# lisaweijler/SE3Conv3D

Measured on AMD Instinct MI355X. Metric: Mpoints/sec fwd+bwd PNEConvLayerRotEquiv (N=64k,k=32,F=2), higher is better.
Workload: dtype bf16x3 (fp32 split into bf16 hi+lo, 3 MFMA products, fp32 accumulate); 1 GPU; headline: 4-level PNEConvLayerRotEquiv stack, N=65536, k=32, F=2, C=64; conv-only fwd+bwd (dX,dA,dbeta,dW), one scene per GPU; n_points=65536, clouds_per_gpu=1, k=32, frames=2, num_basis=32, point_order=random, launch=hipGraph replay of the captured step, cpu_threads_per_rank=8

## Files before the change

se3conv3d_amd/_lib.py:

```python
from __future__ import annotations

import ctypes as C
import os

_PKG = os.path.dirname(os.path.abspath(__file__))
LIB_PATH = os.path.join(_PKG, "lib", f"libse3conv_hip{os.environ.get('SE3_LIB_SUFFIX', '')}.so")

SE3_OK = 0
ABI_VERSION = 6
PRECISIONS = {"fp32": 0, "bf16x3": 1, "bf16x3_t16": 2}
REL_ROT = {"6D": (0, 9), "matrix": (1, 12), "quaternion": (2, 7)}


class Se3Shape(C.Structure):

    _fields_ = [
        ("n_in", C.c_int64), ("n_out", C.c_int64), ("n_edges", C.c_int64),
        ("f_in", C.c_int32), ("f_out", C.c_int32), ("c_in", C.c_int32), ("c_out", C.c_int32),
        ("num_basis", C.c_int32), ("precision", C.c_int32),
    ]


class Se3Prepared(C.Structure):

    _fields_ = [("geom_in", C.c_void_p), ("geom_out", C.c_void_p), ("feat_words", C.c_void_p),
                ("geom_in_valid", C.c_int32), ("geom_out_valid", C.c_int32), ("feat_words_valid", C.c_int32)]


class Se3LibraryError(RuntimeError):
    pass


_P = C.c_void_p
_I64 = C.c_int64
_I32 = C.c_int32
_SZ = C.c_size_t
_F = C.c_float
_SHP = C.POINTER(Se3Shape)

SIGNATURES = {
    "se3_abi_version": (C.c_int, []),
    "se3_error_string": (C.c_char_p, [C.c_int]),
    "se3conv_intermediate_bytes_per_element": (C.c_int, [_SHP, C.c_int]),
    "se3conv_intermediate_row_bytes": (C.c_int64, [_SHP, C.c_int]),
    "se3_compute_keys": (C.c_int, [_P, _P, _P, _P, _P, _I64, _P, _P]),
    "se3_batch_aabb": (C.c_int, [_P, _P, _I64, _I32, _P, _P, _P]),
    "se3_grid_subsample_workspace_bytes": (_SZ, [_I64, _I32]),
    "se3_grid_subsample": (C.c_int, [_P, _P, _I64, _I32, _F, _P, _SZ, _P, _P, _P, _P, _P, _P, _P]),
    "se3_segment_pool": (C.c_int, [_P, _P, _P, _I64, _I32, _I32, _P, _P, _P]),
    "se3_segment_unpool": (C.c_int, [_P, _P, _P, _P, _I64, _I32, _I32, _P, _P]),
    "se3_frame_pool": (C.c_int, [_P, _I64, _I32, _I32, _I32, _P, _P, _P]),
    "se3_frame_unpool": (C.c_int, [_P, _P, _I64, _I32, _I32, _I32, _P, _P]),
    "se3_ball_query_grid": (C.c_int, [_P, _P, _I64, _I32, _F, _P, _P, _P, _P]),
    "se3_ball_query_grid_from_box": (C.c_int, [_P, _P, _I32, _F, _P, _P, _P]),
    "se3_ball_query_needs_grid": (C.c_int, [_I64]),
    "se3_ball_query_workspace_bytes": (_SZ, [_I64, _I64]),
    "se3_ball_query_count": (C.c_int, [_P, _P, _P, _P, _P, _P, _F, _I64, _I64, _P, _SZ, _P, _P]),
    "se3_ball_query_store": (C.c_int, [_P, _P, _F, _I64, _I64, _P, _SZ, _P, _I64, _P, _P]),
    "se3_ball_query_bounded": (C.c_int, [_P, _P, _P, _P, _P, _P, _F, _I64, _I64, _I32, _P, _SZ, _I64, _P, _P, _P, _P, _P]),
    "se3_ball_query_grid_bytes": (_SZ, [_I64]),
    "se3_ball_query_bounded_shared": (C.c_int, [_P, _P, _P, _P, _P, _P, _F, _I64, _I64, _I32, _P, _SZ, _I32, _P, _SZ, _I64, _P,
                                                _P, _P, _P, _P]),
    "se3_csr_transpose_workspace_bytes": (_SZ, [_I64]),
    "se3_csr_transpose": (C.c_int, [_P, _I64, _I64, _P, _SZ, _P, _P, _P, _P]),
    "se3_csr_transpose_bounded": (C.c_int, [_P, _I64, _P, _I64, _P, _SZ, _P, _P, _P, _P]),
    "se3_rot_tensors": (C.c_int, [_P, _P, _P, _P, _P, _P, _P, _SHP, _P, _P, _P, _P]),
    "se3_rot_tensors_rel": (C.c_int, [_P, _P, _P, _P, _P, _P, _P, _SHP, _I32, _P, _P, _P, _P]),
    "se3_feat_basis_proj": (C.c_int, [_P, _P, _P, _P, _I64, _I64, _I64, _I32, _I32, _P, _P]),
    "se3_feat_basis_proj_grad": (C.c_int, [_P, _P, _P, _P, _P, _I64, _I64, _I64, _I32, _I32, _P, _P, _P]),
    "se3conv_fwd_workspace_bytes": (_SZ, [_SHP, C.c_int]),
    "se3conv_fwd": (C.c_int, [_P] * 12 + [_SHP, _P, _P, _P, _SZ, _P]),
    "se3conv_bwd_workspace_bytes": (_SZ, [_SHP, C.c_int, C.c_int, C.c_int]),
    "se3conv_bwd_needs_t": (C.c_int, [_SHP, C.c_int]),
    "se3conv_bwd": (C.c_int, [_P] * 17 + [_SHP, _P, _P, _P, _P, _P, _SZ, _P]),
    "se3conv_fwd_prepared": (C.c_int, [_P] * 12 + [_SHP, _P, _P, _P, _SZ, _P, C.POINTER(Se3Prepared)]),
    "se3conv_bwd_prepared": (C.c_int, [_P] * 17 + [_SHP, _P, _P, _P, _P, _P, _SZ, _P, C.POINTER(Se3Prepared)]),
    "se3_knn_query": (C.c_int, [_P, _P, _I64, _I32, _P, _P]),
    "se3_knn_query_pair": (C.c_int, [_P, _P, _I64, _P, _P, _I64, _I32, _P, _P]),
    "se3_grid_pick": (C.c_int, [_P, _P, _P, _I64, _P, _P, _P]),
    "se3_rows_gather": (C.c_int, [_P, _P, _I64, _I64, _P, _P]),
    "se3_rows_scatter": (C.c_int, [_P, _P, _I64, _I64, _P, _P]),
    "se3_knn_query_grid_workspace_bytes": (C.c_size_t, [_I64]),
    "se3_knn_grid_params": (C.c_int, [_P, _I64, _P, _P, _I32, _I32, C.c_float, _P, _P, _P, _P]),
    "se3_knn_query_grid": (C.c_int, [_P, _P, _P, _P, _P, _I64, _I32, _P, _P, C.c_size_t, _P]),
    "se3_pca_frames": (C.c_int, [_P, _P, _I64, _I32, _I32, _P, _P]),
    "se3_shuffle_frames": (C.c_int, [_P, _P, _I64, _I32, _I32, _P, _P]),
    "se3_glue_workspace_bytes": (_SZ, [_I32]),
    "se3_bn_fwd": (C.c_int, [_P, _P, _P, _I64, _I32, _F, _F, _P, _P, _P, _P, _P, _P, _P, _SZ, _P]),
    "se3_affine_act": (C.c_int, [_P, _P, _P, _P, _I64, _I32, _I32, _P, _P]),
    "se3_bn_bwd": (C.c_int, [_P, _P, _P, _P, _P, _I64, _I32, _P, _P, _P, _P, _SZ, _P]),
    "se3_skip_fwd": (C.c_int, [_P, _P, _P, _P, _F, _P, _I64, _I32, _P, _P]),
    "se3_skip_bwd": (C.c_int, [_P, _P, _P, _P, _F, _P, _I64, _I32, _P, _P, _P, _SZ, _P]),
    "se3_bias_gelu_bwd": (C.c_int, [_P, _P, _P, _I64, _I32, _P, _P, _P, _SZ, _P]),
    "se3_linear_wgrad_workspace_bytes": (_SZ, [_I64, _I32, _I32]),
    "se3_linear_wgrad": (C.c_int, [_P, _P, _I64, _I32, _I32, _P, _P, _SZ, _P]),
    "se3_profile_enable": (C.c_int, [C.c_int]),
    "se3_profile_reset": (C.c_int, []),
    "se3_profile_read": (C.c_int, [C.c_char_p, C.POINTER(C.c_double), C.POINTER(C.c_int64)]),
    "se3_profile_tags": (C.c_int, [C.c_char_p, _SZ]),
}

CAPPED_SIGNATURES = {
    "se3_ball_query_capped_workspace_bytes": (_SZ, [_I64, _I64]),
    "se3_ball_query_capped": (C.c_int, [_P, _P, _P, _P, _P, _P, _F, _I64, _I64, _I32, _P, _SZ, _I32, _P, _SZ, _I64, _P, _P, _P, _P,
                                        _P, _I32, C.c_uint32, _P, _P]),
}

_lib = None


def load() -> C.CDLL:
    global _lib
    if _lib is not None:
        return _lib
    if not os.path.exists(LIB_PATH):
        raise Se3LibraryError(
            f"{LIB_PATH} not found: build it with `python -m se3conv3d_amd.build` "
            "(there is deliberately no CPU fallback for the HIP path)")
    lib = C.CDLL(LIB_PATH)
    lib.se3_abi_version.restype = C.c_int
    if lib.se3_abi_version() != ABI_VERSION:
        raise Se3LibraryError(f"{LIB_PATH} has ABI version {lib.se3_abi_version()}, this binding expects {ABI_VERSION}: "
                              "rebuild it (`python -m se3conv3d_amd.build`)")
    for name, (res, args) in list(SIGNATURES.items()) + list(CAPPED_SIGNATURES.items()):
        try:
            fn = getattr(lib, name)
        except AttributeError:
            raise Se3LibraryError(f"{LIB_PATH} does not export {name}: it was built from older sources -- rebuild it "
                                  "(`python -m se3conv3d_amd.build`)") from None
        fn.restype = res
        fn.argtypes = args
    _lib = lib
    return lib


def check(code: int, what: str) -> None:
    if code != SE3_OK:
        msg = load().se3_error_string(code).decode()
        raise Se3LibraryError(f"{what} failed with code {code}: {msg}")
```

se3conv3d_amd/build.py:

```python
from __future__ import annotations

import hashlib
import os
import shutil
import subprocess
import sys
from concurrent.futures import ThreadPoolExecutor

PKG = os.path.dirname(os.path.abspath(__file__))
CSRC = os.path.join(PKG, "csrc")
SUFFIX = os.environ.get("SE3_LIB_SUFFIX", "")
LIBDIR = os.path.join(PKG, "lib")
OBJDIR = os.path.join(LIBDIR, "obj" + SUFFIX) if SUFFIX else LIBDIR
LIB = os.path.join(LIBDIR, f"libse3conv_hip{SUFFIX}.so")
SOURCES = ["geometry.hip", "edge_kernels.hip", "edge_bf16.hip", "edge_dx.hip", "gemm.hip", "gemm_bf16.hip", "prep.hip", "frames.hip", "glue.hip", "api.hip"]
HEADERS = [os.path.join(CSRC, "common.h"), os.path.join(CSRC, "edge_bf16_body.h"), os.path.join(os.path.dirname(PKG), "include", "se3conv.h"),
           os.path.join(os.path.dirname(PKG), "include", "se3conv_capped.h")]
ARCH = "gfx950"
FLAGS = os.environ.get("SE3_CXXFLAGS", "").split() + ["-O3", "-fno-slp-vectorize", "-std=c++17", "-fPIC", f"--offload-arch={ARCH}", "-fno-gpu-rdc", "-Wall", "-Wno-unused-function"]


def _hipcc() -> str:
    exe = shutil.which("hipcc") or "/opt/rocm/bin/hipcc"
    if not os.path.exists(exe):
        raise RuntimeError("hipcc not found: the HIP library cannot be built on this machine")
    return exe


def _stale(target: str, deps) -> bool:
    if not os.path.exists(target):
        return True
    t = os.path.getmtime(target)
    return any(os.path.getmtime(d) > t for d in deps)


def _fingerprint() -> str:
    return hashlib.sha256(" ".join([ARCH, *FLAGS]).encode()).hexdigest()


def build(force: bool = False, verbose: bool = True) -> str:
    os.makedirs(OBJDIR, exist_ok=True)
    hipcc = _hipcc()
    stamp = os.path.join(OBJDIR, "build_flags.sha256")
    fp = _fingerprint()
    try:
        with open(stamp) as fh:
            same_flags = fh.read().strip() == fp
    except OSError:
        same_flags = False
    force = force or not same_flags
    objs, jobs = [], []
    for src in SOURCES:
        s = os.path.join(CSRC, src)
        o = os.path.join(OBJDIR, src.replace(".hip", ".o"))
        objs.append(o)
        if force or _stale(o, [s] + HEADERS):
            jobs.append([hipcc, *FLAGS, "-c", s, "-o", o])

    def run(cmd):
        if verbose:
            print(" ".join(cmd), flush=True)
        subprocess.run(cmd, check=True)

    if jobs:
        if os.path.exists(stamp):
            os.remove(stamp)
        with ThreadPoolExecutor(max_workers=min(6, len(jobs))) as ex:
            list(ex.map(run, jobs))
    if jobs or force or _stale(LIB, objs):
        run([hipcc, "-shared", "-fPIC", f"--offload-arch={ARCH}", "-Wl,--no-undefined", *objs, "-o", LIB])
    with open(stamp, "w") as fh:
        fh.write(fp + "\n")
    return LIB


if __name__ == "__main__":
    print(build(force="--force" in sys.argv))
```

se3conv3d_amd/csrc/api.hip:

```cpp
#include <cstdlib>
#include <cstring>
#include <map>
#include <mutex>
#include <string>
#include <utility>
#include <vector>

#include "common.h"

namespace se3 {

namespace {

__global__ void transpose_kernel(const float* __restrict__ src, float* __restrict__ dst, int rows, int cols) {
  const int64_t total = (int64_t)rows * cols;
  for (int64_t i = (int64_t)blockIdx.x * blockDim.x + threadIdx.x; i < total; i += (int64_t)gridDim.x * blockDim.x) {
    const int c = (int)(i / rows), r = (int)(i % rows);
    dst[i] = src[(int64_t)r * cols + c];
  }
}

__global__ void permute_weights_oki_kernel(const float* __restrict__ w, float* __restrict__ w2, int c_in, int kb,
                                           int c_out) {
  const int64_t total = (int64_t)c_in * kb * c_out;
  for (int64_t idx = (int64_t)blockIdx.x * blockDim.x + threadIdx.x; idx < total;
       idx += (int64_t)gridDim.x * blockDim.x) {
    const int i = (int)(idx % c_in);
    const int ok = (int)(idx / c_in);
    const int k = ok % kb, o = ok / kb;
    w2[idx] = w[((int64_t)i * kb + k) * c_out + o];
  }
}

__global__ __launch_bounds__(256) void reduce_param_partials_kernel(const float* __restrict__ partials, int n_partials,
                                                                    float* __restrict__ grad_axes,
                                                                    float* __restrict__ grad_biases, float scale) {
  __shared__ float red[256];
  const int i = blockIdx.x;
  float s = 0.f;
  for (int p = threadIdx.x; p < n_partials; p += 256) s += partials[(int64_t)p * kDescExt * kBasis + i];
  red[threadIdx.x] = s;
  __syncthreads();
  for (int w = 128; w > 0; w >>= 1) {
    if (threadIdx.x < w) red[threadIdx.x] += red[threadIdx.x + w];
    __syncthreads();
  }
  if (threadIdx.x == 0) {
    if (i < SE3_DESC_DIMS * kBasis) {
      if (grad_axes) grad_axes[i] = red[0] * scale;
    } else if (grad_biases) {
      grad_biases[i - SE3_DESC_DIMS * kBasis] = red[0] * scale;
    }
  }
}


__device__ __forceinline__ void matrix_to_quaternion(const float m[9], float q[4]) {
  const float t[4] = {1.0f + m[0] + m[4] + m[8], 1.0f + m[0] - m[4] - m[8], 1.0f - m[0] + m[4] - m[8],
                      1.0f - m[0] - m[4] + m[8]};
  float qa[4];
  int best = 0;
#pragma unroll
  for (int i = 0; i < 4; ++i) {
    qa[i] = t[i] > 0.f ? sqrtf(t[i]) : 0.f;
    if (qa[i] > qa[best]) best = i;
  }
  const float c[4][4] = {{qa[0] * qa[0], m[7] - m[5], m[2] - m[6], m[3] - m[1]},
                         {m[7] - m[5], qa[1] * qa[1], m[3] + m[1], m[2] + m[6]},
                         {m[2] - m[6], m[3] + m[1], qa[2] * qa[2], m[5] + m[7]},
                         {m[3] - m[1], m[6] + m[2], m[7] + m[5], qa[3] * qa[3]}};
  const float den = 2.0f * fmaxf(qa[best], 0.1f);
#pragma unroll
  for (int i = 0; i < 4; ++i) q[i] = (best == 0 ? c[0][i] : best == 1 ? c[1][i] : best == 2 ? c[2][i] : c[3][i]) / den;
}

template <int REL>
__global__ void rot_tensors_kernel(const float* __restrict__ pts_in, const float* __restrict__ pts_out,
                                   const float* __restrict__ frames_in, const float* __restrict__ frames_out,
                                   const int32_t* __restrict__ neighbors, const int32_t* __restrict__ ends,
                                   const float* __restrict__ rho_p, int64_t n_edges, int f_in, int f_out,
                                   float* __restrict__ desc, int32_t* __restrict__ fe_neighbors) {
  constexpr int D = REL == 0 ? 9 : (REL == 1 ? 12 : 7);
  const float rho = *rho_p;
  const int ff = f_in * f_out;
  for (int64_t t = (int64_t)blockIdx.x * blockDim.x + threadIdx.x; t < n_edges * ff;
       t += (int64_t)gridDim.x * blockDim.x) {
    const int64_t e = t / ff;
    const int ab = (int)(t - e * ff);
    const int a = ab / f_in, b = ab % f_in;
    const int s = neighbors[e * 2], p = neighbors[e * 2 + 1];
    const int start = s > 0 ? ends[s - 1] : 0;
    const int deg = ends[s] - start;
    const int64_t idx = (int64_t)ff * start + (int64_t)a * deg * f_in + (e - start) * f_in + b;
    float x[3], y[3], ri[9], ro[9], d[9];
#pragma unroll
    for (int i = 0; i < 3; ++i) x[i] = pts_in[(int64_t)p * 3 + i], y[i] = pts_out[(int64_t)s * 3 + i];
#pragma unroll
    for (int i = 0; i < 9; ++i)
      ri[i] = frames_in[((int64_t)p * f_in + b) * 9 + i], ro[i] = frames_out[((int64_t)s * f_out + a) * 9 + i];
    edge_descriptor(x, ri, y, ro, rho, d);
    if constexpr (REL == 0) {
#pragma unroll
      for (int i = 0; i < 9; ++i) desc[idx * 9 + i] = d[i];
    } else {
      float rel[9];
#pragma unroll
      for (int i = 0; i < 6; ++i) rel[i] = d[3 + i];
#pragma unroll
      for (int c = 0; c < 3; ++c) rel[6 + c] = ro[2] * ri[c] + ro[5] * ri[3 + c] + ro[8] * ri[6 + c];
#pragma unroll
      for (int i = 0; i < 3; ++i) desc[idx * D + i] = d[i];
      if constexpr (REL == 1) {
#pragma unroll
        for (int i = 0; i < 9; ++i) desc[idx * D + 3 + i] = rel[i];
      } else {
        float q[4];
        matrix_to_quaternion(rel, q);
#pragma unroll
        for (int i = 0; i < 4; ++i) desc[idx * D + 3 + i] = q[i];
      }
    }
    fe_neighbors[idx * 2] = s * f_out + a;
    fe_neighbors[idx * 2 + 1] = p * f_in + b;
  }
}

__global__ void rot_tensor_ends_kernel(const int32_t* __restrict__ ends, int64_t n_out, int f_in, int f_out,
                                       int32_t* __restrict__ fe_ends) {
  for (int64_t m = (int64_t)blockIdx.x * blockDim.x + threadIdx.x; m < n_out * f_out;
       m += (int64_t)gridDim.x * blockDim.x) {
    const int64_t s = m / f_out;
    const int a = (int)(m - s * f_out);
    const int start = s > 0 ? ends[s - 1] : 0;
    const int deg = ends[s] - start;
    fe_ends[m] = f_in * f_out * start + (a + 1) * deg * f_in;
  }
}

__global__ __launch_bounds__(256) void feat_basis_proj_kernel(const float* __restrict__ basis,
                                                              const float* __restrict__ feat,
                                                              const int32_t* __restrict__ neighbors,
                                                              const int32_t* __restrict__ ends, int channels, int kb,
                                                              float* __restrict__ out) {
  const int64_t m = blockIdx.x;
  const int start = m > 0 ? ends[m - 1] : 0, end = ends[m];
  const int k = threadIdx.x % kb, cg = threadIdx.x / kb, ncg = blockDim.x / kb;
  for (int c = cg; c < channels; c += ncg) {
    float acc = 0.f;
    for (int e = start; e < end; ++e)
      acc += basis[(int64_t)e * kb + k] * feat[(int64_t)neighbors[(int64_t)e * 2 + 1] * channels + c];
    out[(m * channels + c) * kb + k] = acc;
  }
}

__device__ __forceinline__ int row_of_edge(const int32_t* __restrict__ ends, int64_t n_rows, int64_t e) {
  int64_t lo = 0, hi = n_rows;
  while (lo < hi) {
    const int64_t mid = (lo + hi) >> 1;
    if (ends[mid] <= e) lo = mid + 1; else hi = mid;
  }
  return (int)lo;
// ... 285 lines not shown
  const size_t wsz = (size_t)s->c_in * kBasis * s->c_out * 4;
  l.slices = (s->num_basis + kBasis - 1) / kBasis;
  l.a32 = take(SE3_DESC_DIMS * kBasis * 4);
  l.b32 = take(kBasis * 4);
  l.w32 = take(wsz);
  l.out_tmp = take(l.slices > 1 ? out_tmp_bytes : 0);
  if (grads) {
    l.da32 = take(SE3_DESC_DIMS * kBasis * 4);
    l.db32 = take(kBasis * 4);
    l.dw32 = take(wsz);
  }
  l.inner = take(inner_bytes);
  l.total = off;
  return l;
}
int64_t slice_items(const se3conv_shape* s) {
  const int64_t n_w = (int64_t)s->c_in * kBasis * s->c_out;
  return n_w > SE3_DESC_DIMS * kBasis ? n_w : SE3_DESC_DIMS * kBasis;
}
se3conv_shape with_32_basis(const se3conv_shape* s) {
  se3conv_shape t = *s;
  t.num_basis = kBasis;
  return t;
}

}
}

using namespace se3;

extern "C" int se3_abi_version(void) { return SE3_ABI_VERSION; }

extern "C" const char* se3_error_string(int code) {
  switch (code) {
    case SE3_OK: return "ok";
    case SE3_ERR_INVALID_ARGUMENT: return "invalid argument (null pointer, negative size or bad shape)";
    case SE3_ERR_UNSUPPORTED: return "unsupported shape (int32-sized clouds; API-parity ops: K in {8, 16, 32, 64})";
    case SE3_ERR_WORKSPACE: return "workspace too small";
    case SE3_ERR_LAUNCH: return "HIP launch/runtime error";
    default: return "unknown error";
  }
}

extern "C" int se3_rot_tensors_rel(const float* pts_in, const float* pts_out, const float* frames_in,
                                   const float* frames_out, const int32_t* neighbors, const int32_t* ends,
                                   const float* rho, const se3conv_shape* s, int32_t rel_rot, float* desc,
                                   int32_t* fe_neighbors, int32_t* fe_ends, void* stream_) {
  if (!shape_ok(s) || rel_rot < SE3_REL_ROT_6D || rel_rot > SE3_REL_ROT_QUATERNION) return SE3_ERR_INVALID_ARGUMENT;
  if (s->n_edges * s->f_in * s->f_out >= (1ll << 31)) return SE3_ERR_UNSUPPORTED;
  hipStream_t stream = (hipStream_t)stream_;
  if (s->n_out > 0) {
    if (!ends || !fe_ends) return SE3_ERR_INVALID_ARGUMENT;
    hipLaunchKernelGGL(rot_tensor_ends_kernel, dim3(grid_for(s->n_out * s->f_out)), dim3(256), 0, stream, ends, s->n_out,
                       s->f_in, s->f_out, fe_ends);
  }
  if (s->n_edges > 0) {
    if (!pts_in || !pts_out || !frames_in || !frames_out || !neighbors || !ends || !rho || !desc || !fe_neighbors)
      return SE3_ERR_INVALID_ARGUMENT;
    const dim3 grid(grid_for(s->n_edges * s->f_in * s->f_out));
#define SE3_ROT(REL)                                                                                                  \
  hipLaunchKernelGGL(rot_tensors_kernel<REL>, grid, dim3(256), 0, stream, pts_in, pts_out, frames_in, frames_out, neighbors, \
                     ends, rho, s->n_edges, s->f_in, s->f_out, desc, fe_neighbors)
    if (rel_rot == SE3_REL_ROT_6D) SE3_ROT(0);
    else if (rel_rot == SE3_REL_ROT_MATRIX) SE3_ROT(1);
    else SE3_ROT(2);
#undef SE3_ROT
  }
  return check_launch();
}

extern "C" int se3_rot_tensors(const float* pts_in, const float* pts_out, const float* frames_in,
                               const float* frames_out, const int32_t* neighbors, const int32_t* ends,
                               const float* rho, const se3conv_shape* s, float* desc, int32_t* fe_neighbors,
                               int32_t* fe_ends, void* stream) {
  return se3_rot_tensors_rel(pts_in, pts_out, frames_in, frames_out, neighbors, ends, rho, s, SE3_REL_ROT_6D, desc,
                             fe_neighbors, fe_ends, stream);
}

static bool basis_count_ok(int kb) { return kb == 8 || kb == 16 || kb == 32 || kb == 64; }

extern "C" int se3_feat_basis_proj(const float* basis, const float* feat, const int32_t* neighbors, const int32_t* ends,
                                   int64_t n_edges, int64_t n_rows, int64_t n_feat, int32_t channels,
                                   int32_t num_basis, float* out, void* stream) {
  if (n_edges < 0 || n_rows < 0 || n_feat < 0 || channels < 1) return SE3_ERR_INVALID_ARGUMENT;
  if (!basis_count_ok(num_basis)) return SE3_ERR_UNSUPPORTED;
  if (n_rows == 0) return SE3_OK;
  if (!ends || !out || (n_edges > 0 && (!basis || !feat || !neighbors))) return SE3_ERR_INVALID_ARGUMENT;
  if (n_rows >= (1ll << 31)) return SE3_ERR_UNSUPPORTED;
  hipLaunchKernelGGL(feat_basis_proj_kernel, dim3((unsigned)n_rows), dim3(256), 0, (hipStream_t)stream, basis, feat,
                     neighbors, ends, channels, num_basis, out);
  return check_launch();
}

extern "C" int se3_feat_basis_proj_grad(const float* basis, const float* feat, const int32_t* neighbors,
                                        const int32_t* ends, const float* grad_out, int64_t n_edges, int64_t n_rows,
                                        int64_t n_feat, int32_t channels, int32_t num_basis, float* g_feat,
                                        float* g_basis, void* stream_) {
  if (n_edges < 0 || n_rows < 0 || n_feat < 0 || channels < 1) return SE3_ERR_INVALID_ARGUMENT;
  if (!basis_count_ok(num_basis)) return SE3_ERR_UNSUPPORTED;
  hipStream_t stream = (hipStream_t)stream_;
  if (n_feat > 0) {
    if (!g_feat) return SE3_ERR_INVALID_ARGUMENT;
    if (int rc = launch_fill_words(g_feat, 0u, n_feat * channels, stream)) return rc;
  }
  if (n_edges == 0) return SE3_OK;
  if (!basis || !feat || !neighbors || !ends || !grad_out || !g_basis) return SE3_ERR_INVALID_ARGUMENT;
  hipLaunchKernelGGL(feat_basis_proj_grad_basis_kernel, dim3(grid_for(n_edges * num_basis)), dim3(256), 0, stream, feat,
                     neighbors, ends, grad_out, n_edges, n_rows, channels, num_basis, g_basis);
  hipLaunchKernelGGL(feat_basis_proj_grad_feat_kernel, dim3(grid_for(n_edges * channels)), dim3(256), 0, stream, basis,
                     neighbors, ends, grad_out, n_edges, n_rows, channels, num_basis, g_feat);
  return check_launch();
}

static int64_t intermediate_row_bytes(const se3conv_shape* s, int which) {
  const int64_t ck = (int64_t)(which == 1 ? s->c_out : s->c_in) * s->num_basis;
  if (s->precision == SE3_PRECISION_FP32 || s->num_basis != kBasis || which == 2) return ck * 4;
  const BwdPlan p = plan_bwd(s, true, true, false);
  const int fmt = which == 0 ? p.fmt_t : p.fmt_u;
  return fmt == 2 ? t16_row_bytes(which == 0 ? s->c_in : s->c_out) : ck * (fmt == 1 ? 3 : 4);
}
extern "C" int64_t se3conv_intermediate_row_bytes(const se3conv_shape* s, int which) {
  if (!shape_ok(s) || which < 0 || which > 2) return SE3_ERR_INVALID_ARGUMENT;
  return intermediate_row_bytes(s, which);
}
extern "C" int se3conv_intermediate_bytes_per_element(const se3conv_shape* s, int which) {
  if (!shape_ok(s) || which < 0 || which > 2) return SE3_ERR_INVALID_ARGUMENT;
  const int64_t ck = (int64_t)(which == 1 ? s->c_out : s->c_in) * s->num_basis;
  return (int)(intermediate_row_bytes(s, which) / ck);
}

extern "C" size_t se3conv_fwd_workspace_bytes(const se3conv_shape* s, int save_t) {
  if (!shape_ok(s)) return 0;
  if (s->num_basis != kBasis) {
    const se3conv_shape s32 = with_32_basis(s);
    return any_basis_layout(s, (size_t)s->n_out * s->f_out * s->c_out * 4, false, plan_fwd(&s32, false).total).total;
  }
  return plan_fwd(s, save_t != 0).total;
}

extern "C" int se3conv_fwd(const float* pts_in, const float* pts_out, const float* frames_in, const float* frames_out,
                           const int32_t* neighbors, const int32_t* ends, const float* feat, const float* proj_axes,
                           const float* proj_biases, const float* conv_weights, const float* rho, const float* nu,
                           const se3conv_shape* s, float* out, float* t_save, void* workspace, size_t workspace_bytes,
                           void* stream_) {
  return se3conv_fwd_prepared(pts_in, pts_out, frames_in, frames_out, neighbors, ends, feat, proj_axes, proj_biases, conv_weights,
                              rho, nu, s, out, t_save, workspace, workspace_bytes, stream_, nullptr);
}

extern "C" int se3conv_fwd_prepared(const float* pts_in, const float* pts_out, const float* frames_in, const float* frames_out,
                                    const int32_t* neighbors, const int32_t* ends, const float* feat, const float* proj_axes,
                                    const float* proj_biases, const float* conv_weights, const float* rho, const float* nu,
                                    const se3conv_shape* s, float* out, float* t_save, void* workspace, size_t workspace_bytes,
                                    void* stream_, const se3conv_prepared* prep) {
  if (!shape_ok(s)) return SE3_ERR_INVALID_ARGUMENT;
  if (s->num_basis != kBasis) {
    if (s->n_out == 0) return SE3_OK;
    if (!proj_axes || !proj_biases || !conv_weights || !out || !workspace) return SE3_ERR_INVALID_ARGUMENT;
    const se3conv_shape s32 = with_32_basis(s);
    const int64_t n_out_el = s->n_out * s->f_out * s->c_out;
    const AnyBasisLayout l = any_basis_layout(s, (size_t)n_out_el * 4, false, plan_fwd(&s32, false).total);
    if (workspace_bytes < l.total) return SE3_ERR_WORKSPACE;
    hipStream_t stream = (hipStream_t)stream_;
    char* ws = (char*)workspace;
    float *a32 = (float*)(ws + l.a32), *b32 = (float*)(ws + l.b32), *w32 = (float*)(ws + l.w32);
    for (int sl = 0; sl < l.slices; ++sl) {
      const int k0 = sl * kBasis, kn = s->num_basis - k0 < kBasis ? s->num_basis - k0 : kBasis;
      hipLaunchKernelGGL(slice_params_kernel, dim3(grid_for(slice_items(s))), dim3(256), 0, stream,
                         proj_axes, proj_biases, conv_weights, s->num_basis, k0, kn, s->c_in, s->c_out, a32, b32, w32);
      float* dst = sl == 0 ? out : (float*)(ws + l.out_tmp);
      if (int rc = se3conv_fwd(pts_in, pts_out, frames_in, frames_out, neighbors, ends, feat, a32, b32, w32, rho, nu, &s32, dst,
                               nullptr, ws + l.inner, l.total - l.inner, stream_))
        return rc;
      if (sl > 0)
        hipLaunchKernelGGL(add_into_kernel, dim3(grid_for(n_out_el)), dim3(256), 0, stream, out, dst, n_out_el);
    }
    return check_launch();
  }
  if (int rc = shape_supported(s)) return rc;
  if (s->n_out == 0) return SE3_OK;
  if (!pts_out || !frames_out || !ends || !proj_axes || !proj_biases || !conv_weights || !rho || !nu || !out ||
      !workspace || (s->n_edges > 0 && (!pts_in || !frames_in || !neighbors || !feat)))
    return SE3_ERR_INVALID_ARGUMENT;
  const FwdPlan p = plan_fwd(s, t_save != nullptr);
  if (workspace_bytes < p.total) return SE3_ERR_WORKSPACE;
  hipStream_t stream = (hipStream_t)stream_;
  char* ws = (char*)workspace;
  float* axes_ext = (float*)(ws + p.axes_ext);
  float* t = t_save ? t_save : (float*)(ws + p.t);

  EdgeGeom g = forward_geom(s, pts_in, pts_out, frames_in, frames_out, neighbors, ends);
  const int64_t rows_out = s->n_out * s->f_out;
  const int ck = s->c_in * s->num_basis;
  const float inv_fin = 1.0f / (float)s->f_in;
  PrepBatch pb;
  pb.axes(proj_axes, proj_biases, axes_ext);
  prepare_geometry(pb, prep, s, (float*)(ws + p.geom_in), (float*)(ws + p.geom_out), &g, nullptr);
  if (s->precision == SE3_PRECISION_FP32) {
    if (int rc = pb.launch(stream)) return rc;
    if (int rc = launch_edge_t("edge_t_fwd", g, feat, s->c_in, s->n_in * s->f_in, axes_ext, rho, t, stream)) return rc;
    return launch_gemm_nn("gemm_out", t, conv_weights, out, rows_out, s->c_out, ck, nu, inv_fin, stream, (float*)(ws + p.split));
  }
  uint32_t* featpk = prep && prep->feat_words ? prep->feat_words : (uint32_t*)(ws + p.featpk);
  const bool need_featpk = !(prep && prep->feat_words && prep->feat_words_valid);
  uint16_t* bt_hi = (uint16_t*)(ws + p.bt_hi);
  uint16_t* bt_lo = (uint16_t*)(ws + p.bt_lo);
  const float inv_phi = inv_fin / kGeluOut;
  if (need_featpk) pb.split(feat, featpk, s->n_in * s->f_in * s->c_in);
  pb.weights(conv_weights, s->c_in, s->num_basis, s->c_out, 0, bt_hi, bt_lo, nullptr, 1.0f, false, p.fmt_t);
  if (int rc = pb.launch(stream)) return rc;
  if (int rc = launch_edge_t_bf16("edge_t_fwd", g, featpk, s->c_in, s->n_in * s->f_in, axes_ext, rho, (uint32_t*)t, stream, p.fmt_t))
    return rc;
  return launch_gemm_nn_bf16("gemm_out", (const uint32_t*)t, bt_hi, bt_lo, out, false, rows_out, s->c_out, ck,
                             (float*)(ws + p.split), nu, inv_phi, stream, p.fmt_t);
}

extern "C" int se3conv_bwd_needs_t(const se3conv_shape* s, int want_feat) {
  if (!shape_ok(s)) return SE3_ERR_INVALID_ARGUMENT;
  if (s->num_basis != kBasis) return 0;
  return plan_bwd(s, want_feat != 0, true, false).dw == WeightGrad::u ? 0 : 1;
}

extern "C" size_t se3conv_bwd_workspace_bytes(const se3conv_shape* s, int want_feat, int want_params, int have_t) {
  if (!shape_ok(s)) return 0;
  if (s->num_basis != kBasis) {
    const se3conv_shape s32 = with_32_basis(s);
    return any_basis_layout(s, want_feat ? (size_t)s->n_in * s->f_in * s->c_in * 4 : 0, want_params != 0,
                            plan_bwd(&s32, want_feat != 0, want_params != 0, false).total).total;
  }
  return plan_bwd(s, want_feat != 0, want_params != 0, have_t != 0).total;
}

extern "C" int se3conv_bwd(const float* pts_in, const float* pts_out, const float* frames_in, const float* frames_out,
                           const int32_t* neighbors, const int32_t* ends, const int32_t* t_samples,
                           const int32_t* t_ends, const int32_t* t_edge_ids, const float* feat, const float* proj_axes,
                           const float* proj_biases,
                           const float* conv_weights, const float* rho, const float* nu, const float* t_save,
                           const float* grad_out, const se3conv_shape* s, float* grad_feat, float* grad_axes,
                           float* grad_biases, float* grad_weights, void* workspace, size_t workspace_bytes,
                           void* stream_) {
  return se3conv_bwd_prepared(pts_in, pts_out, frames_in, frames_out, neighbors, ends, t_samples, t_ends, t_edge_ids, feat, proj_axes,
                              proj_biases, conv_weights, rho, nu, t_save, grad_out, s, grad_feat, grad_axes, grad_biases, grad_weights,
                              workspace, workspace_bytes, stream_, nullptr);
}

extern "C" int se3conv_bwd_prepared(const float* pts_in, const float* pts_out, const float* frames_in, const float* frames_out,
                                    const int32_t* neighbors, const int32_t* ends, const int32_t* t_samples,
                                    const int32_t* t_ends, const int32_t* t_edge_ids, const float* feat, const float* proj_axes,
                                    const float* proj_biases, const float* conv_weights, const float* rho, const float* nu,
                                    const float* t_save, const float* grad_out, const se3conv_shape* s, float* grad_feat,
                                    float* grad_axes, float* grad_biases, float* grad_weights, void* workspace,
                                    size_t workspace_bytes, void* stream_, const se3conv_prepared* prep) {
  if (!shape_ok(s)) return SE3_ERR_INVALID_ARGUMENT;
  if (s->num_basis != kBasis) {
    const bool wf = grad_feat != nullptr, wp = grad_axes || grad_biases || grad_weights;
    if (!wf && !wp) return SE3_OK;
    if (!proj_axes || !proj_biases || !conv_weights || !workspace) return SE3_ERR_INVALID_ARGUMENT;
    const se3conv_shape s32 = with_32_basis(s);
    const int64_t n_in_el = s->n_in * s->f_in * s->c_in;
    const AnyBasisLayout l = any_basis_layout(s, wf ? (size_t)n_in_el * 4 : 0, wp, plan_bwd(&s32, wf, wp, false).total);
    if (workspace_bytes < l.total) return SE3_ERR_WORKSPACE;
    hipStream_t stream = (hipStream_t)stream_;
    char* ws = (char*)workspace;
    float *a32 = (float*)(ws + l.a32), *b32 = (float*)(ws + l.b32), *w32 = (float*)(ws + l.w32);
    float *da32 = wp ? (float*)(ws + l.da32) : nullptr, *db32 = wp ? (float*)(ws + l.db32) : nullptr;
    float* dw32 = wp ? (float*)(ws + l.dw32) : nullptr;
    const dim3 pgrid(grid_for(slice_items(s)));
    for (int sl = 0; sl < l.slices; ++sl) {
      const int k0 = sl * kBasis, kn = s->num_basis - k0 < kBasis ? s->num_basis - k0 : kBasis;
      hipLaunchKernelGGL(slice_params_kernel, pgrid, dim3(256), 0, stream, proj_axes, proj_biases, conv_weights,
                         s->num_basis, k0, kn, s->c_in, s->c_out, a32, b32, w32);
      float* dx = !wf ? nullptr : (sl == 0 ? grad_feat : (float*)(ws + l.out_tmp));
      if (int rc = se3conv_bwd(pts_in, pts_out, frames_in, frames_out, neighbors, ends, t_samples, t_ends, t_edge_ids, feat, a32, b32, w32, rho,
                               nu, nullptr, grad_out, &s32, dx, da32, db32, dw32, ws + l.inner, l.total - l.inner, stream_))
        return rc;
      if (wf && sl > 0 && n_in_el > 0)
        hipLaunchKernelGGL(add_into_kernel, dim3(grid_for(n_in_el)), dim3(256), 0, stream, grad_feat, dx, n_in_el);
      if (wp)
        hipLaunchKernelGGL(unslice_grads_kernel, pgrid, dim3(256), 0, stream, da32, db32, dw32, s->num_basis, k0, kn, s->c_in,
                           s->c_out, grad_axes, grad_biases, grad_weights);
    }
    return check_launch();
  }
  if (int rc = shape_supported(s)) return rc;
  const bool want_feat = grad_feat != nullptr;
  const bool want_params = grad_axes || grad_biases || grad_weights;
  if (!want_feat && !want_params) return SE3_OK;
  if (!proj_axes || !proj_biases || !conv_weights || !rho || !nu || !workspace) return SE3_ERR_INVALID_ARGUMENT;
  if (s->n_out > 0 && (!pts_out || !frames_out || !ends || !grad_out)) return SE3_ERR_INVALID_ARGUMENT;
  if (s->n_in > 0 && (!pts_in || !frames_in || !feat)) return SE3_ERR_INVALID_ARGUMENT;
  if (s->n_edges > 0 && !neighbors) return SE3_ERR_INVALID_ARGUMENT;
  if (want_feat && s->n_in > 0 && (!t_ends || (s->n_edges > 0 && !t_samples))) return SE3_ERR_INVALID_ARGUMENT;
  const BwdPlan p = plan_bwd(s, want_feat, want_params, t_save != nullptr);
  if (workspace_bytes < p.total) return SE3_ERR_WORKSPACE;
  hipStream_t stream = (hipStream_t)stream_;
  char* ws = (char*)workspace;
  float* axes_ext = (float*)(ws + p.axes_ext);
  float* big = (float*)(ws + p.big);
  const int kb = s->num_basis;
  const int ck = s->c_in * kb;
  const int64_t rows_out = s->n_out * s->f_out, rows_in = s->n_in * s->f_in;
  const float inv_fin = 1.0f / (float)s->f_in;
  float* partials = (float*)(ws + p.param_partials);
  float* tn_partials = (float*)(ws + p.tn_partials);

  EdgeGeom g = forward_geom(s, pts_in, pts_out, frames_in, frames_out, neighbors, ends);
  EdgeGeom gt = transposed_geom(s, pts_in, pts_out, frames_in, frames_out, t_samples, t_ends);
  PrepBatch pb;
  pb.axes(proj_axes, proj_biases, axes_ext);
  prepare_geometry(pb, prep, s, (float*)(ws + p.geom_in), (float*)(ws + p.geom_out), &g, &gt);

  if (!p.fast) {
    if (int rc = pb.launch(stream)) return rc;
    if (want_params) {
      float* wt = (float*)(ws + p.wt);
      hipLaunchKernelGGL(transpose_kernel, dim3(grid_for((int64_t)ck * s->c_out)), dim3(256), 0, stream, conv_weights,
                         wt, ck, s->c_out);
      if (int rc = launch_gemm_nn("gemm_gradT", grad_out, wt, big, rows_out, ck, s->c_out, nu, inv_fin, stream)) return rc;
      if (grad_axes || grad_biases) {
        int n_part = 0;
        if (int rc = launch_edge_param_grad("edge_param_grad", g, feat, s->c_in, rows_in, axes_ext, rho, big, partials,
                                            p.n_param_partials, &n_part, stream))
          return rc;
        hipLaunchKernelGGL(reduce_param_partials_kernel, dim3(kDescExt * kBasis), dim3(256), 0, stream, partials,
                           n_part, grad_axes, grad_biases, 1.0f);
      }
      if (grad_weights) {
        const float* t = t_save;
        if (p.dw == WeightGrad::t_recomputed) {
          float* tt = (float*)(ws + p.t);
          if (int rc = launch_edge_t("edge_t_recompute", g, feat, s->c_in, rows_in, axes_ext, rho, tt, stream)) return rc;
          t = tt;
        }
        if (int rc = launch_gemm_tn("gemm_gradW", t, grad_out, grad_weights, tn_partials, p.tn.splits, p.tn.m, p.tn.ka,
                                    p.tn.n, nu, inv_fin, stream))
          return rc;
      }
    }
    if (p.feat_branch) {
      float* u = (float*)(ws + p.u);
      if (int rc = launch_edge_t("edge_t_transposed", gt, grad_out, s->c_out, rows_out, axes_ext, rho, u, stream)) return rc;
      float* w2 = (float*)(ws + p.w2);
      hipLaunchKernelGGL(permute_weights_oki_kernel, dim3(grid_for((int64_t)ck * s->c_out)), dim3(256), 0, stream,
                         conv_weights, w2, s->c_in, kb, s->c_out);
      if (int rc = launch_gemm_nn("gemm_gradX", u, w2, grad_feat, rows_in, s->c_in, s->c_out * kb, nu, inv_fin, stream,
                                  (float*)(ws + p.split_x)))
        return rc;
    }
    return check_launch();
  }

  const bool u_form = p.feat_branch && p.feat == FeatGrad::u, edge_major = p.feat == FeatGrad::edge_major;
  uint16_t* bt_hi = (uint16_t*)(ws + p.bt_hi);
  uint16_t* bt_lo = (uint16_t*)(ws + p.bt_lo);
  uint16_t* bx_hi = (uint16_t*)(ws + p.bx_hi);
  uint16_t* bx_lo = (uint16_t*)(ws + p.bx_lo);
  uint32_t* gpk = (uint32_t*)(ws + p.gpk);
  const bool have_featpk = prep && prep->feat_words && prep->feat_words_valid;
  uint32_t* featpk = prep && prep->feat_words ? prep->feat_words : (uint32_t*)(ws + p.featpk);
  uint32_t* bigw = (uint32_t*)big;
  uint32_t* u = (uint32_t*)(ws + p.u);
  const float inv_phi = inv_fin / kGeluOut;
  pb.split(grad_out, gpk, rows_out * s->c_out);
  if (u_form) pb.weights(conv_weights, s->c_in, kb, s->c_out, 2, bx_hi, bx_lo, nullptr, 1.0f, false, p.fmt_u);
  if (want_params && !have_featpk) pb.split(feat, featpk, rows_in * s->c_in);
  if (p.grad_t)
    pb.weights(conv_weights, s->c_in, kb, s->c_out, 1, bt_hi, bt_lo, nu, inv_fin, p.strip_t);
  if (int rc = pb.launch(stream)) return rc;
  ReduceBatch final_sums;

  if (u_form) {
    if (int rc = launch_edge_t_bf16("edge_t_transposed", gt, gpk, s->c_out, rows_out, axes_ext, rho, u, stream, p.fmt_u))
      return rc;
  }
  if (p.grad_t) {
    if (int rc = p.strip_t ? launch_gemm_strip_bf16("gemm_gradT", gpk, bt_hi, bt_lo, bigw, rows_out, ck, s->c_out, stream)
                           : launch_gemm_nn_bf16("gemm_gradT", gpk, bt_hi, bt_lo, bigw, true, rows_out, ck, s->c_out,
                                                 (float*)(ws + p.split), nullptr, 1.0f, stream))
      return rc;
  }
  if (edge_major) {
    float* d_rows = (float*)(ws + p.dx_rows);
    if (int rc = launch_edge_dx_bf16("edge_dx", g, axes_ext, rho, bigw, s->c_in, d_rows, stream)) return rc;
    if (int rc = launch_dx_gather_sum("dx_gather", d_rows, neighbors, ends, t_samples, t_ends, t_edge_ids, s->n_in, s->f_in * s->c_in,
                                      1.0f / kGeluOut, grad_feat, stream))
      return rc;
  }
  if (grad_axes || grad_biases) {
    int n_part = 0;
    if (int rc = launch_edge_param_grad_bf16("edge_param_grad", g, featpk, s->c_in, rows_in, axes_ext, rho, bigw, partials,
                                             p.n_param_partials, &n_part, stream))
      return rc;
    final_sums.params(partials, n_part, grad_axes, grad_biases, 0.5f);
  }
  if (u_form) {
    if (int rc = launch_gemm_nn_bf16("gemm_gradX", u, bx_hi, bx_lo, grad_feat, false, rows_in, s->c_in, s->c_out * kb,
                                     (float*)(ws + p.split_x), nu, inv_phi, stream, p.fmt_u, &final_sums))
      return rc;
  }
  if (grad_weights) {
    if (p.dw == WeightGrad::u) {
      if (int rc = launch_gemm_tn_bf16("gemm_gradW", u, featpk, grad_weights, tn_partials, p.tn.splits, p.tn.m, p.tn.ka, p.tn.n,
                                       nu, inv_phi, stream, p.fmt_u, &final_sums, true))
        return rc;
    } else {
      const uint32_t* t = (const uint32_t*)t_save;
      if (p.dw == WeightGrad::t_recomputed) {
        uint32_t* tt = (uint32_t*)(ws + p.t);
        if (int rc = launch_edge_t_bf16("edge_t_recompute", g, featpk, s->c_in, rows_in, axes_ext, rho, tt, stream, p.fmt_t)) return rc;
        t = tt;
      }
      if (int rc = launch_gemm_tn_bf16("gemm_gradW", t, gpk, grad_weights, tn_partials, p.tn.splits, p.tn.m, p.tn.ka, p.tn.n, nu,
                                       inv_phi, stream, p.fmt_t, &final_sums))
        return rc;
    }
  }
  return final_sums.launch(stream);
}


namespace se3 {
namespace {
struct ProfRec { std::string tag; hipEvent_t start, stop; };
std::mutex g_prof_mu;
bool g_prof_on = false;
std::vector<ProfRec> g_prof_recs;
std::map<std::string, std::pair<double, int64_t>> g_prof_acc;
ProfRec* g_prof_open = nullptr;

void prof_drain_locked() {
  for (auto& r : g_prof_recs) {
    float ms = 0.f;
    if (hipEventSynchronize(r.stop) == hipSuccess && hipEventElapsedTime(&ms, r.start, r.stop) == hipSuccess) {
      auto& a = g_prof_acc[r.tag];
      a.first += ms;
      a.second += 1;
    }
    (void)hipEventDestroy(r.start);
    (void)hipEventDestroy(r.stop);
  }
  g_prof_recs.clear();
}
}

void prof_begin(const char* tag, hipStream_t stream) {
  if (!g_prof_on) return;
  std::lock_guard<std::mutex> lk(g_prof_mu);
  ProfRec r;
  r.tag = tag;
  if (hipEventCreate(&r.start) != hipSuccess || hipEventCreate(&r.stop) != hipSuccess) return;
  (void)hipEventRecord(r.start, stream);
  g_prof_recs.push_back(r);
  g_prof_open = &g_prof_recs.back();
}

void prof_end(hipStream_t stream) {
  if (!g_prof_on) return;
  std::lock_guard<std::mutex> lk(g_prof_mu);
  if (g_prof_open) (void)hipEventRecord(g_prof_open->stop, stream);
  g_prof_open = nullptr;
// ... 38 lines not shown
```

se3conv3d_amd/csrc/common.h:

```cpp
#pragma once

#include <hip/hip_runtime.h>
#include <stddef.h>
#include <stdint.h>

#include "../../include/se3conv.h"

namespace se3 {

using f32x16 = __attribute__((__vector_size__(16 * sizeof(float)))) float;
using f32x4 = __attribute__((__vector_size__(4 * sizeof(float)))) float;

constexpr int kWave = 64;
constexpr int kBasis = 32;
constexpr int kDescExt = 10;

__host__ __device__ constexpr int acc_row(int reg, int h) { return (reg & 3) + 8 * (reg >> 2) + 4 * h; }

__device__ __forceinline__ f32x16 mfma32(float a, float b, f32x16 c) {
  return __builtin_amdgcn_mfma_f32_32x32x2f32(a, b, c, 0, 0, 0);
}

using bf16x8 = __attribute__((__vector_size__(8 * sizeof(__bf16)))) __bf16;
using bf16x2 = __attribute__((__vector_size__(2 * sizeof(__bf16)))) __bf16;
// ... 132 lines not shown
  gelu_erf_core(x, s, a, e, hq);
  return fmaf(a, hq, 0.5f * x);
}

constexpr float kGeluIn = 0.84932180028801904272f;
constexpr float kGeluOut = 2.0f * kGeluIn;
__device__ __forceinline__ void gelu_scaled_core(float xp, float& a, float& e, float& hq2) {
  a = fabsf(xp);
  const float t = __builtin_amdgcn_rcpf(fmaf(0.23164189f / kGeluIn, a, 1.0f));
  float p = fmaf(1.061405429f, t, -1.453152027f);
  p = fmaf(p, t, 1.421413741f);
  p = fmaf(p, t, -0.284496736f);
  p = fmaf(p, t, 0.254829592f);
  e = __builtin_amdgcn_exp2f(-(xp * xp));
  hq2 = fmaf(-(p * t), e, 1.0f);
}
#ifndef SE3_GELU_POLY
#define SE3_GELU_POLY 5
#endif
__device__ __forceinline__ float gelu_scaled(float xp) {
#if SE3_GELU_POLY == 0
  float a, e, hq2;
  gelu_scaled_core(xp, a, e, hq2);
  return fmaf(a, hq2, xp);
#else
  const float a = fabsf(xp);
#if SE3_GELU_POLY == 7
  float p = fmaf(-3.000000106e-06f, a, 1.157411680e-04f);
  p = fmaf(p, a, -1.839424018e-03f);
  p = fmaf(p, a, 1.570610516e-02f);
  p = fmaf(p, a, -8.734710515e-02f);
  p = fmaf(p, a, -6.359119415e-01f);
  p = fmaf(p, a, -1.355453730e+00f);
  p = fmaf(p, a, 8.137106306e-06f);
#else
  float p = fmaf(-1.070951186e-03f, a, 1.361500331e-02f);
  p = fmaf(p, a, -8.459421670e-02f);
  p = fmaf(p, a, -6.376852093e-01f);
  p = fmaf(p, a, -1.354949055e+00f);
  p = fmaf(p, a, -3.763227806e-05f);
#endif
  const float q2 = __builtin_amdgcn_exp2f(p);
  return fmaf(-a, q2, a + xp);
#endif
}
__device__ __forceinline__ void gelu_scaled_grad(float xp, float& y2, float& dy2) {
  float a, e, hq2;
  gelu_scaled_core(xp, a, e, hq2);
  y2 = fmaf(a, hq2, xp);
  dy2 = fmaf(__builtin_copysignf(1.0f, xp), fmaf(a * e, 0.79788456080286535588f / kGeluIn, hq2), 1.0f);
}
#ifndef SE3_GELU_DPOLY
#define SE3_GELU_DPOLY (SE3_GELU_POLY ? 7 : 0)
#endif
__device__ __forceinline__ float gelu_scaled_dgrad(float xp) {
#if SE3_GELU_DPOLY == 0
  float y2, dy2;
  gelu_scaled_grad(xp, y2, dy2);
  return dy2;
#else
  const float a = fabsf(xp);
  float p = fmaf(-6.029059296e-05f, a, 9.206497925e-04f);
  p = fmaf(p, a, -6.434103474e-03f);
  p = fmaf(p, a, 2.816033363e-02f);
  p = fmaf(p, a, -8.932273835e-02f);
  p = fmaf(p, a, -7.773189545e-01f);
  p = fmaf(p, a, -4.511650503e-01f);
  p = fmaf(p, a, 6.472119689e-01f);
  const float g = fmaf(a - 6.385129094e-01f, __builtin_amdgcn_exp2f(p), 1.0f);
  return fmaf(__builtin_copysignf(1.0f, xp), g, 1.0f);
#endif
}

__device__ __forceinline__ void edge_descriptor(const float x_in[3], const float r_in[9],
                                                const float y_out[3], const float r_out[9],
                                                float rho, float d[9]) {
  const float v0 = (x_in[0] - y_out[0]) * rho;
  const float v1 = (x_in[1] - y_out[1]) * rho;
  const float v2 = (x_in[2] - y_out[2]) * rho;
#pragma unroll
  for (int c = 0; c < 3; ++c) d[c] = v0 * r_out[c] + v1 * r_out[3 + c] + v2 * r_out[6 + c];
#pragma unroll
  for (int r = 0; r < 2; ++r)
#pragma unroll
    for (int c = 0; c < 3; ++c)
      d[3 + 3 * r + c] = r_out[r] * r_in[c] + r_out[3 + r] * r_in[3 + c] + r_out[6 + r] * r_in[6 + c];
}

constexpr int kOobOffset = 0x7fff0000;

__device__ __forceinline__ __amdgpu_buffer_rsrc_t buffer_of(const void* p, int64_t bytes) {
  const uint32_t n = bytes > 0xffffffffll ? 0xffffffffu : (uint32_t)bytes;
  return __builtin_amdgcn_make_buffer_rsrc(const_cast<void*>(p), (short)0, (int)n, 0x00020000);
}

__device__ __forceinline__ void load_geom_record(const __amdgpu_buffer_rsrc_t rs, int row, float x[3], float r[9]) {
  const int off = row * 64;
  const auto v0 = __builtin_amdgcn_raw_buffer_load_b128(rs, off, 0, 0);
  const auto v1 = __builtin_amdgcn_raw_buffer_load_b128(rs, off + 16, 0, 0);
  const auto v2 = __builtin_amdgcn_raw_buffer_load_b128(rs, off + 32, 0, 0);
  x[0] = __uint_as_float(v0[0]), x[1] = __uint_as_float(v0[1]), x[2] = __uint_as_float(v0[2]);
  r[8] = __uint_as_float(v0[3]);
#pragma unroll
  for (int i = 0; i < 4; ++i) r[i] = __uint_as_float(v1[i]), r[4 + i] = __uint_as_float(v2[i]);
}

#ifndef SE3_ROTATE_PRIO
#define SE3_ROTATE_PRIO 1
#endif
__device__ __forceinline__ void rotate_priority(int step_plus_slot) {
#if SE3_ROTATE_PRIO
  switch (step_plus_slot & 3) {
    case 0: __builtin_amdgcn_s_setprio(0); break;
    case 1: __builtin_amdgcn_s_setprio(1); break;
    case 2: __builtin_amdgcn_s_setprio(2); break;
    default: __builtin_amdgcn_s_setprio(3); break;
  }
#endif
}
__device__ __forceinline__ int wave_slot_id() { return (int)__builtin_amdgcn_s_getreg((4 << 0) | (0 << 6) | (3 << 11)) ; }

inline int check_launch() {
  hipError_t e = hipGetLastError();
  return e == hipSuccess ? SE3_OK : SE3_ERR_LAUNCH;
}

inline size_t align_up(size_t v, size_t a) { return (v + a - 1) / a * a; }

int launch_fill_words(void* dst, uint32_t value, int64_t n_words, hipStream_t stream);

void prof_begin(const char* tag, hipStream_t stream);
void prof_end(hipStream_t stream);
struct ProfScope {
  hipStream_t s;
  ProfScope(const char* tag, hipStream_t stream) : s(stream) { prof_begin(tag, s); }
  ~ProfScope() { prof_end(s); }
};

struct EdgeGeom {
  const float* ctr_pts;
  const float* ctr_frames;
  const float* nb_pts;
  const float* nb_frames;
  const float* ctr_geom;
  const float* nb_geom;
  int64_t n_nb;
  int64_t n_edges;
  const int32_t* nbr;
  int nbr_stride, nbr_offset;
  const int32_t* ends;
  int64_t n_ctr;
  int f_ctr, f_nb;
  int transposed;
};

int launch_edge_t(const char* tag, const EdgeGeom& g, const float* feat, int channels, int64_t feat_rows,
                  const float* axes_ext, const float* rho, float* t_out, hipStream_t stream);
int launch_edge_param_grad(const char* tag, const EdgeGeom& g, const float* feat, int channels, int64_t feat_rows,
                           const float* axes_ext, const float* rho, const float* grad_t, float* partials,
                           int n_partials, int* n_used, hipStream_t stream);
int edge_param_grad_blocks(int64_t rows);

int launch_gemm_nn(const char* tag, const float* a, const float* b, float* c, int64_t m, int n, int k,
                   const float* alpha_num, float alpha_scale, hipStream_t stream, float* split_ws = nullptr);
size_t gemm_nn_split_bytes(int64_t m, int n, int k);
int launch_gemm_tn(const char* tag, const float* a, const float* b, float* c, float* partials, int splits, int64_t m,
                   int ka, int n, const float* alpha_num, float alpha_scale, hipStream_t stream);
int gemm_tn_splits(int64_t m, int ka, int n);
int launch_reduce_partials(const float* partials, float* out, int64_t count, int splits, const float* alpha_num,
                           float alpha_scale, hipStream_t stream);

struct ReduceJob {
  int type, blocks;
  const float* partials;
  void *out, *out2;
  int64_t count;
  int splits, packed;
  const float* alpha_num;
  float alpha_scale;
  int perm_n;
};
struct ReduceJobs {
  int count;
  ReduceJob job[4];
};
struct ReduceBatch {
  ReduceJobs jobs{};
  void sum(const float* partials, void* out, int64_t count, int splits, const float* alpha_num, float alpha_scale, bool packed,
           int perm_n = 0);
  void params(const float* partials, int n_partials, float* grad_axes, float* grad_biases, float scale);
  int launch(hipStream_t stream);
};

int launch_split_pack(const float* src, uint32_t* dst, int64_t n, hipStream_t stream);
bool edge_t_bf16_t24_rows(const EdgeGeom& g, int channels);
bool edge_t_bf16_t16_rows(const EdgeGeom& g, int channels);
int launch_edge_t_bf16(const char* tag, const EdgeGeom& g, const uint32_t* feat, int channels, int64_t feat_rows,
                       const float* axes_ext, const float* rho, uint32_t* t_out, hipStream_t stream,
                       int rowfmt = 0);
int edge_param_grad_bf16_channel_blocks(int channels);
int launch_edge_param_grad_bf16(const char* tag, const EdgeGeom& g, const uint32_t* feat, int channels,
                                int64_t feat_rows, const float* axes_ext, const float* rho, const uint32_t* grad_t,
                                float* partials, int n_partials, int* n_used, hipStream_t stream);
bool edge_dx_bf16_applicable(const EdgeGeom& g, int channels);
int launch_edge_dx_bf16(const char* tag, const EdgeGeom& g, const float* axes_ext, const float* rho, const uint32_t* grad_t,
                        int channels, float* d_rows, hipStream_t stream);
int launch_dx_gather_sum(const char* tag, const float* d_rows, const int32_t* neighbors, const int32_t* ends,
                         const int32_t* t_samples, const int32_t* t_ends, const int32_t* t_edge_ids, int64_t n_src, int width,
                         float scale, float* grad_feat, hipStream_t stream);
int launch_prep_weights(const float* w, int c_in, int kb, int c_out, int mode, uint16_t* bt_hi, uint16_t* bt_lo,
                        hipStream_t stream, const float* scale_num = nullptr, float scale = 1.0f,
                        bool frag_layout = false);
__device__ __forceinline__ float knn_dist2(float dx, float dy, float dz) { return fmaf(dz, dz, fmaf(dy, dy, dx * dx)); }
int launch_knn_bruteforce(const float* pts, const int32_t* batch_ids, int64_t n, const float* qpts, const int32_t* qbatch,
                          int64_t m, int k, int32_t* out, hipStream_t stream);
int launch_knn_listed(const float* pts, const int32_t* batch_ids, int64_t n, int k, int32_t* out, const int32_t* list,
                      const int32_t* list_count, hipStream_t stream);

template <int K>
struct TopK {
  uint64_t key[K];
  static __device__ __forceinline__ uint64_t pack(float d, int i) {
    return ((uint64_t)__float_as_uint(d) << 32) | (uint64_t)(uint32_t)i;
  }
  __device__ __forceinline__ float dist(int e) const { return __uint_as_float((uint32_t)(key[e] >> 32)); }
  __device__ __forceinline__ int idx(int e) const { return (int)(uint32_t)key[e]; }
  __device__ __forceinline__ void set(int e, float d, int i) { key[e] = pack(d, i); }
  __device__ __forceinline__ void init() {
#pragma unroll
    for (int e = 0; e < K; ++e) key[e] = pack(3.0e38f, 0x7fffffff);
  }
  __device__ __forceinline__ void cas(int a, int b) {
    const uint64_t x = key[a], y = key[b];
    const bool sw = y < x;
    key[a] = sw ? y : x, key[b] = sw ? x : y;
  }
  __device__ __forceinline__ void insert(float dd, int jj) {
    const uint64_t k = pack(dd, jj);
    if (!(k < key[K - 1])) return;
    key[K - 1] = k;
#pragma unroll
    for (int e = K - 1; e > 0; --e) cas(e - 1, e);
  }
  __device__ __forceinline__ void merge_xor(int mask) {
    uint64_t tmp[K];
#pragma unroll
    for (int e = 0; e < K; ++e) {
      const uint32_t lo = (uint32_t)__shfl_xor((int)(uint32_t)key[K - 1 - e], mask);
      const uint32_t hi = (uint32_t)__shfl_xor((int)(uint32_t)(key[K - 1 - e] >> 32), mask);
      tmp[e] = ((uint64_t)hi << 32) | lo;
    }
#pragma unroll
    for (int e = 0; e < K; ++e)
      if (tmp[e] < key[e]) key[e] = tmp[e];
#pragma unroll
    for (int s = K / 2; s > 0; s >>= 1)
#pragma unroll
      for (int e = 0; e < K; ++e)
        if ((e & s) == 0) cas(e, e + s);
  }
};

struct PrepJob {
  int type, blocks;
  const void *a, *b;
  void *o0, *o1;
  int64_t n;
  int p[8];
  float scale;
};
struct PrepJobs {
  int count;
  PrepJob job[8];
};
struct PrepBatch {
  PrepJobs jobs{};
  int status = SE3_OK;
  void axes(const float* axes, const float* biases, float* ext);
  void geometry(const float* pts, const float* frames, int64_t n, int f, float* records);
  void split(const float* src, uint32_t* dst, int64_t n);
  void weights(const float* w, int c_in, int kb, int c_out, int mode, uint16_t* bt_hi, uint16_t* bt_lo,
               const float* scale_num = nullptr, float scale = 1.0f, bool frag_layout = false,
               int a_rowfmt = 0);
  int launch(hipStream_t stream);
};

int launch_pack_geometry(const float* pts, const float* frames, int64_t n, int f, float* records, hipStream_t stream);
bool gemm_strip_bf16_applicable(int64_t m, int n, int k);
int launch_gemm_strip_bf16(const char* tag, const uint32_t* a, const uint16_t* bt_hi, const uint16_t* bt_lo, uint32_t* c,
                           int64_t m, int n, int k, hipStream_t stream);
int launch_gemm_nn_bf16(const char* tag, const uint32_t* a, const uint16_t* bt_hi, const uint16_t* bt_lo, void* c,
                        bool out_packed, int64_t m, int n, int k, float* split_ws, const float* alpha_num,
                        float alpha_scale, hipStream_t stream, int afmt = 0, ReduceBatch* defer = nullptr);
size_t gemm_nn_bf16_split_bytes(int64_t m, int n, int k);
int launch_gemm_tn_bf16(const char* tag, const uint32_t* a, const uint32_t* b, float* c, float* partials, int splits,
                        int64_t m, int ka, int n, const float* alpha_num, float alpha_scale, hipStream_t stream, int afmt = 0,
                        ReduceBatch* defer = nullptr,
                        bool out_ikn = false);

}
```

se3conv3d_amd/csrc/edge_bf16.hip:

```cpp
#include <cstdlib>

#include "common.h"
#include "edge_bf16_body.h"

#ifndef SE3_TIMELINE
#define SE3_TIMELINE 0
#endif
#if SE3_TIMELINE
#define TL(...) __VA_ARGS__
namespace se3 {
constexpr int kTlWords = 64;
__device__ uint32_t* g_tl_buf = nullptr;
__device__ uint32_t g_tl_cap = 0;
__device__ __forceinline__ uint32_t tl_now() {
  unsigned long long t;
  __builtin_amdgcn_sched_barrier(0);
  asm volatile("s_memtime %0\n\ts_waitcnt lgkmcnt(0)" : "=s"(t)::"memory");
  __builtin_amdgcn_sched_barrier(0);
  return (uint32_t)t;
}
template <class T>
__device__ __forceinline__ void tl_pin(const T& x) { asm volatile("" ::"v"(x)); }
__device__ __forceinline__ void tl_mark(uint32_t* rec, int slot) { const uint32_t t = tl_now(); if (slot < kTlWords) rec[slot] = t; }
__device__ __forceinline__ void tl_seg(uint32_t* rec, uint32_t& prev, int slot) { const uint32_t t = tl_now(); rec[slot] += t - prev; prev = t; }
// ... 164 lines not shown
#pragma unroll
      for (int t = 0; t < CT; ++t) acc[a][t] = zero16();
    int nb_b = 0, q_a = 0;
    float xn_nx[3], rn_nx[9];
    if (n_total > 0) {
      const int nb_a = nbr_of(0);
      nb_b = nbr_of(32);
      TL(tl_mark(tl_rec, 4); tl_pin(nb_a); tl_mark(tl_rec, 5);)
      q_a = row_of(nb_a, 0);
      load_geom_record(nbg_rs, q_a, xn_nx, rn_nx);
    }
    TL(tl_mark(tl_rec, 6);)
    for (int c0 = 0; c0 < n_total; c0 += 32, buf ^= 1) {
      const int cnt = min(32, n_total - c0);
      const int qoff = c0 + kcol < n_total ? q_a * row_bytes : kOobOffset;
      float xn[3], rn[9], d[9];
#pragma unroll
      for (int i = 0; i < 3; ++i) asm volatile("" : "+v"(yc[i]));
#pragma unroll
      for (int i = 0; i < 9; ++i) asm volatile("" : "+v"(rc[i]));
#pragma unroll
      for (int i = 0; i < 3; ++i) xn[i] = xn_nx[i];
#pragma unroll
      for (int i = 0; i < 9; ++i) rn[i] = rn_nx[i];
      const int q_b = row_of(nb_b, c0 + 32);
      nb_b = nbr_of(c0 + 64);

      uint32_t fw[CT][2][8];
#pragma unroll
      for (int s = 0; s < 2; ++s)
#pragma unroll
        for (int j = 0; j < 8; ++j) {
          const int src_off = __builtin_amdgcn_ds_bpermute(hb + 4 * acc_row(8 * s + j, 0), qoff);
#pragma unroll
          for (int t = 0; t < CT; ++t)
            fw[t][s][j] = __builtin_amdgcn_raw_buffer_load_b32(feat_rs, ch_ok[t] ? src_off + cb4[t] : kOobOffset, 0, 0);
        }
      load_geom_record(nbg_rs, q_b, xn_nx, rn_nx);
      q_a = q_b;
      TL(tl_mark(tl_rec, tl_ch + 1); tl_pin(xn[0]); tl_pin(rn[7]); tl_pin(rn[8]); tl_mark(tl_rec, tl_ch + 2);)

      if (TR == 0 || (TR < 0 && !g.transposed))
        edge_descriptor(xn, rn, yc, rc, rho, d);
      else
        edge_descriptor(yc, rc, xn, rn, rho, d);

      {
        float v[8];
#pragma unroll
        for (int j = 0; j < 8; ++j) v[j] = h ? (j == 0 ? d[8] : (j == 1 ? 1.0f : 0.f)) : d[j];
        u32x4 a_hi, a_lo;
        frags_from_floats(v, a_hi, a_lo);
        const u32x4 wb_hi = *reinterpret_cast<const u32x4*>(&lds_w[0][0][lane][0]);
        const u32x4 wb_lo = *reinterpret_cast<const u32x4*>(&lds_w[0][1][lane][0]);
        const f32x16 phi = mfma_bf16x3(a_hi, a_lo, wb_hi, wb_lo, zero16());
        TL(tl_pin(phi[0]); tl_mark(tl_rec, tl_ch + 3);)
#pragma unroll
        for (int s = 0; s < 2; ++s) {
          if (s * 16 < cnt && (NF == 2 || s == wv)) {
            float pv[8];
#pragma unroll
            for (int j = 0; j < 8; ++j) pv[j] = gelu_scaled(phi[8 * s + j]);
            u32x4 b_hi, b_lo;
            frags_from_floats(pv, b_hi, b_lo);
            *reinterpret_cast<u32x4*>(&lds_phi[buf][NF == 2 ? wv : 0][s][0][lane][0]) = b_hi;
            *reinterpret_cast<u32x4*>(&lds_phi[buf][NF == 2 ? wv : 0][s][1][lane][0]) = b_lo;
          }
        }
      }
      TL(tl_mark(tl_rec, tl_ch + 4);)
      __syncthreads();
      TL(tl_mark(tl_rec, tl_ch + 5); tl_pin(fw[0][0][7]); tl_mark(tl_rec, tl_ch + 6);)
#pragma unroll
      for (int s = 0; s < 2; ++s) {
        if (s * 16 < cnt) {
          u32x4 b_hi[NF], b_lo[NF];
#pragma unroll
          for (int a = 0; a < NF; ++a) {
            b_hi[a] = *reinterpret_cast<const u32x4*>(&lds_phi[buf][a][s][0][lane][0]);
            b_lo[a] = *reinterpret_cast<const u32x4*>(&lds_phi[buf][a][s][1][lane][0]);
          }
#pragma unroll
          for (int t = 0; t < CT; ++t) {
            u32x4 fa_hi, fa_lo;
            frags_from_words(fw[t][s], fa_hi, fa_lo);
#pragma unroll
            for (int a = 0; a < NF; ++a) acc[a][t] = mfma_bf16x3(fa_hi, fa_lo, b_hi[a], b_lo[a], acc[a][t]);
          }
        }
      }
      TL(tl_mark(tl_rec, tl_ch + 7); tl_ch += 8;)
    }
    TL(tl_mark(tl_rec, 7); tl_pin(acc[NF - 1][CT - 1][15]); tl_mark(tl_rec, 8);)
#pragma unroll
    for (int a = 0; a < NF; ++a)
#pragma unroll
      for (int t = 0; t < CT; ++t) {
        const int ch0 = cbase + 32 * (CT * wv + t);
        if (t24 == 2) {
          if (!FULL && ch0 >= C) continue;
          char* row = reinterpret_cast<char*>(t_out) + (item * NF + a) * t16_row_bytes(C);
          uint8_t* expo = reinterpret_cast<uint8_t*>(row) + (int64_t)C * kBasis * 2;
#pragma unroll
          for (int j = 0; j < 4; ++j) {
            const int cq = (ch0 >> 2) + 2 * j + h;
            uint32_t m01, m23, eb;
            t16_pack4(acc[a][t][4 * j], acc[a][t][4 * j + 1], acc[a][t][4 * j + 2], acc[a][t][4 * j + 3], m01, m23, eb);
            typedef uint32_t u32x2s __attribute__((ext_vector_type(2)));
            __builtin_nontemporal_store(u32x2s{m01, m23}, reinterpret_cast<u32x2s*>(row) + cq * kBasis + kcol);
            __builtin_nontemporal_store((uint8_t)eb, expo + t16_exp_pos(cq * kBasis + kcol));
          }
          continue;
        }
        if (t24) {
          char* row = reinterpret_cast<char*>(t_out) + (item * NF + a) * t24_row_bytes(C);
#pragma unroll
          for (int r = 0; r < 16; r += 2) {
            const int ch = ch0 + acc_row(r, h);
            if (!FULL && ch >= C) continue;
            uint32_t hp, lp;
            t24_pack2(acc[a][t][r], (FULL || ch + 1 < C) ? acc[a][t][r + 1] : 0.f, hp, lp);
            const int idx = (ch >> 1) * kBasis + kcol;
            __builtin_nontemporal_store(hp, reinterpret_cast<uint32_t*>(row) + idx);
            __builtin_nontemporal_store((uint16_t)lp, reinterpret_cast<uint16_t*>(row + (int64_t)C * kBasis * 2) + idx);
          }
          continue;
        }
        uint32_t* t_row = t_out + ((item * NF + a) * (int64_t)C + ch0) * kBasis;
#pragma unroll
        for (int r = 0; r < 16; r += 2) {
          uint32_t w0, w1;
          split_pack2(acc[a][t][r], acc[a][t][r + 1], w0, w1);
          if (FULL || ch0 + acc_row(r, h) < C) __builtin_nontemporal_store(w0, &t_row[acc_row(r, h) * kBasis + kcol]);
          if (FULL || ch0 + acc_row(r + 1, h) < C) __builtin_nontemporal_store(w1, &t_row[acc_row(r + 1, h) * kBasis + kcol]);
        }
      }
    if (cbase + 64 * CT < C) __syncthreads();
  }
  TL(tl_mark(tl_rec, 9); __builtin_amdgcn_s_waitcnt(0); tl_mark(tl_rec, 10);
     tl_rec[11] = __builtin_amdgcn_s_getreg((4 << 0) | (0 << 6) | (31 << 11)); tl_rec[12] = __builtin_amdgcn_s_getreg((20 << 0) | (0 << 6) | (31 << 11));
     tl_rec[13] = (uint32_t)item; tl_rec[14] = (uint32_t)((tl_ch - 16) >> 3); tl_flush(TR == 1 ? 1 : 0, (uint32_t)(item - item_lo) * 2 + wv, tl_rec);)
  }
}

struct ChunkCursor {
  int j;
  int c0;
  int start;
  int n_total;
  int crow;
  uint32_t item;
};

template <int TR>
__global__ __launch_bounds__(128, SE3_PAIR_WAVES) void edge_t_stream_bf16_kernel(
    EdgeGeom g, const uint32_t* __restrict__ feat, int64_t feat_rows, const float* __restrict__ axes_ext,
    const float* __restrict__ rho_p, char* __restrict__ t_out, uint32_t item_lo, uint32_t item_hi, int fnb_shift) {
  constexpr int C = 64, row_bytes = C * 4;
  __shared__ __attribute__((aligned(16))) uint32_t lds_w[1][2][64][4];
  __shared__ __attribute__((aligned(16))) uint32_t lds_phi[2][2][2][2][64][4];
  TL(__shared__ uint32_t tl_lds[2][kTlWords]; uint32_t* tl_rec = tl_lds[threadIdx.x >> 6]; tl_rec[threadIdx.x & 63] = 0u; tl_mark(tl_rec, 0); uint32_t tl_chunks = 0;)
  const int lane = threadIdx.x & 63, wv = threadIdx.x >> 6;
  const int kcol = lane & 31, h = lane >> 5;
  if (threadIdx.x < 64) mlp_weights_to_lds<1>(lds_w, axes_ext, threadIdx.x);
  __syncthreads();
  const float rho = *rho_p;
  const __amdgpu_buffer_rsrc_t feat_rs = buffer_of(feat, feat_rows * row_bytes);
  const __amdgpu_buffer_rsrc_t nbg_rs = buffer_of(g.nb_geom, g.n_nb * g.f_nb * 64);
  const __amdgpu_buffer_rsrc_t nbr_rs = buffer_of(g.nbr, g.n_edges * g.nbr_stride * 4);
  const uint32_t groups = (uint32_t)g.f_ctr / 2u;
  const uint32_t item0_wg = item_lo + blockIdx.x;
  const int n_mine = (int)((item_hi - item0_wg + gridDim.x - 1) / gridDim.x);
  const int fmask = (1 << fnb_shift) - 1;
  const int hb = 16 * h;

  f32x16 acc[2] = {zero16(), zero16()};
  int buf = 0;
  int prio_step = wave_slot_id();
  const int n_all = n_mine;
  for (int win0 = 0; win0 < n_all; win0 += 64) {
  const int n_mine = min(64, n_all - win0);
  const uint32_t item0 = item0_wg + (uint32_t)win0 * gridDim.x;
  int v_lo, v_hi;
  {
    const uint32_t item = item0 + (uint32_t)min(lane, n_mine - 1) * gridDim.x;
    const uint32_t ctr = item / groups;
    v_hi = g.ends[ctr];
    v_lo = g.ends[max((int)ctr - 1, 0)];
    if (ctr == 0) v_lo = 0;
  }
  auto uni = [](int x) { return __builtin_amdgcn_readfirstlane(x); };
  auto enter = [&](int j, int crow_keep, uint32_t item_keep) {
    ChunkCursor c;
    c.j = j, c.c0 = 0, c.start = 0, c.n_total = 0;
    c.crow = crow_keep, c.item = item_keep;
    if (j < n_mine) {
      const int lo = __builtin_amdgcn_readlane(v_lo, j), hi = __builtin_amdgcn_readlane(v_hi, j);
      c.start = lo, c.n_total = (hi - lo) << fnb_shift;
      c.item = item0 + (uint32_t)j * gridDim.x;
      const uint32_t ctr = c.item / groups;
      c.crow = uni((int)(ctr * (uint32_t)g.f_ctr + (c.item - ctr * groups) * 2u) + wv);
    }
    return c;
  };
  auto advance = [&](const ChunkCursor& c) {
    ChunkCursor r = c;
    if (c.c0 + 32 < c.n_total) r.c0 = c.c0 + 32;
    else if (c.j < n_mine) r = enter(c.j + 1, c.crow, c.item);
    r.j = uni(r.j), r.c0 = uni(r.c0), r.start = uni(r.start), r.n_total = uni(r.n_total), r.item = (uint32_t)uni((int)r.item);
    return r;
  };
  auto fe_of = [&](const ChunkCursor& c) { return max(min(c.c0 + kcol, c.n_total - 1), 0); };
  auto nbr_of = [&](const ChunkCursor& c) {
    const int e = c.start + (fe_of(c) >> fnb_shift);
    return (int)__builtin_amdgcn_raw_buffer_load_b32(nbr_rs, (e * g.nbr_stride + g.nbr_offset) * 4, 0, 0);
  };
  auto row_of = [&](int nb, const ChunkCursor& c) { return (nb << fnb_shift) + (fe_of(c) & fmask); };
  typedef const f32x4 __attribute__((address_space(4))) * crec_t;
  const crec_t ctr_rec = (crec_t)(uintptr_t)g.ctr_geom;
  auto centre = [&](const ChunkCursor& c, float yc[3], float rc[9]) {
    const int row = c.crow;
    const f32x4 v0 = ctr_rec[row * 4], v1 = ctr_rec[row * 4 + 1], v2 = ctr_rec[row * 4 + 2];
    yc[0] = v0[0], yc[1] = v0[1], yc[2] = v0[2], rc[8] = v0[3];
#pragma unroll
    for (int i = 0; i < 4; ++i) rc[i] = v1[i], rc[4 + i] = v2[i];
  };

  ChunkCursor cur, n1, n2;
  cur = enter(0, 0, 0u);
  n1 = advance(cur);
  n2 = advance(n1);
  int q_cur, q_n1;
  float xn_nx[3], rn_nx[9];
  {
    const int nb_cur = nbr_of(cur);
    const int nb_n1 = nbr_of(n1);
    q_cur = row_of(nb_cur, cur);
    load_geom_record(nbg_rs, q_cur, xn_nx, rn_nx);
    q_n1 = row_of(nb_n1, n1);
#pragma unroll
    for (int i = 0; i < 3; ++i) asm volatile("" : "+v"(xn_nx[i]));
#pragma unroll
    for (int i = 0; i < 9; ++i) asm volatile("" : "+v"(rn_nx[i]));
  }
  float yc[3], rc[9];
  centre(cur, yc, rc);

  while (cur.j < n_mine) {
    rotate_priority(prio_step++);
    const int cnt = min(32, cur.n_total - cur.c0);
    const int qoff = cur.c0 + kcol < cur.n_total ? q_cur * row_bytes : kOobOffset;
    float xn[3], rn[9], d[9];
#pragma unroll
    for (int i = 0; i < 3; ++i) xn[i] = xn_nx[i];
#pragma unroll
    for (int i = 0; i < 9; ++i) rn[i] = rn_nx[i];
    const int nb_n2 = nbr_of(n2);

    uint32_t fw[2][8];
#pragma unroll
    for (int s = 0; s < 2; ++s)
#pragma unroll
      for (int j = 0; j < 8; ++j) {
        const int src_off = __builtin_amdgcn_ds_bpermute(hb + 4 * acc_row(8 * s + j, 0), qoff);
        fw[s][j] = __builtin_amdgcn_raw_buffer_load_b32(feat_rs, src_off + (32 * wv + kcol) * 4, 0, 0);
      }
    load_geom_record(nbg_rs, q_n1, xn_nx, rn_nx);
    float yn[3], rnc[9];
    centre(n1, yn, rnc);

    if (TR == 0)
      edge_descriptor(xn, rn, yc, rc, rho, d);
    else
      edge_descriptor(yc, rc, xn, rn, rho, d);

    {
      float v[8];
#pragma unroll
      for (int j = 0; j < 8; ++j) v[j] = h ? (j == 0 ? d[8] : (j == 1 ? 1.0f : 0.f)) : d[j];
      u32x4 a_hi, a_lo;
      frags_from_floats(v, a_hi, a_lo);
      const u32x4 wb_hi = *reinterpret_cast<const u32x4*>(&lds_w[0][0][lane][0]);
      const u32x4 wb_lo = *reinterpret_cast<const u32x4*>(&lds_w[0][1][lane][0]);
      const f32x16 phi = mfma_bf16x3(a_hi, a_lo, wb_hi, wb_lo, zero16());
#pragma unroll
      for (int s = 0; s < 2; ++s) {
        if (s * 16 < cnt) {
          float pv[8];
#pragma unroll
          for (int j = 0; j < 8; ++j) pv[j] = gelu_scaled(phi[8 * s + j]);
          u32x4 b_hi, b_lo;
          frags_from_floats(pv, b_hi, b_lo);
          *reinterpret_cast<u32x4*>(&lds_phi[buf][wv][s][0][lane][0]) = b_hi;
          *reinterpret_cast<u32x4*>(&lds_phi[buf][wv][s][1][lane][0]) = b_lo;
        }
      }
    }
    __syncthreads();
#pragma unroll
    for (int s = 0; s < 2; ++s) {
      if (s * 16 < cnt) {
        u32x4 b_hi[2], b_lo[2];
#pragma unroll
        for (int a = 0; a < 2; ++a) {
          b_hi[a] = *reinterpret_cast<const u32x4*>(&lds_phi[buf][a][s][0][lane][0]);
          b_lo[a] = *reinterpret_cast<const u32x4*>(&lds_phi[buf][a][s][1][lane][0]);
        }
        u32x4 fa_hi, fa_lo;
        frags_from_words(fw[s], fa_hi, fa_lo);
#pragma unroll
        for (int a = 0; a < 2; ++a) acc[a] = mfma_bf16x3(fa_hi, fa_lo, b_hi[a], b_lo[a], acc[a]);
      }
    }
    q_cur = q_n1;
    q_n1 = row_of(nb_n2, n2);
#pragma unroll
    for (int i = 0; i < 3; ++i) asm volatile("" : "+v"(xn_nx[i]));
#pragma unroll
    for (int i = 0; i < 9; ++i) asm volatile("" : "+v"(rn_nx[i]));
    if (n1.j != cur.j) {
#pragma unroll
      for (int a = 0; a < 2; ++a) {
        char* row = t_out + ((int64_t)cur.item * 2 + a) * t24_row_bytes(C);
#pragma unroll
        for (int r = 0; r < 16; r += 2) {
          uint32_t hp, lp;
          t24_pack2(acc[a][r], acc[a][r + 1], hp, lp);
          const int idx = ((32 * wv + acc_row(r, h)) >> 1) * kBasis + kcol;
          __builtin_nontemporal_store(hp, reinterpret_cast<uint32_t*>(row) + idx);
          __builtin_nontemporal_store((uint16_t)lp, reinterpret_cast<uint16_t*>(row + (int64_t)C * kBasis * 2) + idx);
        }
        acc[a] = zero16();
      }
    }
#pragma unroll
    for (int i = 0; i < 3; ++i) yc[i] = yn[i];
#pragma unroll
    for (int i = 0; i < 9; ++i) rc[i] = rnc[i];
    cur = n1, n1 = n2, n2 = advance(n2);
    buf ^= 1;
    TL(++tl_chunks;)
  }
  }
  TL(tl_mark(tl_rec, 9); __builtin_amdgcn_s_waitcnt(0); tl_mark(tl_rec, 10);
     tl_rec[11] = __builtin_amdgcn_s_getreg((4 << 0) | (0 << 6) | (31 << 11)); tl_rec[12] = __builtin_amdgcn_s_getreg((20 << 0) | (0 << 6) | (31 << 11));
     tl_rec[14] = tl_chunks; tl_rec[15] = (uint32_t)n_all; tl_flush(TR == 1 ? 1 : 0, blockIdx.x * 2 + wv, tl_rec);)
}

template <int VW, int FC, int TR>
__global__ __launch_bounds__(256, (VW == 1 && FC == 1) ? 4 : 3) void edge_t_stream1_bf16_kernel(
    EdgeGeom g, const uint32_t* __restrict__ feat, int64_t feat_rows, const float* __restrict__ axes_ext,
    const float* __restrict__ rho_p, char* __restrict__ t_out, uint32_t item_lo, uint32_t item_hi, int fnb_shift) {
  constexpr int C = 32 * VW, row_bytes = C * 4;
  __shared__ __attribute__((aligned(16))) uint32_t lds_w[FC][2][64][4];
  const int lane = threadIdx.x & 63;
  const int kcol = lane & 31, h = lane >> 5;
  if (threadIdx.x < 64) mlp_weights_to_lds<FC>(lds_w, axes_ext, threadIdx.x);
  __syncthreads();
  const float rho = *rho_p;
  const __amdgpu_buffer_rsrc_t feat_rs = buffer_of(feat, feat_rows * row_bytes);
  const __amdgpu_buffer_rsrc_t nbg_rs = buffer_of(g.nb_geom, g.n_nb * g.f_nb * 64);
  const __amdgpu_buffer_rsrc_t nbr_rs = buffer_of(g.nbr, g.n_edges * g.nbr_stride * 4);
  const uint32_t groups = (uint32_t)g.f_ctr / (uint32_t)FC;
  const uint32_t n_waves = gridDim.x * 4u;
  const uint32_t item0_wave = item_lo + (uint32_t)__builtin_amdgcn_readfirstlane((int)(blockIdx.x * 4u + (threadIdx.x >> 6)));
  const int n_all = item0_wave < item_hi ? (int)((item_hi - item0_wave + n_waves - 1) / n_waves) : 0;
  const int fmask = (1 << fnb_shift) - 1;
  const int hb = 16 * h;
  const int cb4 = VW * kcol * 4;

  f32x16 acc[FC][VW];
#pragma unroll
  for (int a = 0; a < FC; ++a)
#pragma unroll
    for (int t = 0; t < VW; ++t) acc[a][t] = zero16();
  int prio_step = wave_slot_id();
  for (int win0 = 0; win0 < n_all; win0 += 64) {
  const int n_mine = min(64, n_all - win0);
  const uint32_t item0 = item0_wave + (uint32_t)win0 * n_waves;
  int v_lo, v_hi;
  {
    const uint32_t item = item0 + (uint32_t)min(lane, n_mine - 1) * n_waves;
    const uint32_t ctr = item / groups;
    v_hi = g.ends[ctr];
    v_lo = g.ends[max((int)ctr - 1, 0)];
    if (ctr == 0) v_lo = 0;
  }
  auto uni = [](int x) { return __builtin_amdgcn_readfirstlane(x); };
  auto enter = [&](int j, int crow_keep, uint32_t item_keep) {
    ChunkCursor c;
    c.j = j, c.c0 = 0, c.start = 0, c.n_total = 0;
    c.crow = crow_keep, c.item = item_keep;
    if (j < n_mine) {
      const int lo = __builtin_amdgcn_readlane(v_lo, j), hi = __builtin_amdgcn_readlane(v_hi, j);
      c.start = lo, c.n_total = (hi - lo) << fnb_shift;
      c.item = item0 + (uint32_t)j * n_waves;
      const uint32_t ctr = c.item / groups;
      c.crow = uni((int)(ctr * (uint32_t)g.f_ctr + (c.item - ctr * groups) * (uint32_t)FC));
    }
    return c;
  };
  auto advance = [&](const ChunkCursor& c) {
    ChunkCursor r = c;
    if (c.c0 + 32 < c.n_total) r.c0 = c.c0 + 32;
    else if (c.j < n_mine) r = enter(c.j + 1, c.crow, c.item);
    r.j = uni(r.j), r.c0 = uni(r.c0), r.start = uni(r.start), r.n_total = uni(r.n_total), r.item = (uint32_t)uni((int)r.item);
    return r;
  };
  auto fe_of = [&](const ChunkCursor& c) { return max(min(c.c0 + kcol, c.n_total - 1), 0); };
  auto nbr_of = [&](const ChunkCursor& c) {
    const int e = c.start + (fe_of(c) >> fnb_shift);
    return (int)__builtin_amdgcn_raw_buffer_load_b32(nbr_rs, (e * g.nbr_stride + g.nbr_offset) * 4, 0, 0);
  };
  auto row_of = [&](int nb, const ChunkCursor& c) { return (nb << fnb_shift) + (fe_of(c) & fmask); };
  typedef const f32x4 __attribute__((address_space(4))) * crec_t;
  const crec_t ctr_rec = (crec_t)(uintptr_t)g.ctr_geom;
  auto centre = [&](const ChunkCursor& c, float yc[3], float rc[9]) {
    const int row = c.crow;
    const f32x4 v0 = ctr_rec[row * 4], v1 = ctr_rec[row * 4 + 1], v2 = ctr_rec[row * 4 + 2];
    if constexpr (FC == 2) {
      const f32x4 w0 = ctr_rec[row * 4 + 4], w1 = ctr_rec[row * 4 + 5], w2 = ctr_rec[row * 4 + 6];
      yc[0] = h ? w0[0] : v0[0], yc[1] = h ? w0[1] : v0[1], yc[2] = h ? w0[2] : v0[2], rc[8] = h ? w0[3] : v0[3];
#pragma unroll
      for (int i = 0; i < 4; ++i) rc[i] = h ? w1[i] : v1[i], rc[4 + i] = h ? w2[i] : v2[i];
    } else {
      yc[0] = v0[0], yc[1] = v0[1], yc[2] = v0[2], rc[8] = v0[3];
#pragma unroll
      for (int i = 0; i < 4; ++i) rc[i] = v1[i], rc[4 + i] = v2[i];
    }
  };

  ChunkCursor cur, n1, n2;
  cur = enter(0, 0, 0u);
  n1 = advance(cur);
  n2 = advance(n1);
  int q_cur, q_n1;
  float xn_nx[3], rn_nx[9];
  {
    const int nb_cur = nbr_of(cur);
    const int nb_n1 = nbr_of(n1);
    q_cur = row_of(nb_cur, cur);
    load_geom_record(nbg_rs, q_cur, xn_nx, rn_nx);
    q_n1 = row_of(nb_n1, n1);
#pragma unroll
    for (int i = 0; i < 3; ++i) asm volatile("" : "+v"(xn_nx[i]));
#pragma unroll
    for (int i = 0; i < 9; ++i) asm volatile("" : "+v"(rn_nx[i]));
  }
  float yc[3], rc[9];
  centre(cur, yc, rc);

  while (cur.j < n_mine) {
    rotate_priority(prio_step++);
    const int cnt = min(32, cur.n_total - cur.c0);
    const int qoff = cur.c0 + kcol < cur.n_total ? q_cur * row_bytes : kOobOffset;
    float xn[3], rn[9], d[9];
#pragma unroll
    for (int i = 0; i < 3; ++i) xn[i] = xn_nx[i];
#pragma unroll
    for (int i = 0; i < 9; ++i) rn[i] = rn_nx[i];
    const int nb_n2 = nbr_of(n2);

    uint32_t fw[2][VW][8];
#pragma unroll
    for (int s = 0; s < 2; ++s)
#pragma unroll
      for (int j = 0; j < 8; ++j) {
        const int src_off = __builtin_amdgcn_ds_bpermute(hb + 4 * acc_row(8 * s + j, 0), qoff);
        if constexpr (VW == 2) {
          const auto v = __builtin_amdgcn_raw_buffer_load_b64(feat_rs, src_off + cb4, 0, 0);
          fw[s][0][j] = v[0], fw[s][1][j] = v[1];
        } else {
          fw[s][0][j] = __builtin_amdgcn_raw_buffer_load_b32(feat_rs, src_off + cb4, 0, 0);
        }
      }
    load_geom_record(nbg_rs, q_n1, xn_nx, rn_nx);
    float yn[3], rnc[9];
    centre(n1, yn, rnc);

    if (TR == 0)
      edge_descriptor(xn, rn, yc, rc, rho, d);
    else
      edge_descriptor(yc, rc, xn, rn, rho, d);

    u32x4 own_hi, own_lo, oth_hi, oth_lo;
    frags_from_floats(d, own_hi, own_lo);
    {
      float d8 = d[8];
      if constexpr (FC == 2) {
        const auto sw = __builtin_amdgcn_permlane32_swap(__float_as_uint(d8), __float_as_uint(d8), false, false);
        d8 = __uint_as_float(h ? sw[0] : sw[1]);
      }
      uint32_t p_hi, p_lo;
      split2(d8, 1.0f, p_hi, p_lo);
      oth_hi = u32x4{p_hi, 0u, 0u, 0u};
      oth_lo = u32x4{p_lo, 0u, 0u, 0u};
    }
    u32x4 fa_hi[2][VW], fa_lo[2][VW];
#pragma unroll
    for (int a = 0; a < FC; ++a) {
      const bool dims07 = FC == 1 ? h == 0 : h == a;
      u32x4 a_hi, a_lo;
#pragma unroll
      for (int i = 0; i < 4; ++i) {
        a_hi[i] = dims07 ? own_hi[i] : oth_hi[i];
        a_lo[i] = dims07 ? own_lo[i] : oth_lo[i];
      }
      const u32x4 wb_hi = *reinterpret_cast<const u32x4*>(&lds_w[a][0][lane][0]);
      const u32x4 wb_lo = *reinterpret_cast<const u32x4*>(&lds_w[a][1][lane][0]);
      const f32x16 phi = mfma_bf16x3(a_hi, a_lo, wb_hi, wb_lo, zero16());
#pragma unroll
      for (int s = 0; s < 2; ++s) {
        if (s * 16 < cnt) {
          float pv[8];
#pragma unroll
          for (int j = 0; j < 8; ++j) pv[j] = gelu_scaled(phi[8 * s + j]);
          u32x4 b_hi, b_lo;
          frags_from_floats(pv, b_hi, b_lo);
#pragma unroll
          for (int t = 0; t < VW; ++t) {
            if (a == 0) frags_from_words(fw[s][t], fa_hi[s][t], fa_lo[s][t]);
            acc[a][t] = mfma_bf16x3(fa_hi[s][t], fa_lo[s][t], b_hi, b_lo, acc[a][t]);
          }
        }
      }
    }
    q_cur = q_n1;
    q_n1 = row_of(nb_n2, n2);
#pragma unroll
    for (int i = 0; i < 3; ++i) asm volatile("" : "+v"(xn_nx[i]));
#pragma unroll
    for (int i = 0; i < 9; ++i) asm volatile("" : "+v"(rn_nx[i]));
    if (n1.j != cur.j) {
#pragma unroll
      for (int a = 0; a < FC; ++a) {
        char* row = t_out + ((int64_t)cur.item * FC + a) * t24_row_bytes(C);
        if constexpr (VW == 2) {
#pragma unroll
          for (int r = 0; r < 16; ++r) {
            uint32_t hp, lp;
            t24_pack2(acc[a][0][r], acc[a][1][r], hp, lp);
            const int idx = acc_row(r, h) * kBasis + kcol;
            __builtin_nontemporal_store(hp, reinterpret_cast<uint32_t*>(row) + idx);
            __builtin_nontemporal_store((uint16_t)lp, reinterpret_cast<uint16_t*>(row + (int64_t)C * kBasis * 2) + idx);
          }
        } else {
#pragma unroll
          for (int r = 0; r < 16; r += 2) {
            uint32_t hp, lp;
            t24_pack2(acc[a][0][r], acc[a][0][r + 1], hp, lp);
            const int idx = (acc_row(r, h) >> 1) * kBasis + kcol;
            __builtin_nontemporal_store(hp, reinterpret_cast<uint32_t*>(row) + idx);
            __builtin_nontemporal_store((uint16_t)lp, reinterpret_cast<uint16_t*>(row + (int64_t)C * kBasis * 2) + idx);
          }
        }
#pragma unroll
        for (int t = 0; t < VW; ++t) acc[a][t] = zero16();
      }
    }
#pragma unroll
    for (int i = 0; i < 3; ++i) yc[i] = yn[i];
#pragma unroll
    for (int i = 0; i < 9; ++i) rc[i] = rnc[i];
    cur = n1, n1 = n2, n2 = advance(n2);
  }
  }
}

__global__ __launch_bounds__(256) void edge_param_grad_bf16_kernel(EdgeGeom g, const uint32_t* __restrict__ feat,
                                                                   int channels, const float* __restrict__ axes_ext,
                                                                   const float* __restrict__ rho_p,
                                                                   const uint32_t* __restrict__ grad_t,
                                                                   float* __restrict__ partials, int64_t rows) {
  __shared__ __attribute__((aligned(16))) float lds_desc[4][32][12];
  __shared__ float lds_red[4][kDescExt][kBasis];
  const int lane = threadIdx.x & 63, wave = threadIdx.x >> 6;
  const int kcol = lane & 31, h = lane >> 5;
  const float rho = *rho_p;
  u32x4 w_hi, w_lo;
  load_mlp_weights(axes_ext, kcol, h, w_hi, w_lo);
  float dacc[kDescExt];
#pragma unroll
  for (int j = 0; j < kDescExt; ++j) dacc[j] = 0.f;
  const bool vec_ok = (channels % 16) == 0;

  for (int64_t m = (int64_t)blockIdx.x * 4 + wave; m < rows; m += (int64_t)gridDim.x * 4) {
    const RowInfo ri = row_info(g, m);
    if (ri.n_total == 0) continue;
    float yc[3], rc[9];
#pragma unroll
    for (int i = 0; i < 3; ++i) yc[i] = g.ctr_pts[ri.ctr * 3 + i];
#pragma unroll
    for (int i = 0; i < 9; ++i) rc[i] = g.ctr_frames[m * 9 + i];
    const uint32_t* gt_row = grad_t + m * (int64_t)channels * kBasis;

    for (int c0 = 0; c0 < ri.n_total; c0 += 32) {
      const int cnt = min(32, ri.n_total - c0);
      const int fe = c0 + min(kcol, cnt - 1);
      float d[kDescExt];
      int q;
      lane_descriptor(g, ri, fe, yc, rc, rho, d, q);
      const f32x16 pre = mlp_preactivation(d, h, w_hi, w_lo);
      if (h == 0) {
        float4* dst = reinterpret_cast<float4*>(&lds_desc[wave][kcol][0]);
        dst[0] = make_float4(d[0], d[1], d[2], d[3]);
        dst[1] = make_float4(d[4], d[5], d[6], d[7]);
        dst[2] = make_float4(d[8], d[9], 0.f, 0.f);
      }

      f32x16 gphi = zero16();
      const uint32_t* f_row = feat + (int64_t)q * channels;
      for (int i0 = 0; i0 < channels; i0 += 16) {
        const int my0 = i0 + 8 * h;
        uint32_t wa[8], wb[8];
        if (vec_ok) {
          const uint4 v0 = *reinterpret_cast<const uint4*>(f_row + my0);
          const uint4 v1 = *reinterpret_cast<const uint4*>(f_row + my0 + 4);
          wa[0] = v0.x, wa[1] = v0.y, wa[2] = v0.z, wa[3] = v0.w, wa[4] = v1.x, wa[5] = v1.y, wa[6] = v1.z, wa[7] = v1.w;
#pragma unroll
          for (int j = 0; j < 8; ++j) wb[j] = gt_row[(int64_t)(my0 + j) * kBasis + kcol];
        } else {
#pragma unroll
          for (int j = 0; j < 8; ++j) {
            const bool ok = my0 + j < channels;
            wa[j] = ok ? f_row[my0 + j] : 0u;
            wb[j] = ok ? gt_row[(int64_t)(my0 + j) * kBasis + kcol] : 0u;
          }
        }
        u32x4 a_hi, a_lo, b_hi, b_lo;
        frags_from_words(wa, a_hi, a_lo);
        frags_from_words(wb, b_hi, b_lo);
        gphi = mfma_bf16x3(a_hi, a_lo, b_hi, b_lo, gphi);
      }

      __builtin_amdgcn_fence(__ATOMIC_RELEASE, "wavefront");
      __builtin_amdgcn_wave_barrier();
      __builtin_amdgcn_fence(__ATOMIC_ACQUIRE, "wavefront");
#pragma unroll
      for (int r = 0; r < 16; ++r) {
        const int n = acc_row(r, h);
        const float dy = gelu_scaled_dgrad(pre[r]);
        const float gp = n < cnt ? gphi[r] * dy : 0.f;
        const float4* src = reinterpret_cast<const float4*>(&lds_desc[wave][n][0]);
        const float4 d0 = src[0], d1 = src[1];
        const float2 d2 = *reinterpret_cast<const float2*>(&lds_desc[wave][n][8]);
        dacc[0] += d0.x * gp, dacc[1] += d0.y * gp, dacc[2] += d0.z * gp, dacc[3] += d0.w * gp;
        dacc[4] += d1.x * gp, dacc[5] += d1.y * gp, dacc[6] += d1.z * gp, dacc[7] += d1.w * gp;
        dacc[8] += d2.x * gp, dacc[9] += d2.y * gp;
      }
      __builtin_amdgcn_fence(__ATOMIC_RELEASE, "wavefront");
      __builtin_amdgcn_wave_barrier();
    }
  }

#pragma unroll
  for (int j = 0; j < kDescExt; ++j) {
    const float v = dacc[j] + __shfl_xor(dacc[j], 32);
    if (h == 0) lds_red[wave][j][kcol] = v;
  }
  __syncthreads();
  for (int i = threadIdx.x; i < kDescExt * kBasis; i += blockDim.x) {
    const int j = i / kBasis, k = i % kBasis;
    partials[(int64_t)blockIdx.x * kDescExt * kBasis + i] =
        lds_red[0][j][k] + lds_red[1][j][k] + lds_red[2][j][k] + lds_red[3][j][k];
  }
}

#ifndef SE3_PG_PAIR_WAVES
#define SE3_PG_PAIR_WAVES 3
#endif
#ifndef SE3_PG_SINGLE_WAVES
#define SE3_PG_SINGLE_WAVES 3
#endif
template <int CH16, int NFR, bool PAIR = false, bool POW2 = false>
__global__ __launch_bounds__(PAIR ? 128 : (NFR == 2 ? 512 : 256), PAIR ? SE3_PG_PAIR_WAVES : (NFR == 2 ? 2 : (CH16 == 3 ? 3 : SE3_PG_SINGLE_WAVES))) void edge_param_grad_bf16_v2_kernel(EdgeGeom g, const uint32_t* __restrict__ feat,
                                                                         int row_ch, int64_t feat_rows,
                                                                         const float* __restrict__ axes_ext,
                                                                         const float* __restrict__ rho_p,
                                                                         const uint32_t* __restrict__ grad_t,
                                                                         float* __restrict__ partials, int64_t n_items,
                                                                         int fnb_shift, int64_t item_lo = 0, int pipe = 0) {
  static_assert(!PAIR || NFR == 2, "the pair form shares the two frames of a point");
  constexpr int NW = PAIR ? 2 : (NFR == 2 ? 8 : 4);
  constexpr int NIMG = PAIR ? 1 : NW;
  constexpr int CSTEP = PAIR ? 64 : 32;
  const int c_off = 64 * (int)blockIdx.y;
  const int row_bytes = row_ch * 4;
  __shared__ __attribute__((aligned(16))) uint32_t lds_w[NFR][2][64][4];
  __shared__ __attribute__((aligned(16))) uint16_t lds_desc[NW][NFR][2][32][12];
  __shared__ __attribute__((aligned(16))) uint32_t lds_gt[NIMG][NFR][CH16][2][64][4];
  float(*lds_red)[kDescExt][kBasis] = reinterpret_cast<float(*)[kDescExt][kBasis]>(&lds_gt[0][0][0][0][0][0]);
  const int lane = threadIdx.x & 63, wave = threadIdx.x >> 6;
  TL(__shared__ uint32_t tl_lds[NW][32]; uint32_t* tl_rec = tl_lds[wave]; if (lane < 32) tl_rec[lane] = 0u; uint32_t tl_prev = tl_now(); tl_rec[18] = tl_prev;)
  const int img = PAIR ? 0 : wave;
  const int kcol = lane & 31, h = lane >> 5;
  if (threadIdx.x < 64) mlp_weights_to_lds<NFR>(reinterpret_cast<uint32_t(*)[2][64][4]>(&lds_w[0][0][0][0]), axes_ext, threadIdx.x);
  __syncthreads();
  const float rho = *rho_p;
  const __amdgpu_buffer_rsrc_t feat_rs = buffer_of(feat, feat_rows * row_bytes);
  const __amdgpu_buffer_rsrc_t nbg_rs = buffer_of(g.nb_geom, g.n_nb * g.f_nb * 64);
  const __amdgpu_buffer_rsrc_t ctrg_rs = buffer_of(g.ctr_geom, g.n_ctr * g.f_ctr * 64);
  f32x16 dacc = zero16();
  TL(tl_seg(tl_rec, tl_prev, 0);)

#ifndef SE3_PG_REVERSE
#define SE3_PG_REVERSE 1
#endif
  const int64_t item_stride = PAIR ? (int64_t)gridDim.x : (int64_t)gridDim.x * NW;
  const int groups = g.f_ctr / NFR;
  int v_lo = 0, v_hi = 0;
  if (pipe) {
    const int64_t item_f = min((int64_t)blockIdx.x + (int64_t)lane * item_stride, n_items - 1);
    const uint32_t ctr = (uint32_t)(item_lo + (SE3_PG_REVERSE ? n_items - 1 - item_f : item_f)) / (uint32_t)groups;
    v_hi = g.ends[ctr];
    v_lo = g.ends[max((int)ctr - 1, 0)];
    if (ctr == 0) v_lo = 0;
  }
  int64_t item_f = PAIR ? (int64_t)blockIdx.x : (int64_t)blockIdx.x * NW + wave;
  int64_t item = 0;
  int start = 0, n_total = 0, ctr_row = 0, local_j = 0;
  float yc[3], rc[9];
  constexpr int NBUILD = PAIR ? 1 : NFR;
  uint32_t gw[NBUILD][CH16][8];
  int nb_a = 0, nb_b = 0;
  const int c_first = PAIR ? 32 * wave : 0;
  auto nbr_of = [&](int c0) {
    const int fe = min(c0 + kcol, n_total - 1);
    const int e = start + (POW2 || fnb_shift >= 0 ? fe >> fnb_shift : fe / g.f_nb);
    return g.nbr[(int64_t)e * g.nbr_stride + g.nbr_offset];
  };
  auto row_of = [&](int nb, int c0) {
    const int fe = min(c0 + kcol, n_total - 1);
    return (POW2 ? nb << fnb_shift : nb * g.f_nb) + (POW2 || fnb_shift >= 0 ? fe & ((1 << fnb_shift) - 1) : fe % g.f_nb);
  };
  auto find_item = [&]() {
    for (; item_f < n_items; item_f += item_stride, ++local_j) {
      item = item_lo + (SE3_PG_REVERSE ? n_items - 1 - item_f : item_f);
      const int64_t ctr = (uint32_t)item / (uint32_t)groups;
      const int a0 = (int)((uint32_t)item - (uint32_t)ctr * (uint32_t)groups) * NFR;
      if (pipe) {
        start = __builtin_amdgcn_readlane(v_lo, local_j);
        n_total = (__builtin_amdgcn_readlane(v_hi, local_j) - start) * g.f_nb;
      } else {
        start = ctr > 0 ? g.ends[ctr - 1] : 0;
        n_total = (g.ends[ctr] - start) * g.f_nb;
      }
      ctr_row = (int)(ctr * g.f_ctr + a0 + (NFR == 2 ? h : 0));
      TL(tl_rec[16] += 1;)
      if (n_total != 0) return true;
    }
    return false;
  };
  auto issue_item_loads = [&]() {
    load_geom_record(ctrg_rs, ctr_row, yc, rc);
    nb_a = nbr_of(c_first);
    nb_b = nbr_of(c_first + CSTEP);
  };
  auto issue_image_loads = [&]() {
#pragma unroll
    for (int ab = 0; ab < NBUILD; ++ab) {
      const int a = PAIR ? wave : ab;
      const uint32_t* gt_row = grad_t + ((item * NFR + a) * (int64_t)row_ch + c_off) * kBasis;
      const int row_left = min(row_ch - c_off, 16 * CH16);
      const uint64_t gt_addr = reinterpret_cast<uint64_t>(gt_row);
      const uint64_t gt_base = ((uint64_t)(uint32_t)__builtin_amdgcn_readfirstlane((uint32_t)(gt_addr >> 32)) << 32) |
                               (uint64_t)(uint32_t)__builtin_amdgcn_readfirstlane((uint32_t)gt_addr);
      const __amdgpu_buffer_rsrc_t gt_rs = buffer_of(reinterpret_cast<const void*>(gt_base), (int64_t)row_left * kBasis * 4);
#pragma unroll
      for (int st = 0; st < CH16; ++st)
#pragma unroll
        for (int j = 0; j < 8; ++j)
          gw[ab][st][j] = __builtin_amdgcn_raw_buffer_load_b32(gt_rs, (8 * h * kBasis + kcol) * 4, (16 * st + j) * kBasis * 4, 0);
    }
  };
  int prio_step = wave_slot_id();
  bool have = find_item();
  TL(tl_seg(tl_rec, tl_prev, 1);)
  if (have) issue_item_loads();
  TL(tl_seg(tl_rec, tl_prev, 3);)
  while (have) {
    issue_image_loads();
    TL(tl_pin(nb_a); tl_seg(tl_rec, tl_prev, 4);)
    int q_a = row_of(nb_a, c_first);
    float xn_nx[3], rn_nx[9];
    load_geom_record(nbg_rs, q_a, xn_nx, rn_nx);
    TL(tl_pin(gw[NBUILD - 1][CH16 - 1][7]); tl_seg(tl_rec, tl_prev, 5);)
#pragma unroll
    for (int ab = 0; ab < NBUILD; ++ab)
#pragma unroll
      for (int st = 0; st < CH16; ++st) {
        const int a = PAIR ? wave : ab;
        u32x4 f_hi, f_lo;
        frags_from_words(gw[ab][st], f_hi, f_lo);
        *reinterpret_cast<u32x4*>(&lds_gt[img][a][st][0][lane][0]) = f_hi;
        *reinterpret_cast<u32x4*>(&lds_gt[img][a][st][1][lane][0]) = f_lo;
      }
    TL(tl_seg(tl_rec, tl_prev, 6);)
    if (PAIR) __syncthreads();
    TL(tl_seg(tl_rec, tl_prev, 7);)

    for (int c0 = c_first; c0 < n_total; c0 += CSTEP) {
      rotate_priority(prio_step++);
      const int cnt = min(32, n_total - c0);
      const int qoff = c0 + kcol < n_total ? q_a * row_bytes + c_off * 4 : kOobOffset;
      float d[9];
      const int q_b = row_of(nb_b, c0 + CSTEP);
      nb_b = nbr_of(c0 + 2 * CSTEP);

      uint32_t fw[CH16][8];
#pragma unroll
      for (int st = 0; st < CH16; ++st) {
        const int voff = c_off + 16 * st < row_ch ? qoff + (16 * st + 8 * h) * 4 : kOobOffset;
        const auto v0 = __builtin_amdgcn_raw_buffer_load_b128(feat_rs, voff, 0, 0);
        const auto v1 = __builtin_amdgcn_raw_buffer_load_b128(feat_rs, voff + 16, 0, 0);
        fw[st][0] = v0[0], fw[st][1] = v0[1], fw[st][2] = v0[2], fw[st][3] = v0[3];
        fw[st][4] = v1[0], fw[st][5] = v1[1], fw[st][6] = v1[2], fw[st][7] = v1[3];
      }
      q_a = q_b;
      TL(tl_seg(tl_rec, tl_prev, 8); tl_pin(xn_nx[0]); tl_pin(rn_nx[7]); tl_pin(rn_nx[8]); tl_seg(tl_rec, tl_prev, 9); tl_rec[17] += 1;)

      if (!g.transposed)
        edge_descriptor(xn_nx, rn_nx, yc, rc, rho, d);
      else
        edge_descriptor(yc, rc, xn_nx, rn_nx, rho, d);
      load_geom_record(nbg_rs, q_b, xn_nx, rn_nx);

      u32x4 own_hi, own_lo, oth_hi = {0u, 0u, 0u, 0u}, oth_lo = {0u, 0u, 0u, 0u};
      frags_from_floats(d, own_hi, own_lo);
      uint32_t own8_hi, own8_lo;
      split2(d[8], 1.0f, own8_hi, own8_lo);
      auto write_desc_rows = [&](int slot) {
        typedef uint32_t u32x2v __attribute__((ext_vector_type(2)));
        uint16_t* dh = &lds_desc[wave][slot][0][kcol][0];
        uint16_t* dl = &lds_desc[wave][slot][1][kcol][0];
        *reinterpret_cast<u32x2v*>(dh) = u32x2v{own_hi[0], own_hi[1]};
        *reinterpret_cast<u32x2v*>(dh + 4) = u32x2v{own_hi[2], own_hi[3]};
        *reinterpret_cast<u32x2v*>(dh + 8) = u32x2v{own8_hi, 0u};
        *reinterpret_cast<u32x2v*>(dl) = u32x2v{own_lo[0], own_lo[1]};
        *reinterpret_cast<u32x2v*>(dl + 4) = u32x2v{own_lo[2], own_lo[3]};
        *reinterpret_cast<u32x2v*>(dl + 8) = u32x2v{own8_lo, 0u};
      };
      if (NFR == 2 || h == 0) write_desc_rows(NFR == 2 ? h : 0);
      {
        float d8 = d[8];
        if (NFR == 2) {
          const auto sw = __builtin_amdgcn_permlane32_swap(__float_as_uint(d8), __float_as_uint(d8), false, false);
          d8 = __uint_as_float(h ? sw[0] : sw[1]);
        }
        uint32_t p_hi, p_lo;
        split2(d8, 1.0f, p_hi, p_lo);
        oth_hi = u32x4{p_hi, 0u, 0u, 0u};
        oth_lo = u32x4{p_lo, 0u, 0u, 0u};
      }
      __builtin_amdgcn_fence(__ATOMIC_RELEASE, "wavefront");
      __builtin_amdgcn_wave_barrier();
      __builtin_amdgcn_fence(__ATOMIC_ACQUIRE, "wavefront");

      const int tr_row = (lane >> 2) & 3, tr_col = min((lane & 3) * 4, 8);
      auto gelu_grad_of_frame = [&](int a, float (&dy)[16]) {
        const bool dims07 = NFR == 2 ? h == a : h == 0;
        u32x4 a_hi, a_lo;
#pragma unroll
        for (int i = 0; i < 4; ++i) {
          a_hi[i] = dims07 ? own_hi[i] : oth_hi[i];
          a_lo[i] = dims07 ? own_lo[i] : oth_lo[i];
        }
        const auto* wl = reinterpret_cast<const uint32_t(*)[2][64][4]>(&lds_w[0][0][0][0]);
        const u32x4 wb_hi = *reinterpret_cast<const u32x4*>(&wl[a][0][lane][0]);
        const u32x4 wb_lo = *reinterpret_cast<const u32x4*>(&wl[a][1][lane][0]);
        const f32x16 pre = mfma_bf16x3(a_hi, a_lo, wb_hi, wb_lo, zero16());
#pragma unroll
        for (int r = 0; r < 16; ++r) {
          dy[r] = gelu_scaled_dgrad(pre[r]);
        }
      };
      auto accumulate_frame = [&](int a, const u32x4 (&fa_hi)[CH16], const u32x4 (&fa_lo)[CH16], const float (&dy)[16]) {
        f32x16 gphi = zero16();
#pragma unroll
        for (int st = 0; st < CH16; ++st) {
          const u32x4 bg_hi = *reinterpret_cast<const u32x4*>(&lds_gt[img][a][st][0][lane][0]);
          const u32x4 bg_lo = *reinterpret_cast<const u32x4*>(&lds_gt[img][a][st][1][lane][0]);
          gphi = mfma_bf16x3(fa_hi[st], fa_lo[st], bg_hi, bg_lo, gphi);
        }
#pragma unroll
        for (int s = 0; s < 2; ++s) {
          if (s * 16 < cnt) {
            float gp[8];
#pragma unroll
            for (int j = 0; j < 8; ++j) gp[j] = gphi[8 * s + j] * dy[8 * s + j];
            u32x4 ga_hi, ga_lo;
            frags_from_floats(gp, ga_hi, ga_lo);
            const int r0 = 16 * s + 4 * h + tr_row;
            const u32x4 db_hi = lds_frag_tr16(&lds_desc[wave][a][0][r0][tr_col], &lds_desc[wave][a][0][r0 + 8][tr_col]);
            const u32x4 db_lo = lds_frag_tr16(&lds_desc[wave][a][1][r0][tr_col], &lds_desc[wave][a][1][r0 + 8][tr_col]);
            dacc = mfma_bf16x3(ga_hi, ga_lo, db_hi, db_lo, dacc);
          }
        }
      };
      u32x4 fa_hi[CH16], fa_lo[CH16];
      TL(tl_seg(tl_rec, tl_prev, 10);)
      float dyv[NFR][16];
#pragma unroll
      for (int a = 0; a < NFR; ++a) gelu_grad_of_frame(a, dyv[a]);
      TL(tl_pin(dyv[NFR - 1][15]); tl_seg(tl_rec, tl_prev, 11); tl_pin(fw[CH16 - 1][7]); tl_seg(tl_rec, tl_prev, 12);)
#pragma unroll
      for (int st = 0; st < CH16; ++st) frags_from_words(fw[st], fa_hi[st], fa_lo[st]);
#pragma unroll
      for (int a = 0; a < NFR; ++a) accumulate_frame(a, fa_hi, fa_lo, dyv[a]);
      __builtin_amdgcn_fence(__ATOMIC_RELEASE, "wavefront");
      __builtin_amdgcn_wave_barrier();
      TL(tl_seg(tl_rec, tl_prev, 13);)
    }
    item_f += item_stride, ++local_j;
    have = find_item();
    TL(tl_seg(tl_rec, tl_prev, 1);)
    if (have) issue_item_loads();
    TL(tl_seg(tl_rec, tl_prev, 3);)
    if (PAIR) __syncthreads();
    TL(tl_seg(tl_rec, tl_prev, 14);)
  }

  __syncthreads();
  if (kcol < kDescExt) {
#pragma unroll
    for (int r = 0; r < 16; ++r) lds_red[wave][kcol][acc_row(r, h)] = dacc[r];
  }
  __syncthreads();
  for (int i = threadIdx.x; i < kDescExt * kBasis; i += blockDim.x) {
    const int j = i / kBasis, k = i % kBasis;
    float sum = 0.f;
#pragma unroll
    for (int w = 0; w < NW; ++w) sum += lds_red[w][j][k];
    partials[((int64_t)blockIdx.y * gridDim.x + blockIdx.x) * kDescExt * kBasis + i] = sum;
  }
  TL(tl_seg(tl_rec, tl_prev, 15); tl_rec[19] = tl_prev;
     tl_rec[20] = __builtin_amdgcn_s_getreg((4 << 0) | (0 << 6) | (31 << 11)); tl_rec[21] = __builtin_amdgcn_s_getreg((20 << 0) | (0 << 6) | (31 << 11));
     tl_flush(2, (blockIdx.y * gridDim.x + blockIdx.x) * NW + wave, tl_rec, 32);)
}

__global__ void pack_geometry_kernel(const float* __restrict__ pts, const float* __restrict__ frames, int64_t rows,
                                     int f, float* __restrict__ records) {
  const int64_t row = (int64_t)blockIdx.x * blockDim.x + threadIdx.x;
  if (row >= rows) return;
  const int64_t pt = row / f;
  const float* r = frames + row * 9;
  float4* dst = reinterpret_cast<float4*>(records + row * 16);
  dst[0] = make_float4(pts[pt * 3], pts[pt * 3 + 1], pts[pt * 3 + 2], r[8]);
  dst[1] = make_float4(r[0], r[1], r[2], r[3]);
  dst[2] = make_float4(r[4], r[5], r[6], r[7]);
  dst[3] = make_float4(0.f, 0.f, 0.f, 0.f);
}

__global__ void split_pack_kernel(const float* __restrict__ src, uint32_t* __restrict__ dst, int64_t n) {
  const int64_t i4 = ((int64_t)blockIdx.x * blockDim.x + threadIdx.x) * 4;
  if (i4 + 3 < n) {
    const float4 v = *reinterpret_cast<const float4*>(src + i4);
    *reinterpret_cast<uint4*>(dst + i4) = make_uint4(split_pack(v.x), split_pack(v.y), split_pack(v.z), split_pack(v.w));
  } else {
    for (int64_t i = i4; i < n; ++i) dst[i] = split_pack(src[i]);
  }
}

}

int launch_pack_geometry(const float* pts, const float* frames, int64_t n, int f, float* records, hipStream_t stream) {
  const int64_t rows = n * f;
  if (rows == 0) return SE3_OK;
  if (rows * 64 >= (int64_t)kOobOffset) return SE3_ERR_UNSUPPORTED;
  hipLaunchKernelGGL(pack_geometry_kernel, dim3((unsigned)((rows + 255) / 256)), dim3(256), 0, stream, pts, frames, rows, f,
                     records);
  return check_launch();
}

int launch_split_pack(const float* src, uint32_t* dst, int64_t n, hipStream_t stream) {
  if (n == 0) return SE3_OK;
  ProfScope prof("split_pack", stream);
  const int64_t blocks = (n + 1023) / 1024;
  hipLaunchKernelGGL(split_pack_kernel, dim3((unsigned)blocks), dim3(256), 0, stream, src, dst, n);
  return check_launch();
}

static bool edge_t_bf16_uses_pair(const EdgeGeom& g, int channels) {
  return channels >= 64 && getenv("SE3_NO_PAIR") == nullptr && !(channels == 64 && g.f_ctr % 2 == 1);
}

bool edge_t_bf16_t24_rows(const EdgeGeom& g, int channels) {
  if (channels % 2 != 0) return false;
  if (edge_t_bf16_uses_pair(g, channels)) return true;
  return channels <= 32 || channels == 64;
}

bool edge_t_bf16_t16_rows(const EdgeGeom& g, int channels) {
  return channels % 64 == 0 && edge_t_bf16_uses_pair(g, channels);
}

static int edge_stream_min_items() {
  static const int v = [] {
    const char* e = getenv("SE3_EDGE_STREAM");
    return e ? (atoi(e) > 0 ? atoi(e) : INT32_MAX) : 4096;
  }();
  return v;
}

static int device_cu_count() {
  static int n_cu = 0;
  if (n_cu == 0) {
    int dev = 0;
    hipDeviceProp_t prop;
    if (hipGetDevice(&dev) != hipSuccess || hipGetDeviceProperties(&prop, dev) != hipSuccess) return -1;
    n_cu = prop.multiProcessorCount > 0 ? prop.multiProcessorCount : 256;
  }
  return n_cu;
}

int launch_edge_t_bf16(const char* tag, const EdgeGeom& g, const uint32_t* feat, int channels, int64_t feat_rows,
                       const float* axes_ext, const float* rho, uint32_t* t_out, hipStream_t stream, int rowfmt) {
  const bool t24 = rowfmt == 1;
  const int64_t rows = g.n_ctr * g.f_ctr;
  if (rows == 0) return SE3_OK;
  if (t24 && !edge_t_bf16_t24_rows(g, channels)) return SE3_ERR_UNSUPPORTED;
  if (rowfmt == 2 && !edge_t_bf16_t16_rows(g, channels)) return SE3_ERR_UNSUPPORTED;
  if (feat_rows * (int64_t)channels * 4 >= (int64_t)kOobOffset) return SE3_ERR_UNSUPPORTED;
  ProfScope prof(tag, stream);
  const int fc = g.f_ctr % 2 == 0 && channels % 128 != 0 ? 2 : 1;
  const int64_t items = rows / fc;
  int shift = -1;
  for (int sft = 0; sft < 8; ++sft)
    if ((1 << sft) == g.f_nb) shift = sft;
  const dim3 block(256);
  if (edge_t_bf16_uses_pair(g, channels)) {
    const bool two = g.f_ctr % 2 == 0;
    const int64_t pair_items = two ? rows / 2 : rows;
    if (channels == 64 && two && shift >= 0 && rowfmt == 1 && pair_items >= edge_stream_min_items() && g.n_edges > 0 &&
        g.n_edges * g.nbr_stride * 4 < (int64_t)kOobOffset && pair_items < (1ll << 31)) {
      const int n_cu = device_cu_count();
      if (n_cu <= 0) return SE3_ERR_LAUNCH;
      constexpr int per_cu = 2 * SE3_PAIR_WAVES;
      int64_t wgs = (int64_t)n_cu * per_cu;
      if (wgs > pair_items) wgs = pair_items;
      const dim3 sgrid((unsigned)wgs), sblock(128);
      if (g.transposed)
        hipLaunchKernelGGL((edge_t_stream_bf16_kernel<1>), sgrid, sblock, 0, stream, g, feat, feat_rows, axes_ext, rho,
                           reinterpret_cast<char*>(t_out), 0u, (uint32_t)pair_items, shift);
      else
        hipLaunchKernelGGL((edge_t_stream_bf16_kernel<0>), sgrid, sblock, 0, stream, g, feat, feat_rows, axes_ext, rho,
                           reinterpret_cast<char*>(t_out), 0u, (uint32_t)pair_items, shift);
      return check_launch();
    }
    const dim3 pgrid((unsigned)pair_items), pblock(128);
#define SE3_PAIR_T(CT, FULL, NF, P2, TR)                                                                                \
  hipLaunchKernelGGL((edge_t_pair_bf16_kernel<CT, FULL, NF, P2, TR>), pgrid, pblock, 0, stream, g, feat, channels, feat_rows, \
                     axes_ext, rho, t_out, 0, pair_items, shift, rowfmt)
#define SE3_PAIR_L(CT, FULL, NF, P2)                 \
  do {                                               \
    if (!(P2)) SE3_PAIR_T(CT, FULL, NF, P2, -1);     \
    else if (g.transposed) SE3_PAIR_T(CT, FULL, NF, P2, 1); \
    else SE3_PAIR_T(CT, FULL, NF, P2, 0);            \
  } while (0)
#define SE3_PAIR(CT, FULL)                                   \
  do {                                                       \
    if (two && shift >= 0) SE3_PAIR_L(CT, FULL, 2, true);    \
    else if (two) SE3_PAIR_L(CT, FULL, 2, false);            \
    else if (shift >= 0) SE3_PAIR_L(CT, FULL, 1, true);      \
    else SE3_PAIR_L(CT, FULL, 1, false);                     \
  } while (0)
    if (channels == 64) SE3_PAIR(1, true);
    else if (channels % 128 == 0) SE3_PAIR(2, true);
    else SE3_PAIR(2, false);
#undef SE3_PAIR
#undef SE3_PAIR_L
#undef SE3_PAIR_T
    return check_launch();
  }
  if (t24 && shift >= 0 && channels == 32 && fc == 2 && items >= edge_stream_min_items() && g.n_edges > 0 &&
      g.n_edges * g.nbr_stride * 4 < (int64_t)kOobOffset && items < (1ll << 31)) {
    const int n_cu = device_cu_count();
    if (n_cu <= 0) return SE3_ERR_LAUNCH;
    constexpr int per_cu = 3;
    int64_t wgs = (int64_t)n_cu * per_cu;
    if (wgs > (items + 3) / 4) wgs = (items + 3) / 4;
    const dim3 sgrid((unsigned)wgs);
    if (g.transposed)
      hipLaunchKernelGGL((edge_t_stream1_bf16_kernel<1, 2, 1>), sgrid, block, 0, stream, g, feat, feat_rows, axes_ext, rho,
                         reinterpret_cast<char*>(t_out), 0u, (uint32_t)items, shift);
    else
      hipLaunchKernelGGL((edge_t_stream1_bf16_kernel<1, 2, 0>), sgrid, block, 0, stream, g, feat, feat_rows, axes_ext, rho,
                         reinterpret_cast<char*>(t_out), 0u, (uint32_t)items, shift);
    return check_launch();
  }
  const dim3 grid((unsigned)((items + 3) / 4));
#define SE3_LAUNCH(VW, FC, FULL, T24)                                                                                 \
  hipLaunchKernelGGL((edge_t_bf16_kernel<VW, FC, FULL, T24>), grid, block, 0, stream, g, feat, channels, feat_rows,     \
                     axes_ext, rho, t_out, items, shift, 0)
#define SE3_LAUNCH_T(VW, FC, FULL)                   \
  do {                                               \
    if (t24) SE3_LAUNCH(VW, FC, FULL, true);         \
    else SE3_LAUNCH(VW, FC, FULL, false);            \
  } while (0)
  if (channels % 128 == 0) {
    SE3_LAUNCH(4, 1, true, false);
  } else if (channels % 64 == 0) {
    if (fc == 2) SE3_LAUNCH_T(2, 2, true); else SE3_LAUNCH_T(2, 1, true);
  } else if (channels % 32 == 0) {
    if (fc == 2) SE3_LAUNCH_T(1, 2, true); else SE3_LAUNCH_T(1, 1, true);
  } else {
    if (fc == 2) SE3_LAUNCH_T(1, 2, false); else SE3_LAUNCH_T(1, 1, false);
  }
#undef SE3_LAUNCH_T
#undef SE3_LAUNCH
  return check_launch();
}

int edge_param_grad_bf16_channel_blocks(int channels) { return channels > 64 && channels % 16 == 0 ? (channels + 63) / 64 : 1; }

int launch_edge_param_grad_bf16(const char* tag, const EdgeGeom& g, const uint32_t* feat, int channels,
                                int64_t feat_rows, const float* axes_ext, const float* rho, const uint32_t* grad_t,
                                float* partials, int n_partials, int* n_used, hipStream_t stream) {
  const int64_t rows = g.n_ctr * g.f_ctr;
  if (feat_rows * (int64_t)channels * 4 >= (int64_t)kOobOffset) return SE3_ERR_UNSUPPORTED;
  ProfScope prof(tag, stream);
  *n_used = n_partials;
  if (channels > 0 && (channels % 16 == 0 || channels < 16)) {
    int shift = -1;
    for (int sft = 0; sft < 8; ++sft)
      if ((1 << sft) == g.f_nb) shift = sft;
    static const bool force_single = getenv("SE3_PG_SINGLE") != nullptr;
    const bool two = g.f_ctr % 2 == 0 && !force_single;
    const int64_t items = two ? rows / 2 : rows;
    if (items <= 0) {
      *n_used = 0;
      return SE3_OK;
    }
    const int blocks_y = edge_param_grad_bf16_channel_blocks(channels);
    if (two && (channels >= 64 || channels == 32)) {
      const int n_cu = device_cu_count();
      if (n_cu <= 0) return SE3_ERR_LAUNCH;
      constexpr int per_cu = 6;
      int64_t wgs = (int64_t)n_cu * per_cu;
      if (wgs > n_partials) wgs = n_partials;
      if (wgs > items) wgs = items;
      if (wgs < 1) wgs = 1;
      const int pipe = (items + wgs - 1) / wgs <= 64 && items < (1ll << 31) ? 1 : 0;
      *n_used = (int)wgs * blocks_y;
      const dim3 pgrid((unsigned)wgs, (unsigned)blocks_y);
      if (channels == 32 && shift >= 0)
        hipLaunchKernelGGL((edge_param_grad_bf16_v2_kernel<2, 2, true, true>), pgrid, dim3(128), 0, stream, g, feat, channels,
                           feat_rows, axes_ext, rho, grad_t, partials, items, shift, 0, pipe);
      else if (channels == 32)
        hipLaunchKernelGGL((edge_param_grad_bf16_v2_kernel<2, 2, true, false>), pgrid, dim3(128), 0, stream, g, feat, channels,
                           feat_rows, axes_ext, rho, grad_t, partials, items, shift, 0, pipe);
      else if (shift >= 0)
        hipLaunchKernelGGL((edge_param_grad_bf16_v2_kernel<4, 2, true, true>), pgrid, dim3(128), 0, stream, g, feat, channels,
                           feat_rows, axes_ext, rho, grad_t, partials, items, shift, 0, pipe);
      else
        hipLaunchKernelGGL((edge_param_grad_bf16_v2_kernel<4, 2, true, false>), pgrid, dim3(128), 0, stream, g, feat, channels,
                           feat_rows, axes_ext, rho, grad_t, partials, items, shift, 0, pipe);
      return check_launch();
    }
    const int n_blocks = n_partials < 512 ? n_partials : 512;
    *n_used = n_blocks * blocks_y;
    const dim3 grid((unsigned)n_blocks, (unsigned)blocks_y);
#define SE3_PG_L(CH16, NFR, P2, THREADS)                                                                                  \
  hipLaunchKernelGGL((edge_param_grad_bf16_v2_kernel<CH16, NFR, false, P2>), grid, dim3(THREADS), 0, stream, g, feat, channels, \
                     feat_rows, axes_ext, rho, grad_t, partials, items, shift, 0)
#define SE3_PG1(CH16)                                      \
  do {                                                     \
    if (shift >= 0) SE3_PG_L(CH16, 1, true, 256);          \
    else SE3_PG_L(CH16, 1, false, 256);                    \
  } while (0)
#define SE3_PG(CH16)                                       \
  do {                                                     \
    if (two && shift >= 0) SE3_PG_L(CH16, 2, true, 512);   \
    else if (two) SE3_PG_L(CH16, 2, false, 512);           \
    else SE3_PG1(CH16);                                    \
  } while (0)
    switch (channels >= 64 ? 4 : (channels + 15) / 16) {
      case 1: SE3_PG(1); break;
      case 2: SE3_PG1(2); break;
      case 3: SE3_PG(3); break;
      default: SE3_PG1(4); break;
    }
#undef SE3_PG
#undef SE3_PG1
#undef SE3_PG_L
    return check_launch();
  }
  *n_used = n_partials < 512 ? n_partials : 512;
  hipLaunchKernelGGL(edge_param_grad_bf16_kernel, dim3(*n_used), dim3(256), 0, stream, g, feat, channels, axes_ext,
                     rho, grad_t, partials, rows);
  return check_launch();
}

}
```

se3conv3d_amd/ops.py:

```python
from __future__ import annotations

import ctypes as C
import functools
from dataclasses import dataclass, field
from typing import Callable, Optional, Tuple

import torch

from . import _lib
from ._lib import Se3Shape


import os as _os

_precision = _os.environ.get("SE3CONV_PRECISION", "bf16x3")
if _precision not in _lib.PRECISIONS:
    raise ValueError(f"SE3CONV_PRECISION={_precision!r}; expected one of {sorted(_lib.PRECISIONS)}")


def set_precision(name: str) -> None:
    global _precision
    if name not in _lib.PRECISIONS:
        raise ValueError(f"precision {name!r}; expected one of {sorted(_lib.PRECISIONS)}")
    _precision = name
# ... 590 lines not shown
    f32, i32 = torch.float32, torch.int32
    if not 1 <= int(k) <= 64:
        raise ValueError(f"knn_query: k = {k}; the kernels keep at most 64 neighbours per point (the reference's own "
                         "kernel has the same limit, knn_query.cu:167)")
    if method == "grid" and k > 32:
        raise ValueError("knn_query: the cell-grid search keeps at most 32 neighbours; use method='scan' or 'auto'")
    if method == "scan" or (method == "auto" and (n < KNN_GRID_MIN_POINTS or k > 32)) or n == 0:
        _lib.check(lib.se3_knn_query(_ptr(pts, f32, "pts"), _ptr(b, i32, "batch_ids", dev), n, int(k),
                                     _ptr(out, i32, "out"), _stream(dev)), "se3_knn_query")
        return out
    box_mn, mx = box if box is not None else batch_aabb(pts, b, n_batches)
    nb = box_mn.shape[0]
    mn = _empty((nb, 3), dtype=f32, device=dev)
    num_cells = _empty(3, dtype=i32, device=dev)
    cell3 = _empty(3, dtype=f32, device=dev)
    _lib.check(lib.se3_knn_grid_params(_ptr(b, i32, "batch_ids", dev), n, _ptr(box_mn, f32, "box_min", dev),
                                       _ptr(mx, f32, "box_max", dev), nb, int(k), float(KNN_CELL_FACTOR), _ptr(mn, f32, "aabb_min"),
                                       _ptr(num_cells, i32, "num_cells"), _ptr(cell3, f32, "cell_size"), _stream(dev)),
               "se3_knn_grid_params")
    ws = _workspace(lib.se3_knn_query_grid_workspace_bytes(n), dev)
    _lib.check(lib.se3_knn_query_grid(
        _ptr(pts, f32, "pts"), _ptr(b, i32, "batch_ids", dev), _ptr(mn, f32, "aabb_min"), _ptr(num_cells, i32, "num_cells"),
        _ptr(cell3, f32, "cell_size"), n, int(k), _ptr(out, i32, "out"), C.c_void_p(ws.data_ptr()), ws.numel(),
        _stream(dev)), "se3_knn_query_grid")
    return out


def knn_query_pair(pts_src, batch_src, pts_q, batch_q, k: int) -> torch.Tensor:
    lib = _lib.load()
    f32, i32 = torch.float32, torch.int32
    ps, pq = _as(pts_src, f32), _as(pts_q, f32)
    bs, bq = _as(batch_src, i32), _as(batch_q, i32)
    if ps.dim() != 2 or ps.shape[1] != 3 or pq.dim() != 2 or pq.shape[1] != 3:
        raise ValueError("knn_query_pair: only [N,3] point sets are supported")
    if not 1 <= int(k) <= 64:
        raise ValueError(f"knn_query_pair: k = {k}; at most 64 neighbours per point")
    dev = pq.device
    out = _empty((pq.shape[0], int(k)), dtype=i32, device=dev)
    _lib.check(lib.se3_knn_query_pair(_ptr(ps, f32, "pts_src", dev), _ptr(bs, i32, "batch_src", dev), ps.shape[0],
                                      _ptr(pq, f32, "pts_q"), _ptr(bq, i32, "batch_q", dev), pq.shape[0], int(k),
                                      _ptr(out, i32, "out"), _stream(dev)), "se3_knn_query_pair")
    return out


class KNNQuery(torch.autograd.Function):

    @staticmethod
    def forward(ctx, p_pt_src, p_batch_id_src, p_k):
        return knn_query(p_pt_src, p_batch_id_src, p_k)

    @staticmethod
    def backward(ctx, grad):
        return None, None, None


def pca_frames(pts, knn_ids, axis_fixed=None) -> torch.Tensor:
    lib = _lib.load()
    pts = _as(pts, torch.float32)
    ids = _as(knn_ids, torch.int32)
    n, k = ids.shape
    axis = int(axis_fixed) if axis_fixed else -1
    if axis not in (-1, 1, 2):
        raise ValueError(f"axis_fixed = {axis_fixed}")
    nf = 4 if axis < 0 else 2
    frames = _empty((n, nf, 9), dtype=torch.float32, device=pts.device)
    _lib.check(lib.se3_pca_frames(_ptr(pts, torch.float32, "pts"), _ptr(ids, torch.int32, "knn", pts.device), n, k, axis,
                                  _ptr(frames, torch.float32, "frames"), _stream(pts.device)), "se3_pca_frames")
    return frames


def shuffle_frames(all_frames, n_frames: int, draws=None) -> torch.Tensor:
    lib = _lib.load()
    all_frames = _as(all_frames, torch.float32)
    n, n_all = all_frames.shape[0], all_frames.shape[1]
    dev = all_frames.device
    if draws is None:
        draws = torch.rand((n, n_all), device=dev)
    draws = _as(draws, torch.float32)
    if tuple(draws.shape) != (n, n_all):
        raise ValueError(f"shuffle_frames: draws {tuple(draws.shape)}, expected {(n, n_all)}")
    out = _empty((n, int(n_frames), all_frames.shape[2]), dtype=torch.float32, device=dev)
    if all_frames.shape[2] != 9:
        raise ValueError("shuffle_frames: frames are [N, n_all, 9]")
    _lib.check(lib.se3_shuffle_frames(_ptr(all_frames, torch.float32, "all_frames"), _ptr(draws, torch.float32, "draws", dev), n,
                                      n_all, int(n_frames), _ptr(out, torch.float32, "out"), _stream(dev)), "se3_shuffle_frames")
    return out


class PreparedRecords:

    __slots__ = ("tensor", "valid", "key", "capture")

    def __init__(self):
        self.tensor, self.valid, self.key, self.capture = None, False, None, None

    def bind(self, pts: torch.Tensor, frames: torch.Tensor) -> "PreparedRecords":
        key = (pts.data_ptr(), pts._version, frames.data_ptr(), frames._version, tuple(frames.shape), str(pts.device))
        if key != self.key:
            rows = frames.shape[0] * frames.shape[1]
            if self.tensor is None or self.tensor.shape[0] != rows or self.tensor.device != pts.device:
                self.tensor = _empty((rows, 16), dtype=torch.float32, device=pts.device)
            self.key, self.valid, self.capture = key, False, None
        return self

    def filled_for(self, capture: Optional[int]) -> bool:
        return self.valid if capture is None else self.capture == capture

    def mark_filled(self, capture: Optional[int]) -> None:
        if capture is None:
            self.valid = True
        else:
            self.valid, self.capture = False, capture


def prepared_records(cloud) -> Optional["PreparedRecords"]:
    holder = getattr(cloud, "_se3_records_", None)
    if holder is None:
        holder = PreparedRecords()
        try:
            cloud._se3_records_ = holder
        except (AttributeError, TypeError):
            return None
    return holder


def invalidate_prepared(cloud) -> None:
    holder = getattr(cloud, "_se3_records_", None)
    if holder is not None:
        holder.valid, holder.capture = False, None


@functools.lru_cache(maxsize=1)
def _hip_get_capture_info():
    fn = C.CDLL("libamdhip64.so").hipStreamGetCaptureInfo
    fn.argtypes = [C.c_void_p, C.POINTER(C.c_int), C.POINTER(C.c_ulonglong)]
    fn.restype = C.c_int
    return fn


def _stream_capture_id(device) -> int:
    status, cid = C.c_int(0), C.c_ulonglong(0)
    err = _hip_get_capture_info()(_stream(device), C.byref(status), C.byref(cid))
    if err != 0 or status.value != 1:
        raise RuntimeError(f"hipStreamGetCaptureInfo: error {err}, capture status {status.value} on a capturing stream")
    return int(cid.value)


def _capture_id(device) -> Optional[int]:
    if device.type != "cuda" or not torch.cuda.is_current_stream_capturing():
        return None
    return _stream_capture_id(device)


@dataclass
class ConvGeometry:

    pts_in: torch.Tensor
    pts_out: torch.Tensor
    frames_in: torch.Tensor
    frames_out: torch.Tensor
    neighbors: torch.Tensor
    ends: torch.Tensor
    _transpose: Optional[Tuple[torch.Tensor, torch.Tensor]] = field(default=None, repr=False)
    symmetric: bool = False
    bounded: bool = False
    sources: Optional[torch.Tensor] = None
    edge_info: Optional[torch.Tensor] = None
    source_major_fn: Optional[Callable[[], Optional[Tuple[torch.Tensor, torch.Tensor]]]] = field(default=None, repr=False)
    _edge_ids: Optional[torch.Tensor] = field(default=None, repr=False)
    records_in: Optional[PreparedRecords] = field(default=None, repr=False)
    records_out: Optional[PreparedRecords] = field(default=None, repr=False)

    @staticmethod
    def build(pts_in, pts_out, frames_in, frames_out, neighbors, ends, symmetric: bool = False) -> "ConvGeometry":
        n_out = pts_out.shape[0]
        ends = _as(ends, torch.int32)
        if ends.shape[0] != n_out:
            raise ValueError(f"start_ids has {ends.shape[0]} entries, expected one per output point ({n_out})")
        fi = _as(frames_in, torch.float32).reshape(pts_in.shape[0], -1, 9)
        fo = _as(frames_out, torch.float32).reshape(n_out, -1, 9)
        nb = _as(neighbors, torch.int32)
        if nb.dim() != 2 or nb.shape[1] != 2:
            raise ValueError("neighbors must be [E,2]")
        if symmetric and pts_in.shape[0] != n_out:
            raise ValueError("a symmetric neighbourhood needs the same cloud on both sides")
        return ConvGeometry(_as(pts_in, torch.float32), _as(pts_out, torch.float32), fi, fo, nb, ends, None, symmetric)

    def transpose(self) -> Tuple[torch.Tensor, torch.Tensor]:
        if self._transpose is None:
            if self.symmetric:
                src = self.sources if self.sources is not None else self.neighbors[:, 1].contiguous()
                self._transpose = (src, self.ends)
            elif self.source_major_fn is not None and (own := self.source_major_fn()) is not None:
                self._transpose = own
            else:
                if self.bounded and self.edge_info is None:
                    raise ValueError("a capacity-bounded edge buffer between two clouds needs its device-side edge count "
                                     "(edge_info) to be transposed: rows past it are unset")
                ts, te, self._edge_ids = csr_transpose(self.neighbors, self.pts_in.shape[0],
                                                       self.edge_info if self.bounded else None, want_edge_ids=True)
                self._transpose = (ts, te)
        return self._transpose

    def shape(self, c_in: int, c_out: int, num_basis: int, precision: Optional[str] = None) -> Se3Shape:
        return Se3Shape(self.pts_in.shape[0], self.pts_out.shape[0], self.neighbors.shape[0],
                        self.frames_in.shape[1], self.frames_out.shape[1], c_in, c_out, num_basis,
                        _lib.PRECISIONS[precision or _precision])


def _geom_ptrs(g: ConvGeometry):
    f32, i32 = torch.float32, torch.int32
    dev = g.pts_out.device
    return [_ptr(g.pts_in, f32, "pts_in", dev), _ptr(g.pts_out, f32, "pts_out", dev),
            _ptr(g.frames_in, f32, "frames_in", dev), _ptr(g.frames_out, f32, "frames_out", dev),
            _ptr(g.neighbors, i32, "neighbors", dev), _ptr(g.ends, i32, "ends", dev)]


def _same_cloud(g: ConvGeometry) -> bool:
    return (g.pts_in.data_ptr() == g.pts_out.data_ptr() and g.frames_in.data_ptr() == g.frames_out.data_ptr()
            and g.pts_in.shape[0] == g.pts_out.shape[0] and g.frames_in.shape[1] == g.frames_out.shape[1])


def _prepared(geom: ConvGeometry, feat_words: Optional[torch.Tensor], feat_words_valid: bool):
    r_in, r_out = geom.records_in, geom.records_out
    if r_in is None and r_out is None and feat_words is None:
        return None, (), None
    p = _lib.Se3Prepared()
    filled = []
    capture = _capture_id(geom.pts_out.device) if (r_in is not None or r_out is not None) else None
    if _same_cloud(geom):
        r_out = None
    if r_in is not None:
        r_in.bind(geom.pts_in, geom.frames_in)
        p.geom_in, p.geom_in_valid = r_in.tensor.data_ptr(), int(r_in.filled_for(capture))
        filled.append(r_in)
    if r_out is not None and r_out is not r_in:
        r_out.bind(geom.pts_out, geom.frames_out)
        p.geom_out, p.geom_out_valid = r_out.tensor.data_ptr(), int(r_out.filled_for(capture))
        filled.append(r_out)
    elif r_out is r_in and r_in is not None:
        p.geom_out, p.geom_out_valid = p.geom_in, 1
    if feat_words is not None:
        p.feat_words, p.feat_words_valid = feat_words.data_ptr(), int(feat_words_valid)
    return p, tuple(filled), capture


def _scalar(t, name, dev) -> torch.Tensor:
    t = torch.as_tensor(t, dtype=torch.float32)
    return t.detach().to(device=dev, dtype=torch.float32).reshape(()).contiguous()


def se3conv_forward(geom: ConvGeometry, feat, proj_axes, proj_biases, conv_weights, rho, nu, save_t: bool = True,
                    precision: Optional[str] = None, feat_words: Optional[torch.Tensor] = None):
    lib = _lib.load()
    f32 = torch.float32
    dev = geom.pts_out.device
    feat = _as(feat, f32)
    a, b, w = _as(proj_axes, f32), _as(proj_biases, f32), _as(conv_weights, f32)
    if a.shape[0] != 9:
        raise ValueError(f"proj_axes_ has {a.shape[0]} rows; only the 9-D ('6D') descriptor is implemented")
    c_in, kb, c_out = w.shape
    if feat.shape != (geom.pts_in.shape[0] * geom.frames_in.shape[1], c_in):
        raise ValueError(f"features are {tuple(feat.shape)}, expected "
                         f"({geom.pts_in.shape[0] * geom.frames_in.shape[1]}, {c_in})")
    shp = geom.shape(c_in, c_out, kb, precision)
    rows = geom.pts_out.shape[0] * geom.frames_out.shape[1]
    out = _empty((rows, c_out), dtype=f32, device=dev)
    t_save = _empty((rows, c_in, kb), dtype=f32, device=dev) if (save_t and kb == 32) else None
    ws = _workspace(lib.se3conv_fwd_workspace_bytes(C.byref(shp), 1 if save_t else 0), dev)
    rho_t, nu_t = _scalar(rho, "rho", dev), _scalar(nu, "nu", dev)
    prep, filled, capture = _prepared(geom, feat_words, False)
    _lib.check(lib.se3conv_fwd_prepared(*_geom_ptrs(geom), _ptr(feat, f32, "features", dev), _ptr(a, f32, "proj_axes_", dev),
                                        _ptr(b, f32, "proj_biases_", dev), _ptr(w, f32, "conv_weights_", dev),
                                        _ptr(rho_t, f32, "norm_neigh_dist_"), _ptr(nu_t, f32, "norm_num_neighs_"),
                                        C.byref(shp), _ptr(out, f32, "out"), _ptr(t_save, f32, "t_save"),
                                        C.c_void_p(ws.data_ptr()), ws.numel(), _stream(dev),
                                        C.byref(prep) if prep is not None else None), "se3conv_fwd")
    for h in filled:
        h.mark_filled(capture)
    return out, t_save


def se3conv_backward(geom: ConvGeometry, feat, proj_axes, proj_biases, conv_weights, rho, nu, t_save, grad_out,
                     want_feat=True, want_params=True, precision: Optional[str] = None,
                     feat_words: Optional[torch.Tensor] = None):
    lib = _lib.load()
    f32, i32 = torch.float32, torch.int32
    dev = geom.pts_out.device
    feat = _as(feat, f32)
    a, b, w = _as(proj_axes, f32), _as(proj_biases, f32), _as(conv_weights, f32)
    g = _as(grad_out, f32)
    c_in, kb, c_out = w.shape
    shp = geom.shape(c_in, c_out, kb, precision)
    d_x = _empty_like(feat) if want_feat else None
    d_a = _empty_like(a) if want_params else None
    d_b = _empty_like(b) if want_params else None
    d_w = _empty_like(w) if want_params else None
    t_samples, t_ends = geom.transpose() if want_feat else (None, None)
    ws = _workspace(lib.se3conv_bwd_workspace_bytes(C.byref(shp), int(want_feat), int(want_params),
                                                    int(t_save is not None)), dev)
    rho_t, nu_t = _scalar(rho, "rho", dev), _scalar(nu, "nu", dev)
    prep, filled, capture = _prepared(geom, feat_words, feat_words is not None)
    _lib.check(lib.se3conv_bwd_prepared(*_geom_ptrs(geom), _ptr(t_samples, i32, "t_samples"), _ptr(t_ends, i32, "t_ends"),
                                        _ptr(geom._edge_ids if want_feat else None, i32, "t_edge_ids"),
                                        _ptr(feat, f32, "features", dev), _ptr(a, f32, "proj_axes_", dev),
                                        _ptr(b, f32, "proj_biases_", dev), _ptr(w, f32, "conv_weights_", dev),
                                        _ptr(rho_t, f32, "rho"), _ptr(nu_t, f32, "nu"), _ptr(t_save, f32, "t_save"),
                                        _ptr(g, f32, "grad_out", dev), C.byref(shp), _ptr(d_x, f32, "grad_feat"),
                                        _ptr(d_a, f32, "grad_axes"), _ptr(d_b, f32, "grad_biases"),
                                        _ptr(d_w, f32, "grad_weights"), C.c_void_p(ws.data_ptr()), ws.numel(), _stream(dev),
                                        C.byref(prep) if prep is not None else None), "se3conv_bwd")
    for h in filled:
        h.mark_filled(capture)
    return d_x, d_a, d_b, d_w


class SE3ConvFunction(torch.autograd.Function):

    @staticmethod
    def forward(ctx, feat, proj_axes, proj_biases, conv_weights, geom: ConvGeometry, rho, nu):
        need_params = any(ctx.needs_input_grad[1:4])
        ctx.precision = _precision
        save_t = need_params
        if save_t:
            c_in, kb, c_out = conv_weights.shape
            shp = geom.shape(c_in, c_out, kb, ctx.precision)
            save_t = _lib.load().se3conv_bwd_needs_t(C.byref(shp), int(bool(ctx.needs_input_grad[0]))) != 0
        fw = None
        if need_params and ctx.precision != "fp32" and conv_weights.shape[1] == 32 and feat.is_cuda:
            fw = _empty(feat.numel(), dtype=torch.int32, device=feat.device)
        out, t_save = se3conv_forward(geom, feat, proj_axes, proj_biases, conv_weights, rho, nu,
                                      save_t=save_t, precision=ctx.precision, feat_words=fw)
        ctx.geom = geom
        ctx.in_dtype = feat.dtype
        ctx.save_for_backward(feat, proj_axes, proj_biases, conv_weights, _scalar(rho, "rho", out.device),
                              _scalar(nu, "nu", out.device), t_save if t_save is not None else torch.empty(0),
                              fw if fw is not None else torch.empty(0))
        ctx.has_t = t_save is not None
        ctx.has_fw = fw is not None
        return out

    @staticmethod
    def backward(ctx, grad_out):
        feat, a, b, w, rho, nu, t_save, fw = ctx.saved_tensors
        want_feat = ctx.needs_input_grad[0]
        want_params = any(ctx.needs_input_grad[1:4])
        d_x, d_a, d_b, d_w = se3conv_backward(ctx.geom, feat, a, b, w, rho, nu, t_save if ctx.has_t else None,
                                              grad_out, want_feat, want_params, precision=ctx.precision,
                                              feat_words=fw if ctx.has_fw else None)
        if d_x is not None:
            d_x = d_x.to(ctx.in_dtype)
        ng = ctx.needs_input_grad
        return (d_x, d_a if ng[1] else None, d_b if ng[2] else None, d_w if ng[3] else None, None, None, None)


def rot_tensors(geom: ConvGeometry, rho, rel_rot: str = "6D"):
    lib = _lib.load()
    if rel_rot not in _lib.REL_ROT:
        raise ValueError(f"rel_rot {rel_rot!r}; expected one of {sorted(_lib.REL_ROT)}")
    mode, dims = _lib.REL_ROT[rel_rot]
    dev = geom.pts_out.device
    shp = geom.shape(1, 1, 32)
    ff = shp.f_in * shp.f_out
    e2 = geom.neighbors.shape[0] * ff
    desc = _empty((e2, dims), dtype=torch.float32, device=dev)
    fe_nb = _empty((e2, 2), dtype=torch.int32, device=dev)
    fe_ends = torch.zeros(geom.pts_out.shape[0] * shp.f_out, dtype=torch.int32, device=dev)
    rho_t = _scalar(rho, "rho", dev)
    _lib.check(lib.se3_rot_tensors_rel(*_geom_ptrs(geom), _ptr(rho_t, torch.float32, "rho"), C.byref(shp), mode,
                                       _ptr(desc, torch.float32, "desc"), _ptr(fe_nb, torch.int32, "fe_neighbors"),
                                       _ptr(fe_ends, torch.int32, "fe_ends"), _stream(dev)), "se3_rot_tensors_rel")
    return desc, fe_nb, fe_ends


class FeatBasisProj(torch.autograd.Function):

    @staticmethod
    def forward(p_ctx, p_pt_basis, p_pt_features, p_neighbors, p_start_ids):
        lib = _lib.load()
        f32, i32 = torch.float32, torch.int32
        basis, feat = _as(p_pt_basis, f32), _as(p_pt_features, f32)
        nb, ends = _as(p_neighbors, i32), _as(p_start_ids, i32)
        p_ctx.save_for_backward(basis, feat, nb, ends)
        p_ctx.dtypes = (p_pt_basis.dtype, p_pt_features.dtype)
        dev = feat.device
        rows, ch, kb = ends.shape[0], feat.shape[1], basis.shape[1]
        out = _empty((rows, ch, kb), dtype=f32, device=dev)
        _lib.check(lib.se3_feat_basis_proj(_ptr(basis, f32, "pt_basis", dev), _ptr(feat, f32, "pt_features"),
                                           _ptr(nb, i32, "neighbors", dev), _ptr(ends, i32, "start_ids", dev),
                                           nb.shape[0], rows, feat.shape[0], ch, kb, _ptr(out, f32, "out"),
                                           _stream(dev)), "se3_feat_basis_proj")
        return out

    @staticmethod
    def backward(p_ctx, p_grads):
        lib = _lib.load()
        f32, i32 = torch.float32, torch.int32
        basis, feat, nb, ends = p_ctx.saved_tensors
        g = _as(p_grads, f32)
        dev = feat.device
        g_feat = _empty_like(feat)
        g_basis = _empty_like(basis)
        _lib.check(lib.se3_feat_basis_proj_grad(
            _ptr(basis, f32, "pt_basis", dev), _ptr(feat, f32, "pt_features"), _ptr(nb, i32, "neighbors"),
            _ptr(ends, i32, "start_ids"), _ptr(g, f32, "grads", dev), nb.shape[0], ends.shape[0], feat.shape[0],
            feat.shape[1], basis.shape[1], _ptr(g_feat, f32, "g_feat"), _ptr(g_basis, f32, "g_basis"), _stream(dev)),
            "se3_feat_basis_proj_grad")
        return g_basis.to(p_ctx.dtypes[0]), g_feat.to(p_ctx.dtypes[1]), None, None


def _glue_ws(c: int, dev) -> torch.Tensor:
    return _workspace(_lib.load().se3_glue_workspace_bytes(int(c)), dev)


class BatchNormTrain(torch.autograd.Function):

    @staticmethod
    def forward(ctx, x, weight, bias, running_mean, running_var, momentum, eps, num_batches_tracked=None):
        lib = _lib.load()
        f32 = torch.float32
        x2 = _as(x, f32)
        if x2.dim() != 2:
            raise ValueError("BatchNormTrain: expected [rows, C] features")
        rows, c = x2.shape
        dev = x2.device
        y = _empty_like(x2)
        mean = _empty(c, dtype=f32, device=dev)
        invstd = _empty(c, dtype=f32, device=dev)
        w = _as(weight, f32) if weight is not None else None
        b = _as(bias, f32) if bias is not None else None
        ws = _glue_ws(c, dev)
        _lib.check(lib.se3_bn_fwd(_ptr(x2, f32, "x"), _ptr(w, f32, "weight", dev), _ptr(b, f32, "bias", dev), rows, c,
                                  float(eps), float(momentum), _ptr(running_mean, f32, "running_mean", dev),
                                  _ptr(running_var, f32, "running_var", dev),
                                  _ptr(num_batches_tracked, torch.int64, "num_batches_tracked", dev), _ptr(y, f32, "y"),
                                  _ptr(mean, f32, "mean"),
                                  _ptr(invstd, f32, "invstd"), C.c_void_p(ws.data_ptr()), ws.numel(), _stream(dev)),
                   "se3_bn_fwd")
        ctx.save_for_backward(x2, w if w is not None else torch.empty(0, device=dev), mean, invstd)
        ctx.has_w = w is not None
        ctx.mark_non_differentiable(*[t for t in (running_mean, running_var, num_batches_tracked) if t is not None])
        return y

    @staticmethod
    def backward(ctx, g):
        lib = _lib.load()
        f32 = torch.float32
        x2, w, mean, invstd = ctx.saved_tensors
        g2 = _as(g, f32)
        rows, c = x2.shape
        dev = x2.device
        dx = _empty_like(x2)
        dgamma = _empty(c, dtype=f32, device=dev)
        dbeta = _empty(c, dtype=f32, device=dev)
        ws = _glue_ws(c, dev)
        _lib.check(lib.se3_bn_bwd(_ptr(g2, f32, "dy", dev), _ptr(x2, f32, "x"), _ptr(mean, f32, "mean"),
                                  _ptr(invstd, f32, "invstd"), _ptr(w if ctx.has_w else None, f32, "weight"), rows, c,
                                  _ptr(dx, f32, "dx"), _ptr(dgamma, f32, "dgamma"), _ptr(dbeta, f32, "dbeta"),
                                  C.c_void_p(ws.data_ptr()), ws.numel(), _stream(dev)), "se3_bn_bwd")
        ng = ctx.needs_input_grad
        return (dx if ng[0] else None, dgamma if ng[1] else None, dbeta if ng[2] else None, None, None, None, None, None)


class SkipDropPath(torch.autograd.Function):
# ... 108 lines not shown
```

Measured before the change: 29.07 Mpoints/s.

## Add degree-sorted item-order tables for edge streaming and param-grad kernels

Adds a GPU histogram/scan/scatter pass that builds a permutation of (center, frame-pair) items ordered by neighbor count, in blocks and optionally reversed. The table is cached per geometry. The forward edge stream, transposed stream and param-grad pair kernels read item ids through it, which is meant to balance per-wave work and cut tail imbalance on the random-order point cloud. In exchange, every item lookup goes through an extra indirect load, and the table is rebuilt outside graph capture whenever the geometry changes.

```diff
diff --git a/include/se3conv_ordered.h b/include/se3conv_ordered.h
--- /dev/null
+++ b/include/se3conv_ordered.h
@@ -0,0 +1,37 @@
+#ifndef SE3CONV_ORDERED_H_
+#define SE3CONV_ORDERED_H_
+
+#include <stddef.h>
+#include <stdint.h>
+
+#include "se3conv.h"
+
+#ifdef __cplusplus
+extern "C" {
+#endif
+
+size_t se3_item_order_workspace_bytes(int64_t n_items, int64_t block_items);
+
+int se3_item_order_build(const int32_t* ends, int64_t n_ctr, int32_t f_ctr, int32_t f_nb, int32_t frames_per_item,
+                         int64_t block_items, int32_t reverse_blocks, uint32_t* order, void* workspace,
+                         size_t workspace_bytes, void* stream);
+
+int se3conv_fwd_ordered(const float* pts_in, const float* pts_out, const float* frames_in, const float* frames_out,
+                        const int32_t* neighbors, const int32_t* ends, const float* feat, const float* proj_axes,
+                        const float* proj_biases, const float* conv_weights, const float* rho, const float* nu,
+                        const se3conv_shape* s, float* out, float* t_save, void* workspace, size_t workspace_bytes,
+                        void* stream, const se3conv_prepared* prep, const uint32_t* order);
+
+int se3conv_bwd_ordered(const float* pts_in, const float* pts_out, const float* frames_in, const float* frames_out,
+                        const int32_t* neighbors, const int32_t* ends, const int32_t* t_samples, const int32_t* t_ends,
+                        const int32_t* t_edge_ids, const float* feat, const float* proj_axes, const float* proj_biases,
+                        const float* conv_weights, const float* rho, const float* nu, const float* t_save,
+                        const float* grad_out, const se3conv_shape* s, float* grad_feat, float* grad_axes,
+                        float* grad_biases, float* grad_weights, void* workspace, size_t workspace_bytes, void* stream,
+                        const se3conv_prepared* prep, const uint32_t* order, const uint32_t* order_t);
+
+#ifdef __cplusplus
+}
+#endif
+
+#endif
diff --git a/se3conv3d_amd/_lib.py b/se3conv3d_amd/_lib.py
--- a/se3conv3d_amd/_lib.py
+++ b/se3conv3d_amd/_lib.py
@@ -106,6 +106,13 @@
                                         _P, _I32, C.c_uint32, _P, _P]),
 }
 
+ORDERED_SIGNATURES = {
+    "se3_item_order_workspace_bytes": (_SZ, [_I64, _I64]),
+    "se3_item_order_build": (C.c_int, [_P, _I64, _I32, _I32, _I32, _I64, _I32, _P, _P, _SZ, _P]),
+    "se3conv_fwd_ordered": (C.c_int, [_P] * 12 + [_SHP, _P, _P, _P, _SZ, _P, C.POINTER(Se3Prepared), _P]),
+    "se3conv_bwd_ordered": (C.c_int, [_P] * 17 + [_SHP, _P, _P, _P, _P, _P, _SZ, _P, C.POINTER(Se3Prepared), _P, _P]),
+}
+
 _lib = None
 
 
@@ -122,7 +129,7 @@
     if lib.se3_abi_version() != ABI_VERSION:
         raise Se3LibraryError(f"{LIB_PATH} has ABI version {lib.se3_abi_version()}, this binding expects {ABI_VERSION}: "
                               "rebuild it (`python -m se3conv3d_amd.build`)")
-    for name, (res, args) in list(SIGNATURES.items()) + list(CAPPED_SIGNATURES.items()):
+    for name, (res, args) in list(SIGNATURES.items()) + list(CAPPED_SIGNATURES.items()) + list(ORDERED_SIGNATURES.items()):
         try:
             fn = getattr(lib, name)
         except AttributeError:
diff --git a/se3conv3d_amd/build.py b/se3conv3d_amd/build.py
--- a/se3conv3d_amd/build.py
+++ b/se3conv3d_amd/build.py
@@ -13,9 +13,9 @@
 LIBDIR = os.path.join(PKG, "lib")
 OBJDIR = os.path.join(LIBDIR, "obj" + SUFFIX) if SUFFIX else LIBDIR
 LIB = os.path.join(LIBDIR, f"libse3conv_hip{SUFFIX}.so")
-SOURCES = ["geometry.hip", "edge_kernels.hip", "edge_bf16.hip", "edge_dx.hip", "gemm.hip", "gemm_bf16.hip", "prep.hip", "frames.hip", "glue.hip", "api.hip"]
+SOURCES = ["geometry.hip", "edge_kernels.hip", "edge_bf16.hip", "edge_dx.hip", "gemm.hip", "gemm_bf16.hip", "prep.hip", "frames.hip", "glue.hip", "item_order.hip", "api.hip"]
 HEADERS = [os.path.join(CSRC, "common.h"), os.path.join(CSRC, "edge_bf16_body.h"), os.path.join(os.path.dirname(PKG), "include", "se3conv.h"),
-           os.path.join(os.path.dirname(PKG), "include", "se3conv_capped.h")]
+           os.path.join(os.path.dirname(PKG), "include", "se3conv_capped.h"), os.path.join(os.path.dirname(PKG), "include", "se3conv_ordered.h")]
 ARCH = "gfx950"
 FLAGS = os.environ.get("SE3_CXXFLAGS", "").split() + ["-O3", "-fno-slp-vectorize", "-std=c++17", "-fPIC", f"--offload-arch={ARCH}", "-fno-gpu-rdc", "-Wall", "-Wno-unused-function"]
 
diff --git a/se3conv3d_amd/csrc/api.hip b/se3conv3d_amd/csrc/api.hip
--- a/se3conv3d_amd/csrc/api.hip
+++ b/se3conv3d_amd/csrc/api.hip
@@ -7,6 +7,7 @@
 #include <vector>
 
 #include "common.h"
+#include "../../include/se3conv_ordered.h"
 
 namespace se3 {
 
@@ -598,6 +599,15 @@
                                     const float* proj_biases, const float* conv_weights, const float* rho, const float* nu,
                                     const se3conv_shape* s, float* out, float* t_save, void* workspace, size_t workspace_bytes,
                                     void* stream_, const se3conv_prepared* prep) {
+  return se3conv_fwd_ordered(pts_in, pts_out, frames_in, frames_out, neighbors, ends, feat, proj_axes, proj_biases, conv_weights,
+                             rho, nu, s, out, t_save, workspace, workspace_bytes, stream_, prep, nullptr);
+}
+
+extern "C" int se3conv_fwd_ordered(const float* pts_in, const float* pts_out, const float* frames_in, const float* frames_out,
+                                   const int32_t* neighbors, const int32_t* ends, const float* feat, const float* proj_axes,
+                                   const float* proj_biases, const float* conv_weights, const float* rho, const float* nu,
+                                   const se3conv_shape* s, float* out, float* t_save, void* workspace, size_t workspace_bytes,
+                                   void* stream_, const se3conv_prepared* prep, const uint32_t* order) {
   if (!shape_ok(s)) return SE3_ERR_INVALID_ARGUMENT;
   if (s->num_basis != kBasis) {
     if (s->n_out == 0) return SE3_OK;
@@ -635,6 +645,7 @@
   float* t = t_save ? t_save : (float*)(ws + p.t);
 
   EdgeGeom g = forward_geom(s, pts_in, pts_out, frames_in, frames_out, neighbors, ends);
+  g.order = order;
   const int64_t rows_out = s->n_out * s->f_out;
   const int ck = s->c_in * s->num_basis;
   const float inv_fin = 1.0f / (float)s->f_in;
@@ -696,6 +707,19 @@
                                     const float* t_save, const float* grad_out, const se3conv_shape* s, float* grad_feat,
                                     float* grad_axes, float* grad_biases, float* grad_weights, void* workspace,
                                     size_t workspace_bytes, void* stream_, const se3conv_prepared* prep) {
+  return se3conv_bwd_ordered(pts_in, pts_out, frames_in, frames_out, neighbors, ends, t_samples, t_ends, t_edge_ids, feat, proj_axes,
+                             proj_biases, conv_weights, rho, nu, t_save, grad_out, s, grad_feat, grad_axes, grad_biases, grad_weights,
+                             workspace, workspace_bytes, stream_, prep, nullptr, nullptr);
+}
+
+extern "C" int se3conv_bwd_ordered(const float* pts_in, const float* pts_out, const float* frames_in, const float* frames_out,
+                                   const int32_t* neighbors, const int32_t* ends, const int32_t* t_samples,
+                                   const int32_t* t_ends, const int32_t* t_edge_ids, const float* feat, const float* proj_axes,
+                                   const float* proj_biases, const float* conv_weights, const float* rho, const float* nu,
+                                   const float* t_save, const float* grad_out, const se3conv_shape* s, float* grad_feat,
+                                   float* grad_axes, float* grad_biases, float* grad_weights, void* workspace,
+                                   size_t workspace_bytes, void* stream_, const se3conv_prepared* prep, const uint32_t* order,
+                                   const uint32_t* order_t) {
   if (!shape_ok(s)) return SE3_ERR_INVALID_ARGUMENT;
   if (s->num_basis != kBasis) {
     const bool wf = grad_feat != nullptr, wp = grad_axes || grad_biases || grad_weights;
@@ -751,6 +775,7 @@
 
   EdgeGeom g = forward_geom(s, pts_in, pts_out, frames_in, frames_out, neighbors, ends);
   EdgeGeom gt = transposed_geom(s, pts_in, pts_out, frames_in, frames_out, t_samples, t_ends);
+  g.order = order, gt.order = order_t;
   PrepBatch pb;
   pb.axes(proj_axes, proj_biases, axes_ext);
   prepare_geometry(pb, prep, s, (float*)(ws + p.geom_in), (float*)(ws + p.geom_out), &g, &gt);
diff --git a/se3conv3d_amd/csrc/common.h b/se3conv3d_amd/csrc/common.h
--- a/se3conv3d_amd/csrc/common.h
+++ b/se3conv3d_amd/csrc/common.h
@@ -308,6 +308,7 @@
   int64_t n_ctr;
   int f_ctr, f_nb;
   int transposed;
+  const uint32_t* order;
 };
 
 int launch_edge_t(const char* tag, const EdgeGeom& g, const float* feat, int channels, int64_t feat_rows,
diff --git a/se3conv3d_amd/csrc/edge_bf16.hip b/se3conv3d_amd/csrc/edge_bf16.hip
--- a/se3conv3d_amd/csrc/edge_bf16.hip
+++ b/se3conv3d_amd/csrc/edge_bf16.hip
@@ -340,7 +340,7 @@
   uint32_t item;
 };
 
-template <int TR>
+template <int TR, bool ORD = false>
 __global__ __launch_bounds__(128, SE3_PAIR_WAVES) void edge_t_stream_bf16_kernel(
     EdgeGeom g, const uint32_t* __restrict__ feat, int64_t feat_rows, const float* __restrict__ axes_ext,
     const float* __restrict__ rho_p, char* __restrict__ t_out, uint32_t item_lo, uint32_t item_hi, int fnb_shift) {
@@ -370,8 +370,10 @@
   const int n_mine = min(64, n_all - win0);
   const uint32_t item0 = item0_wg + (uint32_t)win0 * gridDim.x;
   int v_lo, v_hi;
+  [[maybe_unused]] uint32_t v_item = 0u;
   {
-    const uint32_t item = item0 + (uint32_t)min(lane, n_mine - 1) * gridDim.x;
+    uint32_t item = item0 + (uint32_t)min(lane, n_mine - 1) * gridDim.x;
+    if constexpr (ORD) item = v_item = g.order[item];
     const uint32_t ctr = item / groups;
     v_hi = g.ends[ctr];
     v_lo = g.ends[max((int)ctr - 1, 0)];
@@ -385,7 +387,8 @@
     if (j < n_mine) {
       const int lo = __builtin_amdgcn_readlane(v_lo, j), hi = __builtin_amdgcn_readlane(v_hi, j);
       c.start = lo, c.n_total = (hi - lo) << fnb_shift;
-      c.item = item0 + (uint32_t)j * gridDim.x;
+      if constexpr (ORD) c.item = (uint32_t)__builtin_amdgcn_readlane((int)v_item, j);
+      else c.item = item0 + (uint32_t)j * gridDim.x;
       const uint32_t ctr = c.item / groups;
       c.crow = uni((int)(ctr * (uint32_t)g.f_ctr + (c.item - ctr * groups) * 2u) + wv);
     }
@@ -535,7 +538,7 @@
      tl_rec[14] = tl_chunks; tl_rec[15] = (uint32_t)n_all; tl_flush(TR == 1 ? 1 : 0, blockIdx.x * 2 + wv, tl_rec);)
 }
 
-template <int VW, int FC, int TR>
+template <int VW, int FC, int TR, bool ORD = false>
 __global__ __launch_bounds__(256, (VW == 1 && FC == 1) ? 4 : 3) void edge_t_stream1_bf16_kernel(
     EdgeGeom g, const uint32_t* __restrict__ feat, int64_t feat_rows, const float* __restrict__ axes_ext,
     const float* __restrict__ rho_p, char* __restrict__ t_out, uint32_t item_lo, uint32_t item_hi, int fnb_shift) {
@@ -567,8 +570,10 @@
   const int n_mine = min(64, n_all - win0);
   const uint32_t item0 = item0_wave + (uint32_t)win0 * n_waves;
   int v_lo, v_hi;
+  [[maybe_unused]] uint32_t v_item = 0u;
   {
-    const uint32_t item = item0 + (uint32_t)min(lane, n_mine - 1) * n_waves;
+    uint32_t item = item0 + (uint32_t)min(lane, n_mine - 1) * n_waves;
+    if constexpr (ORD) item = v_item = g.order[item];
     const uint32_t ctr = item / groups;
     v_hi = g.ends[ctr];
     v_lo = g.ends[max((int)ctr - 1, 0)];
@@ -582,7 +587,8 @@
     if (j < n_mine) {
       const int lo = __builtin_amdgcn_readlane(v_lo, j), hi = __builtin_amdgcn_readlane(v_hi, j);
       c.start = lo, c.n_total = (hi - lo) << fnb_shift;
-      c.item = item0 + (uint32_t)j * n_waves;
+      if constexpr (ORD) c.item = (uint32_t)__builtin_amdgcn_readlane((int)v_item, j);
+      else c.item = item0 + (uint32_t)j * n_waves;
       const uint32_t ctr = c.item / groups;
       c.crow = uni((int)(ctr * (uint32_t)g.f_ctr + (c.item - ctr * groups) * (uint32_t)FC));
     }
@@ -860,7 +866,7 @@
 #ifndef SE3_PG_SINGLE_WAVES
 #define SE3_PG_SINGLE_WAVES 3
 #endif
-template <int CH16, int NFR, bool PAIR = false, bool POW2 = false>
+template <int CH16, int NFR, bool PAIR = false, bool POW2 = false, bool ORD = false>
 __global__ __launch_bounds__(PAIR ? 128 : (NFR == 2 ? 512 : 256), PAIR ? SE3_PG_PAIR_WAVES : (NFR == 2 ? 2 : (CH16 == 3 ? 3 : SE3_PG_SINGLE_WAVES))) void edge_param_grad_bf16_v2_kernel(EdgeGeom g, const uint32_t* __restrict__ feat,
                                                                          int row_ch, int64_t feat_rows,
                                                                          const float* __restrict__ axes_ext,
@@ -896,10 +902,13 @@
 #endif
   const int64_t item_stride = PAIR ? (int64_t)gridDim.x : (int64_t)gridDim.x * NW;
   const int groups = g.f_ctr / NFR;
+  static_assert(!ORD || PAIR, "only the pair form reads an item-order table");
   int v_lo = 0, v_hi = 0;
+  [[maybe_unused]] uint32_t v_item = 0u;
   if (pipe) {
     const int64_t item_f = min((int64_t)blockIdx.x + (int64_t)lane * item_stride, n_items - 1);
-    const uint32_t ctr = (uint32_t)(item_lo + (SE3_PG_REVERSE ? n_items - 1 - item_f : item_f)) / (uint32_t)groups;
+    if constexpr (ORD) v_item = g.order[item_f];
+    const uint32_t ctr = (uint32_t)(item_lo + (ORD ? (int64_t)v_item : (SE3_PG_REVERSE ? n_items - 1 - item_f : item_f))) / (uint32_t)groups;
     v_hi = g.ends[ctr];
     v_lo = g.ends[max((int)ctr - 1, 0)];
     if (ctr == 0) v_lo = 0;
@@ -923,7 +932,8 @@
   };
   auto find_item = [&]() {
     for (; item_f < n_items; item_f += item_stride, ++local_j) {
-      item = item_lo + (SE3_PG_REVERSE ? n_items - 1 - item_f : item_f);
+      if constexpr (ORD) item = item_lo + (int64_t)(uint32_t)__builtin_amdgcn_readlane((int)v_item, local_j);
+      else item = item_lo + (SE3_PG_REVERSE ? n_items - 1 - item_f : item_f);
       const int64_t ctr = (uint32_t)item / (uint32_t)groups;
       const int a0 = (int)((uint32_t)item - (uint32_t)ctr * (uint32_t)groups) * NFR;
       if (pipe) {
@@ -1227,12 +1237,12 @@
       int64_t wgs = (int64_t)n_cu * per_cu;
       if (wgs > pair_items) wgs = pair_items;
       const dim3 sgrid((unsigned)wgs), sblock(128);
-      if (g.transposed)
-        hipLaunchKernelGGL((edge_t_stream_bf16_kernel<1>), sgrid, sblock, 0, stream, g, feat, feat_rows, axes_ext, rho,
-                           reinterpret_cast<char*>(t_out), 0u, (uint32_t)pair_items, shift);
-      else
-        hipLaunchKernelGGL((edge_t_stream_bf16_kernel<0>), sgrid, sblock, 0, stream, g, feat, feat_rows, axes_ext, rho,
-                           reinterpret_cast<char*>(t_out), 0u, (uint32_t)pair_items, shift);
+#define SE3_STREAM(TR, ORD)                                                                                                 \
+  hipLaunchKernelGGL((edge_t_stream_bf16_kernel<TR, ORD>), sgrid, sblock, 0, stream, g, feat, feat_rows, axes_ext, rho, \
+                     reinterpret_cast<char*>(t_out), 0u, (uint32_t)pair_items, shift)
+      if (g.transposed) { if (g.order) SE3_STREAM(1, true); else SE3_STREAM(1, false); }
+      else { if (g.order) SE3_STREAM(0, true); else SE3_STREAM(0, false); }
+#undef SE3_STREAM
       return check_launch();
     }
     const dim3 pgrid((unsigned)pair_items), pblock(128);
@@ -1268,12 +1278,12 @@
     int64_t wgs = (int64_t)n_cu * per_cu;
     if (wgs > (items + 3) / 4) wgs = (items + 3) / 4;
     const dim3 sgrid((unsigned)wgs);
-    if (g.transposed)
-      hipLaunchKernelGGL((edge_t_stream1_bf16_kernel<1, 2, 1>), sgrid, block, 0, stream, g, feat, feat_rows, axes_ext, rho,
-                         reinterpret_cast<char*>(t_out), 0u, (uint32_t)items, shift);
-    else
-      hipLaunchKernelGGL((edge_t_stream1_bf16_kernel<1, 2, 0>), sgrid, block, 0, stream, g, feat, feat_rows, axes_ext, rho,
-                         reinterpret_cast<char*>(t_out), 0u, (uint32_t)items, shift);
+#define SE3_STREAM1(TR, ORD)                                                                                                 \
+  hipLaunchKernelGGL((edge_t_stream1_bf16_kernel<1, 2, TR, ORD>), sgrid, block, 0, stream, g, feat, feat_rows, axes_ext, rho, \
+                     reinterpret_cast<char*>(t_out), 0u, (uint32_t)items, shift)
+    if (g.transposed) { if (g.order) SE3_STREAM1(1, true); else SE3_STREAM1(1, false); }
+    else { if (g.order) SE3_STREAM1(0, true); else SE3_STREAM1(0, false); }
+#undef SE3_STREAM1
     return check_launch();
   }
   const dim3 grid((unsigned)((items + 3) / 4));
@@ -1331,18 +1341,15 @@
       const int pipe = (items + wgs - 1) / wgs <= 64 && items < (1ll << 31) ? 1 : 0;
       *n_used = (int)wgs * blocks_y;
       const dim3 pgrid((unsigned)wgs, (unsigned)blocks_y);
-      if (channels == 32 && shift >= 0)
-        hipLaunchKernelGGL((edge_param_grad_bf16_v2_kernel<2, 2, true, true>), pgrid, dim3(128), 0, stream, g, feat, channels,
-                           feat_rows, axes_ext, rho, grad_t, partials, items, shift, 0, pipe);
-      else if (channels == 32)
-        hipLaunchKernelGGL((edge_param_grad_bf16_v2_kernel<2, 2, true, false>), pgrid, dim3(128), 0, stream, g, feat, channels,
-                           feat_rows, axes_ext, rho, grad_t, partials, items, shift, 0, pipe);
-      else if (shift >= 0)
-        hipLaunchKernelGGL((edge_param_grad_bf16_v2_kernel<4, 2, true, true>), pgrid, dim3(128), 0, stream, g, feat, channels,
-                           feat_rows, axes_ext, rho, grad_t, partials, items, shift, 0, pipe);
-      else
-        hipLaunchKernelGGL((edge_param_grad_bf16_v2_kernel<4, 2, true, false>), pgrid, dim3(128), 0, stream, g, feat, channels,
-                           feat_rows, axes_ext, rho, grad_t, partials, items, shift, 0, pipe);
+      const bool ord = g.order != nullptr && pipe && shift >= 0;
+#define SE3_PG_PAIR(CH16, P2, ORD)                                                                                          \
+  hipLaunchKernelGGL((edge_param_grad_bf16_v2_kernel<CH16, 2, true, P2, ORD>), pgrid, dim3(128), 0, stream, g, feat, channels, \
+                     feat_rows, axes_ext, rho, grad_t, partials, items, shift, 0, pipe)
+      if (channels == 32 && shift >= 0) { if (ord) SE3_PG_PAIR(2, true, true); else SE3_PG_PAIR(2, true, false); }
+      else if (channels == 32) SE3_PG_PAIR(2, false, false);
+      else if (shift >= 0) { if (ord) SE3_PG_PAIR(4, true, true); else SE3_PG_PAIR(4, true, false); }
+      else SE3_PG_PAIR(4, false, false);
+#undef SE3_PG_PAIR
       return check_launch();
     }
     const int n_blocks = n_partials < 512 ? n_partials : 512;
diff --git a/se3conv3d_amd/csrc/item_order.hip b/se3conv3d_amd/csrc/item_order.hip
--- /dev/null
+++ b/se3conv3d_amd/csrc/item_order.hip
@@ -0,0 +1,156 @@
+#include "common.h"
+#include "../../include/se3conv_ordered.h"
+
+namespace se3 {
+namespace {
+
+constexpr int kOrderCap = 4;
+constexpr int kOrderClasses = kOrderCap + 1;
+constexpr int kOrderTile = 1024;
+constexpr int kFieldBits = 12;
+
+__device__ __forceinline__ int order_class(const int32_t* __restrict__ ends, uint32_t item, uint32_t groups, int f_nb) {
+  const uint32_t ctr = item / groups;
+  const int lo = ctr > 0 ? ends[ctr - 1] : 0;
+  const int64_t fe = (int64_t)(ends[ctr] - lo) * f_nb;
+  const int64_t chunks = (fe + 31) / 32;
+  return (int)(chunks < kOrderCap ? (chunks < 0 ? 0 : chunks) : kOrderCap);
+}
+
+__device__ __forceinline__ uint64_t tile_scan(const int32_t* __restrict__ ends, uint32_t first, uint32_t hi, uint32_t groups,
+                                              int f_nb, int cls[4], uint64_t* total) {
+  __shared__ uint64_t lds_scan[2][256];
+  uint64_t mine = 0;
+#pragma unroll
+  for (int k = 0; k < 4; ++k) {
+    const uint32_t item = first + 4u * threadIdx.x + (uint32_t)k;
+    cls[k] = -1;
+    if (item < hi && item >= first) {
+      cls[k] = kOrderCap - order_class(ends, item, groups, f_nb);
+      mine += 1ull << (kFieldBits * cls[k]);
+    }
+  }
+  int cur = 0;
+  lds_scan[0][threadIdx.x] = mine;
+  __syncthreads();
+  for (int d = 1; d < 256; d <<= 1, cur ^= 1) {
+    uint64_t v = lds_scan[cur][threadIdx.x];
+    if ((int)threadIdx.x >= d) v += lds_scan[cur][threadIdx.x - d];
+    lds_scan[cur ^ 1][threadIdx.x] = v;
+    __syncthreads();
+  }
+  const uint64_t incl = lds_scan[cur][threadIdx.x];
+  *total = lds_scan[cur][255];
+  __syncthreads();
+  return incl - mine;
+}
+
+__global__ __launch_bounds__(256) void order_hist_kernel(const int32_t* __restrict__ ends, uint32_t n_items, uint32_t groups,
+                                                         int f_nb, uint32_t block, uint32_t tiles_per_block,
+                                                         uint32_t* __restrict__ hist) {
+  const uint32_t b = blockIdx.x / tiles_per_block, t = blockIdx.x % tiles_per_block;
+  const uint64_t lo64 = (uint64_t)b * block, hi64 = lo64 + block < n_items ? lo64 + block : n_items;
+  const uint64_t first64 = lo64 + (uint64_t)t * kOrderTile;
+  int cls[4];
+  uint64_t total;
+  const uint32_t first = first64 < hi64 ? (uint32_t)first64 : (uint32_t)hi64;
+  tile_scan(ends, first, (uint32_t)hi64, groups, f_nb, cls, &total);
+  if (threadIdx.x < kOrderClasses)
+    hist[(size_t)blockIdx.x * kOrderClasses + threadIdx.x] = (uint32_t)(total >> (kFieldBits * threadIdx.x)) & ((1u << kFieldBits) - 1u);
+}
+
+__global__ __launch_bounds__(256) void order_scan_kernel(uint32_t n_items, uint32_t block, uint32_t tiles_per_block,
+                                                         int reverse_blocks, uint32_t* __restrict__ hist) {
+  __shared__ uint32_t lds[2][256];
+  const uint32_t b = blockIdx.x;
+  const uint64_t lo64 = (uint64_t)b * block, hi64 = lo64 + block < n_items ? lo64 + block : n_items;
+  uint32_t running = reverse_blocks ? (uint32_t)(n_items - hi64) : (uint32_t)lo64;
+  uint32_t* h = hist + (size_t)b * tiles_per_block * kOrderClasses;
+  for (int c = 0; c < kOrderClasses; ++c)
+    for (uint32_t t0 = 0; t0 < tiles_per_block; t0 += 256) {
+      const uint32_t t = t0 + threadIdx.x;
+      const uint32_t mine = t < tiles_per_block ? h[(size_t)t * kOrderClasses + c] : 0u;
+      int cur = 0;
+      lds[0][threadIdx.x] = mine;
+      __syncthreads();
+      for (int d = 1; d < 256; d <<= 1, cur ^= 1) {
+        uint32_t v = lds[cur][threadIdx.x];
+        if ((int)threadIdx.x >= d) v += lds[cur][threadIdx.x - d];
+        lds[cur ^ 1][threadIdx.x] = v;
+        __syncthreads();
+      }
+      const uint32_t incl = lds[cur][threadIdx.x], total = lds[cur][255];
+      __syncthreads();
+      if (t < tiles_per_block) h[(size_t)t * kOrderClasses + c] = running + incl - mine;
+      running += total;
+    }
+}
+
+__global__ __launch_bounds__(256) void order_scatter_kernel(const int32_t* __restrict__ ends, uint32_t n_items, uint32_t groups,
+                                                            int f_nb, uint32_t block, uint32_t tiles_per_block,
+                                                            const uint32_t* __restrict__ offs, uint32_t* __restrict__ order) {
+  const uint32_t b = blockIdx.x / tiles_per_block, t = blockIdx.x % tiles_per_block;
+  const uint64_t lo64 = (uint64_t)b * block, hi64 = lo64 + block < n_items ? lo64 + block : n_items;
+  const uint64_t first64 = lo64 + (uint64_t)t * kOrderTile;
+  int cls[4];
+  uint64_t total;
+  const uint32_t first = first64 < hi64 ? (uint32_t)first64 : (uint32_t)hi64;
+  uint64_t before = tile_scan(ends, first, (uint32_t)hi64, groups, f_nb, cls, &total);
+#pragma unroll
+  for (int k = 0; k < 4; ++k) {
+    if (cls[k] < 0) continue;
+    const uint32_t rank = (uint32_t)(before >> (kFieldBits * cls[k])) & ((1u << kFieldBits) - 1u);
+    const uint32_t pos = offs[(size_t)blockIdx.x * kOrderClasses + cls[k]] + rank;
+    if (pos < n_items) order[pos] = first + 4u * threadIdx.x + (uint32_t)k;
+    before += 1ull << (kFieldBits * cls[k]);
+  }
+}
+
+struct OrderPlan {
+  uint32_t block, n_blocks, tiles_per_block;
+  size_t bytes;
+};
+
+bool order_plan(int64_t n_items, int64_t block_items, OrderPlan* p) {
+  if (n_items < 0 || n_items >= (1ll << 31) || block_items < 0 || block_items % kOrderTile != 0) return false;
+  const int64_t block = block_items == 0 || block_items >= n_items ? (n_items > 0 ? n_items : 1) : block_items;
+  p->block = (uint32_t)block;
+  p->n_blocks = (uint32_t)((n_items + block - 1) / block);
+  p->tiles_per_block = (uint32_t)((block + kOrderTile - 1) / kOrderTile);
+  p->bytes = (size_t)p->n_blocks * p->tiles_per_block * kOrderClasses * sizeof(uint32_t);
+  return true;
+}
+
+}
+}
+
+using namespace se3;
+
+extern "C" size_t se3_item_order_workspace_bytes(int64_t n_items, int64_t block_items) {
+  OrderPlan p;
+  if (!order_plan(n_items, block_items, &p)) return 0;
+  return align_up(p.bytes, 256);
+}
+
+extern "C" int se3_item_order_build(const int32_t* ends, int64_t n_ctr, int32_t f_ctr, int32_t f_nb, int32_t frames_per_item,
+                                    int64_t block_items, int32_t reverse_blocks, uint32_t* order, void* workspace,
+                                    size_t workspace_bytes, void* stream_) {
+  if (n_ctr < 0 || f_ctr <= 0 || f_nb <= 0 || frames_per_item <= 0 || f_ctr % frames_per_item != 0) return SE3_ERR_INVALID_ARGUMENT;
+  const int64_t groups = f_ctr / frames_per_item, n_items = n_ctr * groups;
+  OrderPlan p;
+  if (!order_plan(n_items, block_items, &p)) return n_items >= (1ll << 31) ? SE3_ERR_UNSUPPORTED : SE3_ERR_INVALID_ARGUMENT;
+  if (n_items == 0) return SE3_OK;
+  if (!ends || !order || !workspace) return SE3_ERR_INVALID_ARGUMENT;
+  if (workspace_bytes < p.bytes) return SE3_ERR_WORKSPACE;
+  hipStream_t stream = (hipStream_t)stream_;
+  ProfScope prof("item_order", stream);
+  uint32_t* hist = (uint32_t*)workspace;
+  const dim3 tiles(p.n_blocks * p.tiles_per_block), wg(256);
+  hipLaunchKernelGGL(order_hist_kernel, tiles, wg, 0, stream, ends, (uint32_t)n_items, (uint32_t)groups, f_nb, p.block,
+                     p.tiles_per_block, hist);
+  hipLaunchKernelGGL(order_scan_kernel, dim3(p.n_blocks), wg, 0, stream, (uint32_t)n_items, p.block, p.tiles_per_block,
+                     reverse_blocks != 0, hist);
+  hipLaunchKernelGGL(order_scatter_kernel, tiles, wg, 0, stream, ends, (uint32_t)n_items, (uint32_t)groups, f_nb, p.block,
+                     p.tiles_per_block, hist, order);
+  return check_launch();
+}
diff --git a/se3conv3d_amd/ops.py b/se3conv3d_amd/ops.py
--- a/se3conv3d_amd/ops.py
+++ b/se3conv3d_amd/ops.py
@@ -766,6 +766,51 @@
     return _stream_capture_id(device)
 
 
+ITEM_ORDER_STAGES = frozenset(t for t in _os.environ.get("SE3_ITEM_ORDER", "fwd,tr,pg").split(",") if t in ("fwd", "tr", "pg"))
+ITEM_ORDER_BLOCK = int(_os.environ.get("SE3_ITEM_ORDER_BLOCK", "0"))
+ITEM_ORDER_MIN = int(_os.environ.get("SE3_ITEM_ORDER_MIN", "4096"))
+
+
+def item_order(ends: torch.Tensor, f_ctr: int, f_nb: int, block_items: int = 0, reverse_blocks: bool = False,
+               out: Optional[torch.Tensor] = None) -> torch.Tensor:
+    lib = _lib.load()
+    dev = ends.device
+    n_ctr = int(ends.shape[0])
+    n_items = n_ctr * (f_ctr // 2)
+    if out is None:
+        out = _empty(n_items, dtype=torch.int32, device=dev)
+    ws = _workspace(lib.se3_item_order_workspace_bytes(n_items, block_items), dev)
+    _lib.check(lib.se3_item_order_build(_ptr(ends, torch.int32, "ends"), n_ctr, f_ctr, f_nb, 2, block_items, int(reverse_blocks),
+                                        _ptr(out, torch.int32, "order", dev), C.c_void_p(ws.data_ptr()), ws.numel(), _stream(dev)),
+               "se3_item_order_build")
+    return out
+
+
+class ItemOrder:
+
+    __slots__ = ("table", "key")
+
+    def __init__(self):
+        self.table, self.key = None, None
+
+    def get(self, ends: torch.Tensor, f_ctr: int, f_nb: int, reverse_blocks: bool) -> Optional[torch.Tensor]:
+        n_items = int(ends.shape[0]) * (f_ctr // 2)
+        if (not ends.is_cuda or f_ctr % 2 != 0 or f_nb & (f_nb - 1) != 0 or n_items < ITEM_ORDER_MIN
+                or n_items >= 1 << 31):
+            return None
+        key = (ends.data_ptr(), ends._version, n_items, f_ctr, f_nb, ITEM_ORDER_BLOCK, bool(reverse_blocks), str(ends.device))
+        if key == self.key:
+            return self.table
+        if torch.cuda.is_current_stream_capturing():
+            return None
+        if self.table is None or self.table.shape[0] != n_items or self.table.device != ends.device:
+            self.table = None
+        self.key = None
+        self.table = item_order(ends, f_ctr, f_nb, ITEM_ORDER_BLOCK, reverse_blocks, out=self.table)
+        self.key = key
+        return self.table
+
+
 @dataclass
 class ConvGeometry:
 
@@ -784,6 +829,22 @@
     _edge_ids: Optional[torch.Tensor] = field(default=None, repr=False)
     records_in: Optional[PreparedRecords] = field(default=None, repr=False)
     records_out: Optional[PreparedRecords] = field(default=None, repr=False)
+    _order: ItemOrder = field(default_factory=ItemOrder, repr=False)
+    _order_t: ItemOrder = field(default_factory=ItemOrder, repr=False)
+
+    def item_orders(self, want_t: bool, kb: int, precision: Optional[str]):
+        if not ITEM_ORDER_STAGES or kb != 32 or (precision or _precision) == "fp32":
+            return None, None
+        f_in, f_out = int(self.frames_in.shape[1]), int(self.frames_out.shape[1])
+        order = self._order.get(self.ends, f_out, f_in, True)
+        order_t = None
+        if want_t and "tr" in ITEM_ORDER_STAGES:
+            t_ends = self.transpose()[1]
+            if t_ends.data_ptr() == self.ends.data_ptr() and f_in == f_out:
+                order_t = order
+            else:
+                order_t = self._order_t.get(t_ends, f_in, f_out, False)
+        return order, order_t
 
     @staticmethod
     def build(pts_in, pts_out, frames_in, frames_out, neighbors, ends, symmetric: bool = False) -> "ConvGeometry":
@@ -884,12 +945,14 @@
     ws = _workspace(lib.se3conv_fwd_workspace_bytes(C.byref(shp), 1 if save_t else 0), dev)
     rho_t, nu_t = _scalar(rho, "rho", dev), _scalar(nu, "nu", dev)
     prep, filled, capture = _prepared(geom, feat_words, False)
-    _lib.check(lib.se3conv_fwd_prepared(*_geom_ptrs(geom), _ptr(feat, f32, "features", dev), _ptr(a, f32, "proj_axes_", dev),
-                                        _ptr(b, f32, "proj_biases_", dev), _ptr(w, f32, "conv_weights_", dev),
-                                        _ptr(rho_t, f32, "norm_neigh_dist_"), _ptr(nu_t, f32, "norm_num_neighs_"),
-                                        C.byref(shp), _ptr(out, f32, "out"), _ptr(t_save, f32, "t_save"),
-                                        C.c_void_p(ws.data_ptr()), ws.numel(), _stream(dev),
-                                        C.byref(prep) if prep is not None else None), "se3conv_fwd")
+    order = geom.item_orders(False, kb, precision)[0] if "fwd" in ITEM_ORDER_STAGES else None
+    fwd = lib.se3conv_fwd_prepared if order is None else lib.se3conv_fwd_ordered
+    _lib.check(fwd(*_geom_ptrs(geom), _ptr(feat, f32, "features", dev), _ptr(a, f32, "proj_axes_", dev),
+                   _ptr(b, f32, "proj_biases_", dev), _ptr(w, f32, "conv_weights_", dev),
+                   _ptr(rho_t, f32, "norm_neigh_dist_"), _ptr(nu_t, f32, "norm_num_neighs_"),
+                   C.byref(shp), _ptr(out, f32, "out"), _ptr(t_save, f32, "t_save"),
+                   C.c_void_p(ws.data_ptr()), ws.numel(), _stream(dev), C.byref(prep) if prep is not None else None,
+                   *(() if order is None else (_ptr(order, torch.int32, "order", dev),))), "se3conv_fwd")
     for h in filled:
         h.mark_filled(capture)
     return out, t_save
@@ -915,15 +978,20 @@
                                                     int(t_save is not None)), dev)
     rho_t, nu_t = _scalar(rho, "rho", dev), _scalar(nu, "nu", dev)
     prep, filled, capture = _prepared(geom, feat_words, feat_words is not None)
-    _lib.check(lib.se3conv_bwd_prepared(*_geom_ptrs(geom), _ptr(t_samples, i32, "t_samples"), _ptr(t_ends, i32, "t_ends"),
-                                        _ptr(geom._edge_ids if want_feat else None, i32, "t_edge_ids"),
-                                        _ptr(feat, f32, "features", dev), _ptr(a, f32, "proj_axes_", dev),
-                                        _ptr(b, f32, "proj_biases_", dev), _ptr(w, f32, "conv_weights_", dev),
-                                        _ptr(rho_t, f32, "rho"), _ptr(nu_t, f32, "nu"), _ptr(t_save, f32, "t_save"),
-                                        _ptr(g, f32, "grad_out", dev), C.byref(shp), _ptr(d_x, f32, "grad_feat"),
-                                        _ptr(d_a, f32, "grad_axes"), _ptr(d_b, f32, "grad_biases"),
-                                        _ptr(d_w, f32, "grad_weights"), C.c_void_p(ws.data_ptr()), ws.numel(), _stream(dev),
-                                        C.byref(prep) if prep is not None else None), "se3conv_bwd")
+    order, order_t = geom.item_orders(want_feat, kb, precision)
+    if not (want_params and "pg" in ITEM_ORDER_STAGES):
+        order = None
+    tables = () if order is None and order_t is None else (_ptr(order, torch.int32, "order", dev), _ptr(order_t, torch.int32, "order_t", dev))
+    bwd = lib.se3conv_bwd_ordered if tables else lib.se3conv_bwd_prepared
+    _lib.check(bwd(*_geom_ptrs(geom), _ptr(t_samples, i32, "t_samples"), _ptr(t_ends, i32, "t_ends"),
+                   _ptr(geom._edge_ids if want_feat else None, i32, "t_edge_ids"),
+                   _ptr(feat, f32, "features", dev), _ptr(a, f32, "proj_axes_", dev),
+                   _ptr(b, f32, "proj_biases_", dev), _ptr(w, f32, "conv_weights_", dev),
+                   _ptr(rho_t, f32, "rho"), _ptr(nu_t, f32, "nu"), _ptr(t_save, f32, "t_save"),
+                   _ptr(g, f32, "grad_out", dev), C.byref(shp), _ptr(d_x, f32, "grad_feat"),
+                   _ptr(d_a, f32, "grad_axes"), _ptr(d_b, f32, "grad_biases"),
+                   _ptr(d_w, f32, "grad_weights"), C.c_void_p(ws.data_ptr()), ws.numel(), _stream(dev),
+                   C.byref(prep) if prep is not None else None, *tables), "se3conv_bwd")
     for h in filled:
         h.mark_filled(capture)
     return d_x, d_a, d_b, d_w
```

Measured after the change: 29.01 Mpoints/s. About the same (-0.2%).
